# HPCForge/Bubbleformer

Hardware: AMD Instinct MI355X
Metric: train samples/sec, FiLMAViT 16x192x192x4ch, bs=8 per GPU (higher is better)
Workload: dtype bf16; 1 GPU; FiLMAViT-small (E=384, 6 heads, 12 blocks, P=16, 9 fluid params) fwd + relative-L2 loss + bwd + AdamW, 4-field 16x192x192 clips, batch 8 per GPU (BASELINE.json configs[1]); global_batch=8, parallelism=dp1

## Files before the change

### bubbleformer_amd/_lib.py

```python
import ctypes as C
import os
import subprocess

_HERE = os.path.dirname(os.path.abspath(__file__))
LIB_PATH = os.path.join(_HERE, "libbubbleformer_hip.so")
CSRC = os.path.join(_HERE, "csrc")

BF_DTYPE_F32, BF_DTYPE_BF16 = 0, 1
BF_LAY_KC, BF_LAY_XC = 0, 1
BF_PRO_NONE, BF_PRO_AFFINE, BF_PRO_AFFINE_GELU, BF_PRO_GELU = 0, 1, 2, 3
BF_AUX_NONE, BF_AUX_ADD, BF_AUX_DGELU = 0, 1, 2
BF_OUT_STORE, BF_OUT_STORE_F32, BF_OUT_ATOMIC_F32 = 0, 1, 2
BF_MAX_STAGES = 5
BF_LOSS_LIMBS = 5

vp, fp, i32, i64, f32 = C.c_void_p, C.c_void_p, C.c_int32, C.c_int64, C.c_float


class Operand(C.Structure):
    _fields_ = [("p", vp), ("ld", i64), ("layout", i32), ("seglen", i32), ("segstride", i64), ("gw", i32), ("gh", i32),
                ("gc", i32), ("pro", i32), ("sc", fp), ("sh", fp), ("rows_per_frame", i32), ("nch", i32)]


class Epilogue(C.Structure):
    _fields_ = [("bias", fp), ("colscale", fp), ("colshift", fp), ("aux_mode", i32), ("aux", vp), ("ld_aux", i64),
                ("out_mode", i32), ("c", vp), ("ldc", i64), ("seglen", i32), ("segstride", i64), ("gw", i32), ("gh", i32),
                ("gc", i32), ("gelu_out", vp), ("colsum", fp), ("rowscale", fp), ("rows_per_group", i32)]


class Dims(C.Structure):
    _fields_ = [(n, i32) for n in ("dtype", "B", "T", "h", "w", "E", "heads", "attn_scale", "feat_scale", "patch", "cin",
                                   "cout", "nfluid")]


TEMPORAL_FIELDS = ("gamma", "attn_scale_factor", "norm1_w", "norm1_b", "norm2_w", "norm2_b", "input_head_w", "input_head_b",
                   "output_head_w", "output_head_b", "qnorm_w", "qnorm_b", "knorm_w", "knorm_b", "rel_pos_emb")
SPATIAL_FIELDS = ("gamma_att", "gamma_mlp", "attn_scale_factor_x", "attn_scale_factor_y", "low_freq_scalar",
                  "high_freq_scalar", "norm1_w", "norm1_b", "norm2_w", "norm2_b", "input_head_w", "input_head_b",
                  "output_head_w", "output_head_b", "qnorm_w", "qnorm_b", "knorm_w", "knorm_b", "rel_pos_emb", "fc1_w", "fc1_b",
                  "fc2_w", "fc2_b", "mlp_norm_w", "mlp_norm_b")


class TemporalParams(C.Structure):
    _fields_ = [(n, fp) for n in TEMPORAL_FIELDS]


class SpatialParams(C.Structure):
    _fields_ = [(n, fp) for n in SPATIAL_FIELDS]


class FrameNorm(C.Structure):
    _fields_ = [("w", fp), ("b", fp), ("g", fp), ("gdiv", i32), ("mean", fp), ("rstd", fp), ("sc", fp), ("sh", fp), ("resid", vp), ("out", vp)]


class EmbedParams(C.Structure):
    _fields_ = [("conv_w", fp * BF_MAX_STAGES), ("in_w", fp * BF_MAX_STAGES), ("in_b", fp * BF_MAX_STAGES), ("film_ln_w", fp),
                ("film_ln_b", fp), ("film_w", fp), ("film_b", fp)]


class DebedParams(C.Structure):
    _fields_ = [("conv_w", fp * BF_MAX_STAGES), ("in_w", fp * BF_MAX_STAGES), ("in_b", fp * BF_MAX_STAGES)]


class ConvSrc(C.Structure):
    _fields_ = [("p", vp), ("C", i32), ("nchw", i32), ("f32", i32)]


class ConvGeo(C.Structure):
    _fields_ = [(n, i32) for n in ("F", "Hi", "Wi", "Ho", "Wo", "kh", "kw", "stride", "pad")]


BF_CONV_PRO_NONE, BF_CONV_PRO_AFFINE_GELU, BF_CONV_PRO_GELU = 0, 1, 2


class RenderTile(C.Structure):
    _fields_ = [("a", fp), ("b", fp), ("mask", fp), ("frame_stride", i64), ("slot_stride", i64), ("mask_frame_stride", i64), ("mask_slot_stride", i64),
                ("range", vp), ("kind", i32)]


class RenderGeom(C.Structure):
    _fields_ = [(n, i32) for n in ("H", "W", "scale", "rows", "cols", "ox", "oy", "pitch_x", "pitch_y", "bar_dx", "bar_w", "img_h", "img_w", "stride")] + [
        ("stroke", C.c_double)]


BF_RENDER_SDF, BF_RENDER_TEMP, BF_RENDER_SPEED = 0, 1, 2
BF_RENDER_MAX_TILES = 6

STAGE_DONE_FN = C.CFUNCTYPE(None, C.c_int, C.c_void_p)
P = C.POINTER
SIGNATURES = {
    "bf_last_error": (C.c_char_p, []),
    "bf_abi_version": (C.c_int, []),
    "bf_prof_enable": (None, [C.c_int]),
    "bf_debug_force_generic_attn": (None, [C.c_int]),
    "bf_debug_tokred_fold": (None, [C.c_int]),
    "bf_side_defer": (None, [C.c_int]),
    "bf_prep_stages": (C.c_int, [C.POINTER(Dims), C.c_int, C.POINTER(C.c_int32), C.POINTER(vp), C.POINTER(vp), C.POINTER(vp), vp]),
    "bf_stage_prepared": (None, [C.c_int]),
    "bf_trunk_train_fwd": (C.c_int, [C.POINTER(Dims), C.c_int, C.POINTER(C.c_int32), C.POINTER(vp), C.POINTER(vp), C.POINTER(vp), C.POINTER(vp), vp,
                                     C.POINTER(vp), vp, vp]),
    "bf_trunk_train_bwd": (C.c_int, [C.POINTER(Dims), C.c_int, C.POINTER(C.c_int32), C.POINTER(vp), C.POINTER(vp), C.POINTER(vp), C.POINTER(vp),
                                     C.POINTER(vp), vp, C.POINTER(vp), vp, C.POINTER(vp), vp, vp, vp, vp, vp]),
    "bf_field_stats_ws_doubles": (i64, [C.c_int]),
    "bf_field_stats": (C.c_int, [fp, vp, vp, C.c_int, vp, vp, vp]),
    "bf_stage_chain_next": (C.c_int, [C.POINTER(Dims), C.c_int, vp, vp]),
    "bf_stage_next_scale": (C.c_int, [fp, C.c_int]),
    "bf_gemm_fwd_frames": (C.c_int, [C.c_int, C.c_int, C.c_int, C.c_int, vp, i64, vp, i64, fp, fp, fp, fp, C.c_int, vp, vp, C.c_int,
                                     C.POINTER(FrameNorm), C.POINTER(FrameNorm), vp]),
    "bf_trunk_eval_weights_bytes": (i64, [C.POINTER(Dims), C.c_int, C.POINTER(C.c_int32)]),
    "bf_trunk_eval_prepare": (C.c_int, [C.POINTER(Dims), C.c_int, C.POINTER(C.c_int32), C.POINTER(vp), vp, vp]),
    "bf_trunk_eval_fwd": (C.c_int, [C.POINTER(Dims), C.c_int, C.POINTER(C.c_int32), C.POINTER(vp), vp, vp, vp, vp, vp]),
    "bf_frame_linear": (C.c_int, [C.c_int, C.c_int, C.c_int, C.c_int, C.c_int, vp, i64, vp, i64, fp, fp, fp, fp, fp, vp, i64, C.c_int, fp, fp, fp,
                                  vp, i64, fp, fp, vp, i64, vp]),
    "bf_side_join": (C.c_int, [vp]),
    "bf_prof_report": (C.c_int, [C.c_char_p, C.c_int]),
    "bf_gemm": (C.c_int, [C.c_int, C.c_int, C.c_int, C.c_int, P(Operand), P(Operand), P(Epilogue), C.c_int, vp]),
    "bf_gemm_tokred": (C.c_int, [C.c_int, C.c_int, C.c_int, i64, vp, i64, vp, i64, fp, C.c_int, fp, fp, i64, vp]),
    "bf_gemm_tokred_ws_floats": (i64, [C.c_int, C.c_int, i64]),
    "bf_gemm_inbwd_frames": (C.c_int, [C.c_int, C.c_int, C.c_int, C.c_int, vp, i64, vp, i64, vp, vp, vp, C.c_int, fp, fp, fp, fp, fp, C.c_int, vp]),
    "bf_gemm_inbwd_frames_chain": (C.c_int, [C.c_int, C.c_int, C.c_int, C.c_int, vp, i64, vp, i64, vp, vp, vp, C.c_int, fp, fp, fp, fp, fp, C.c_int,
                                             vp, vp, fp, fp, fp, fp, C.c_int, fp, vp]),
    "bf_in_stats": (C.c_int, [C.c_int, vp, C.c_int, C.c_int, C.c_int, fp, fp, fp, C.c_int, fp, fp, fp, fp, fp, fp, vp]),
    "bf_in_ws_floats": (i64, [C.c_int, C.c_int, C.c_int, C.c_int]),
    "bf_affine_apply": (C.c_int, [C.c_int, vp, vp, fp, fp, vp, i64, C.c_int, C.c_int, vp]),
    "bf_in_bwd": (C.c_int, [C.c_int, vp, vp, vp, vp, C.c_int, C.c_int, C.c_int, fp, fp, fp, fp, fp, C.c_int, C.c_int, fp, fp,
                            fp, fp, fp, vp]),
    "bf_colsum": (C.c_int, [C.c_int, vp, i64, C.c_int, fp, fp, vp]),
    "bf_attn_axial_fwd": (C.c_int, [C.c_int, vp, vp, i64, C.c_int, C.c_int, C.c_int, C.c_int, fp, fp, fp, fp, fp, fp, fp, vp]),
    "bf_attn_axial_norm_fwd": (C.c_int, [C.c_int, vp, vp, vp, i64, C.c_int, C.c_int, C.c_int, C.c_int, fp, fp, fp, fp, fp, fp, fp, fp, fp, fp, fp, fp,
                                         fp, vp]),
    "bf_attn_fwd": (C.c_int, [C.c_int, vp, vp, i64, C.c_int, i64, i64, i64, i64, C.c_int, C.c_int, fp, fp, fp, fp, fp, fp, f32,
                              C.c_int, vp]),
    "bf_attn_bwd": (C.c_int, [C.c_int, vp, vp, vp, i64, C.c_int, i64, i64, i64, i64, C.c_int, C.c_int, fp, fp, fp, fp, fp, fp,
                              fp, fp, fp, fp, fp, fp, f32, C.c_int, fp, i64, vp]),
    "bf_im2col_nchw": (C.c_int, [C.c_int, fp, vp, C.c_int, C.c_int, C.c_int, C.c_int, C.c_int, vp]),
    "bf_col2im_nchw": (C.c_int, [C.c_int, vp, fp, C.c_int, C.c_int, C.c_int, C.c_int, C.c_int, vp]),
    "bf_pm2nchw": (C.c_int, [fp, fp, fp, fp, C.c_int, C.c_int, C.c_int, C.c_int, C.c_int, vp]),
    "bf_debed_last_bwd": (C.c_int, [C.c_int, fp, fp, fp, fp, fp, vp, vp, vp, C.c_int, C.c_int, C.c_int, C.c_int, C.c_int, C.c_int, vp]),
    "bf_debed_last_bwd_norm": (C.c_int, [C.c_int, fp, fp, fp, fp, fp, vp, vp, vp, fp, fp, fp, fp, vp, fp, fp, C.c_int, C.c_int, C.c_int, C.c_int, C.c_int,
                                         C.c_int, fp, C.c_int64, vp]),
    "bf_gather_gemm": (C.c_int, [C.c_int, vp, vp, C.c_int, fp, fp, vp, C.c_int, C.c_int, C.c_int, C.c_int, C.c_int, vp]),
    "bf_scatter_gemm": (C.c_int, [C.c_int, vp, vp, C.c_int, fp, fp, vp, fp, C.c_int, C.c_int, C.c_int, C.c_int, C.c_int, vp]),
    "bf_gather_wgrad_ws_floats": (C.c_int64, [C.c_int, C.c_int, C.c_int]),
    "bf_gather_wgrad": (C.c_int, [C.c_int, vp, vp, fp, fp, fp, fp, fp, C.c_int, C.c_int, C.c_int, C.c_int, C.c_int, C.c_int, fp, C.c_int64, vp]),
    "bf_gather_gemm_rebuilt": (C.c_int, [C.c_int, vp, vp, vp, C.c_int, fp, fp, vp, C.c_int, C.c_int, C.c_int, C.c_int, C.c_int, vp]),
    "bf_gather_wgrad_rebuilt": (C.c_int, [C.c_int, vp, vp, vp, fp, fp, fp, C.c_int, C.c_int, C.c_int, C.c_int, C.c_int, C.c_int, fp, C.c_int64, vp]),
    "bf_stage_chain_head": (C.c_int, [vp, vp, vp]),
    "bf_stage_chain_tail": (C.c_int, [vp, vp, C.c_int]),
    "bf_embed_tail_ws_floats": (C.c_int64, [C.c_int, C.c_int, C.c_int, C.c_int, C.c_int]),
    "bf_embed_tail_bwd": (C.c_int, [C.c_int, vp, vp, vp, vp, vp, fp, fp, fp, fp, fp, fp, fp, fp, C.c_int, C.c_int, C.c_int, C.c_int, C.c_int, C.c_int,
                                    fp, C.c_int64, vp]),
    "bf_embed_first": (C.c_int, [C.c_int, fp, vp, vp, vp, C.c_int, C.c_int, C.c_int, C.c_int, C.c_int, C.c_int, fp, vp]),
    "bf_in_stats_merge_slices": (C.c_int, [C.c_int, C.c_int, C.c_int, C.c_int, C.c_int, fp, fp, fp, C.c_int, fp, fp, fp, fp, fp, fp, vp]),
    "bf_debed_last": (C.c_int, [C.c_int, vp, fp, fp, vp, fp, fp, fp, C.c_int, C.c_int, C.c_int, C.c_int, C.c_int, C.c_int, vp]),
    "bf_lploss_finalize": (C.c_int, [fp, C.c_int, C.c_int, fp, fp, vp]),
    "bf_nchw2pm": (C.c_int, [C.c_int, fp, fp, fp, fp, fp, vp, C.c_int, C.c_int, C.c_int, C.c_int, C.c_int, vp]),
    "bf_wprep": (C.c_int, [C.c_int, C.c_int, fp, vp, C.c_int, C.c_int, C.c_int, vp]),
    "bf_wgrad_unprep": (C.c_int, [C.c_int, fp, fp, C.c_int, C.c_int, C.c_int, C.c_int, vp]),
    "bf_film_net_fwd": (C.c_int, [fp, fp, fp, fp, fp, fp, fp, fp, C.c_int, C.c_int, C.c_int, vp]),
    "bf_film_net_bwd": (C.c_int, [fp, fp, fp, fp, fp, fp, fp, fp, fp, C.c_int, C.c_int, C.c_int, vp]),
    "bf_adamw": (C.c_int, [fp, fp, fp, fp, i64, C.c_int, f32, f32, f32, f32, f32, f32, vp]),
    "bf_adam": (C.c_int, [fp, fp, fp, fp, i64, C.c_int, f32, f32, f32, f32, f32, f32, vp]),
    "bf_lion": (C.c_int, [fp, fp, fp, i64, f32, f32, f32, f32, f32, vp]),
    "bf_grad_norm_ws_doubles": (i64, [i64]),
    "bf_grad_norm": (C.c_int, [fp, i64, f32, f32, fp, vp, i64, vp]),
    "bf_adamw_dev": (C.c_int, [fp, fp, fp, fp, i64, C.c_int, f32, f32, f32, f32, f32, f32, fp, f32, vp]),
    "bf_adam_dev": (C.c_int, [fp, fp, fp, fp, i64, C.c_int, f32, f32, f32, f32, f32, f32, fp, f32, vp]),
    "bf_lion_dev": (C.c_int, [fp, fp, fp, i64, f32, f32, f32, f32, f32, fp, f32, vp]),
    "bf_eikonal_sum": (C.c_int, [fp, i64, C.c_int, C.c_int, f32, vp, vp]),
    "bf_eikonal_l1_frames": (C.c_int, [fp, i64, C.c_int, C.c_int, f32, fp, vp]),
    "bf_heatflux_rows": (C.c_int, [fp, fp, i64, i64, C.c_int, f32, f32, f32, f32, fp, vp]),
    "bf_clip_gather": (C.c_int, [fp, i64, vp, vp, C.c_int, fp, fp, fp, C.c_int, C.c_int, C.c_int, C.c_int, C.c_int, C.c_int, C.c_int, vp]),
    "bf_clip_gather_batch": (C.c_int, [fp, i64, vp, i64, vp, vp, fp, fp, C.c_int, C.c_int, fp, vp, fp, fp, C.c_int, C.c_int, fp, fp, vp, C.c_int, fp,
                                       C.c_int, C.c_int, C.c_int, C.c_int, C.c_int, vp]),
    "bf_rollout_score_ws_doubles": (i64, [C.c_int, C.c_int, C.c_int, C.c_int, C.c_int]),
    "bf_rollout_score": (C.c_int, [fp, fp, i64, i64, C.c_int, vp, vp, vp, fp, fp, C.c_int, f32, fp, fp, fp, fp, fp, fp, vp, i64, C.c_int, C.c_int,
                                   C.c_int, C.c_int, C.c_int, C.c_int, C.c_int, C.c_int, vp]),
    "bf_rollout_heatflux": (C.c_int, [fp, fp, i64, i64, C.c_int, vp, vp, vp, fp, fp, C.c_int, C.c_int, fp, f32, f32, f32, f32, fp, fp, C.c_int, C.c_int,
                                      C.c_int, C.c_int, C.c_int, C.c_int, C.c_int, C.c_int, vp]),
    "bf_kde_kl_ws_doubles": (i64, [C.c_int, i64, i64, C.c_int]),
# ... 100 lines not shown
```

### bubbleformer_amd/csrc/bf_common.h

```cpp
#pragma once
#include <hip/hip_runtime.h>
#include <stdint.h>
#include <math.h>

#include "../../include/bubbleformer_hip.h"

typedef __bf16 bf16;
typedef __attribute__((ext_vector_type(8))) __bf16 bf16x8;
typedef __attribute__((ext_vector_type(4))) __bf16 bf16x4;
typedef __attribute__((ext_vector_type(4))) short s16x4;
typedef __attribute__((ext_vector_type(4))) float f32x4;

#define BF_WAVE 64
#define BF_IN_EPS 1e-5f

#define BF_CHECK_LAUNCH()                                   \
    do {                                                    \
        hipError_t e__ = hipGetLastError();                 \
        if (e__ != hipSuccess) return bf_fail(e__, __FILE__, __LINE__); \
    } while (0)
#define BF_REQUIRE(cond, msg)                                \
    do {                                                     \
        if (!(cond)) return bf_fail_msg(msg, __FILE__, __LINE__); \
    } while (0)

int bf_prof_begin(hipStream_t st);
bool bf_prof_is_on();
void bf_prof_end(int idx, hipStream_t st, const char* name, double flops, double bytes);
struct BfProfScope {
    int idx; hipStream_t st; const char* name; double flops, bytes;
    BfProfScope(hipStream_t s, const char* n, double f, double b) : idx(bf_prof_begin(s)), st(s), name(n), flops(f), bytes(b) {}
    ~BfProfScope() { if (idx >= 0) bf_prof_end(idx, st, name, flops, bytes); }
};

int bf_in_bwd_partials(int dtype, const void* dy, const void* x, const void* add, void* dx, int frames, int S, int C, const float* mean,
                       const float* rstd, const float* w, const float* b, const float* g, int gdiv, int gelu, float* ws, hipStream_t stream);
int bf_attn_bwd_partials(int dtype, const void* qkv, const void* dout, void* dqkv, int64_t nseq, int L, int64_t inner, int64_t outer_stride,
                         int64_t inner_stride, int64_t tok_stride, int heads, int d, const float* qw, const float* qb, const float* kw,
                         const float* kb, const float* emb, const float* hscale, float* dqw, float* dqb, float* dkw, float* dkb, float* demb,
                         float* dhscale, float out_scale, int accumulate, float* ws, int64_t ws_floats, int* rows, hipStream_t stream);
int bf_in_stats_apply(int dtype, const void* x, int frames, int S, int C, const float* w, const float* b, const float* g, int gdiv, const float* gb,
                      float* mean, float* rstd, float* sc, float* sh, float* ws, const void* resid, void* out, hipStream_t stream);
int bf_in_stats_apply_chain(int dtype, const void* x, int frames, int S, int C, const float* w, const float* b, const float* g, int gdiv, const float* gb,
                            float* mean, float* rstd, float* sc, float* sh, float* ws, const void* resid, void* out, const float* nw, const float* nb,
                            float* nmean, float* nrstd, float* nsc, float* nsh, void* nxn, bool* chained, hipStream_t stream);
int bf_wprep_multi(int dtype, int n, const int* mode, const float* const* src, void* const* dst, const int* R, const int* K, const int* Kp, hipStream_t st);
int bf_frame_scale(int dtype, const void* z, const float* m, int fdiv, void* out, long nrows, int S, int C, hipStream_t st);

int bf_gemm_slabs(int dtype, int M, int N, int K, const bf_operand* A, const bf_operand* B, float* out, long ldc, int accumulate, int splitk,
                  float* ws, long ws_floats, hipStream_t st);
int bf_tokred_narrow(int dtype, int C, int64_t P, const void* wide, const void* narrow, float* out, int ldo, int accumulate, int transposed,
                     const float* sc, const float* sh, int64_t rows_per_frame, float* ws, int64_t ws_floats, hipStream_t st);
int bf_gemm_pair_scaled(int M, int N, int K, const bf_operand* A, const bf_operand* B, const bf_epilogue* E, void* out2, const float* rowfac,
                        int rows_per_group, hipStream_t st);

#ifdef BF_EXPERIMENTS
#include <stdlib.h>
inline int bf_knob(const char* name, int dflt) { const char* v = getenv(name); return v ? atoi(v) : dflt; }
#else
constexpr int bf_knob(const char*, int dflt) { return dflt; }
#endif

struct BfPerDeviceOnce {
    bool done[64] = {};
    bool& flag() { int dev = 0; (void)hipGetDevice(&dev); return done[(dev >= 0 && dev < 64) ? dev : 0]; }
};
template <class T> struct BfPerDevice {
    T tab[64] = {};
    T& get() { int dev = 0; (void)hipGetDevice(&dev); return tab[(dev >= 0 && dev < 64) ? dev : 0]; }
};
int bf_fail(hipError_t e, const char* file, int line);
int bf_fail_msg(const char* msg, const char* file, int line);
int bf_decline(const char* msg);

__device__ __forceinline__ float to_f(float x) { return x; }
__device__ __forceinline__ float to_f(bf16 x) { return (float)x; }
template <typename T> __device__ __forceinline__ T from_f(float x);
template <> __device__ __forceinline__ float from_f<float>(float x) { return x; }
template <> __device__ __forceinline__ bf16 from_f<bf16>(float x) { return (bf16)x; }

template <typename T> struct Chunk;
template <> struct Chunk<float> {
    static constexpr int N = 4;
    float4 raw;
    __device__ __forceinline__ void load(const float* p) { raw = *reinterpret_cast<const float4*>(p); }
    __device__ __forceinline__ void store(float* p) const { *reinterpret_cast<float4*>(p) = raw; }
    __device__ __forceinline__ void zero() { raw = make_float4(0.f, 0.f, 0.f, 0.f); }
    __device__ __forceinline__ float get(int i) const { return i == 0 ? raw.x : i == 1 ? raw.y : i == 2 ? raw.z : raw.w; }
    __device__ __forceinline__ void set(int i, float v) { if (i == 0) raw.x = v; else if (i == 1) raw.y = v; else if (i == 2) raw.z = v; else raw.w = v; }
};
template <> struct Chunk<bf16> {
    static constexpr int N = 8;
    bf16x8 raw;
    __device__ __forceinline__ void load(const bf16* p) { raw = *reinterpret_cast<const bf16x8*>(p); }
    __device__ __forceinline__ void store(bf16* p) const { *reinterpret_cast<bf16x8*>(p) = raw; }
    __device__ __forceinline__ void zero() { for (int i = 0; i < 8; ++i) raw[i] = (bf16)0.f; }
    __device__ __forceinline__ float get(int i) const { return (float)raw[i]; }
    __device__ __forceinline__ void set(int i, float v) { raw[i] = (bf16)v; }
};

__device__ __forceinline__ float erf_fast(float x) {
    const float ax = fabsf(x);
    const float t = __builtin_amdgcn_rcpf(1.0f + 0.3275911f * ax);
    const float poly = t * (0.254829592f + t * (-0.284496736f + t * (1.421413741f + t * (-1.453152027f + t * 1.061405429f))));
    const float r = 1.0f - poly * __expf(-ax * ax);
    return copysignf(r, x);
}
__device__ __forceinline__ float gelu_f(float x) { return 0.5f * x * (1.0f + erf_fast(x * 0.70710678118654752440f)); }
__device__ __forceinline__ float dgelu_f(float x) {
    const float ax = fabsf(x) * 0.70710678118654752440f;
    const float t = __builtin_amdgcn_rcpf(1.0f + 0.3275911f * ax);
    const float poly = t * (0.254829592f + t * (-0.284496736f + t * (1.421413741f + t * (-1.453152027f + t * 1.061405429f))));
    const float e = __expf(-0.5f * x * x);
    const float cdf = 0.5f * (1.0f + copysignf(1.0f - poly * e, x));
    return cdf + x * (0.39894228040143267794f * e);
}

__device__ __forceinline__ float phi_fast(float x) {
    const float xc = fminf(fmaxf(x, -4.0f), 4.0f), u = xc * xc;
    float r = -1.520480094e-09f;
    r = r * u + 1.180964698e-07f; r = r * u - 4.014221545e-06f; r = r * u + 7.960997465e-05f; r = r * u - 1.041295800e-03f;
    r = r * u + 9.641715296e-03f; r = r * u - 6.614117438e-02f; r = r * u + 3.988329119e-01f;
    return 0.5f + xc * r;
}
__device__ __forceinline__ float gelu_fast(float x) { return x * phi_fast(x); }
__device__ __forceinline__ float dgelu_fast(float x) {
    const float xc = fminf(fmaxf(x, -4.0f), 4.0f), u = xc * xc;
    float r = 9.387459194e-10f;
    r = r * u - 7.941240515e-08f; r = r * u + 2.950722870e-06f; r = r * u - 6.380590451e-05f; r = r * u + 8.975979855e-04f;
// ... 21 lines not shown
```

### bubbleformer_amd/csrc/embed_debed.hip

```cpp
#include "model_common.h"

using namespace bfm;

namespace {
inline int roundup(int v, int m) { return (v + m - 1) / m * m; }

struct EmbedSaved {
    float *gb, *dgb, *chat, *crstd;
    void* patches; int Kp;
    void* y[BF_MAX_STAGES]; void* wc[BF_MAX_STAGES];
    float *mean[BF_MAX_STAGES], *rstd[BF_MAX_STAGES], *sc[BF_MAX_STAGES], *sh[BF_MAX_STAGES];
    int C[BF_MAX_STAGES], gh[BF_MAX_STAGES], gw[BF_MAX_STAGES]; long P[BF_MAX_STAGES];
    size_t bytes;
    EmbedSaved(const D& d, void* base) {
        Arena a(base);
        const int np = d.nfluid > 0 ? d.nfluid : 1;
        gb = a.f32((size_t)2 * d.B * d.E); dgb = a.f32((size_t)2 * d.B * d.E); chat = a.f32((size_t)d.B * np); crstd = a.f32(d.B);
        Kp = roundup(4 * d.cin, 8);
        const int H = d.h * d.patch, W = d.w * d.patch;
        for (int i = 0; i < d.nst; ++i) {
            C[i] = (i == d.nst - 1) ? d.E : d.E / 4;
            gh[i] = H >> (i + 1); gw[i] = W >> (i + 1);
            P[i] = d.F * gh[i] * gw[i];
        }
        patches = a.take((size_t)P[0] * Kp * d.es);
        for (int i = 0; i < d.nst; ++i) {
            const int kin = i == 0 ? Kp : 4 * C[i - 1];
            y[i] = a.take((size_t)P[i] * C[i] * d.es);
            wc[i] = a.take((size_t)C[i] * kin * d.es);
            const size_t fc = (size_t)d.F * C[i];
            mean[i] = a.f32(fc); rstd[i] = a.f32(fc); sc[i] = a.f32(fc); sh[i] = a.f32(fc);
        }
        bytes = a.off;
    }
};
struct DebedSaved {
    float *lossbuf, *coef;
    void* y[BF_MAX_STAGES]; void* wc[BF_MAX_STAGES];
    float *mean[BF_MAX_STAGES], *rstd[BF_MAX_STAGES], *sc[BF_MAX_STAGES], *sh[BF_MAX_STAGES];
    int Cin[BF_MAX_STAGES], Co[BF_MAX_STAGES], gh[BF_MAX_STAGES], gw[BF_MAX_STAGES]; long Pin[BF_MAX_STAGES];
    int Np;
    size_t bytes;
    DebedSaved(const D& d, void* base) {
        Arena a(base);
        lossbuf = a.f32((size_t)d.F * d.cout * 2 * 2 * BF_LOSS_LIMBS); coef = a.f32((size_t)d.F * d.cout);
        Np = roundup(4 * d.cout, 8);
        for (int i = 0; i < d.nst; ++i) {
            Cin[i] = i == 0 ? d.E : d.E / 4;
            Co[i] = (i == d.nst - 1) ? d.cout : d.E / 4;
            gh[i] = d.h << i; gw[i] = d.w << i;
            Pin[i] = d.F * gh[i] * gw[i];
            const bool last = i == d.nst - 1;
            wc[i] = a.take((size_t)Cin[i] * (last ? Np : 4 * Co[i]) * d.es);
            if (!last) {
                y[i] = a.take((size_t)Pin[i] * 4 * Co[i] * d.es);
                const size_t fc = (size_t)d.F * Co[i];
                mean[i] = a.f32(fc); rstd[i] = a.f32(fc); sc[i] = a.f32(fc); sh[i] = a.f32(fc);
            } else { y[i] = nullptr; mean[i] = rstd[i] = sc[i] = sh[i] = nullptr; }
        }
        bytes = a.off;
    }
};
int wgrad_slabs_else_atomics(const D& d, const Scratch& sc, int M, int N, long K, const bf_operand& A, const bf_operand& Bo, long ld, hipStream_t ss,
                             bool slabs = true) {
    const int splitk = splitk_for(M, N, K);
    const int src = slabs ? bf_gemm_slabs(d.dtype, M, N, (int)K, &A, &Bo, sc.wg, ld, 0, splitk, (float*)sc.t1b, sc.t1b_floats, ss) : 1;
    if (src <= 0) return src;
    ZERO_ON(ss, sc.wg, (size_t)M * N * 4);
    bf_epilogue e = epi_atomic(sc.wg, ld);
    return bf_gemm(d.dtype, M, N, (int)K, &A, &Bo, &e, splitk, ss);
}
}

extern "C" int64_t bf_embed_saved_bytes(const bf_dims* s) { D d; if (get_dims(s, &d) || d.nst < 1) return -1; return (int64_t)EmbedSaved(d, nullptr).bytes; }
extern "C" int64_t bf_debed_saved_bytes(const bf_dims* s) { D d; if (get_dims(s, &d) || d.nst < 1) return -1; return (int64_t)DebedSaved(d, nullptr).bytes; }

extern "C" int bf_embed_fwd(const bf_dims* dims, const bf_embed_params* p, const float* x, const float* fluid, void* out, void* saved,
                            void* scratch, bf_stream_t s) {
    D d; TRY(get_dims(dims, &d));
    BF_REQUIRE(p && x && out && saved && scratch && d.nst >= 1 && d.cin >= 1, "bf_embed_fwd: bad arguments");
    BF_REQUIRE((d.nfluid > 0) == (fluid != nullptr), "bf_embed_fwd: fluid parameters must be given exactly when nfluid > 0");
    hipStream_t st = (hipStream_t)s;
    TrunkLinks& L = links();
    L.clear(true);
    TRY(side_join_pending(L, st));
    EmbedSaved sv(d, saved);
    Scratch sc(d, scratch);
    const int n = d.nst, H = d.h * d.patch, W = d.w * d.patch;
    if (d.nfluid > 0)
        TRY(bf_film_net_fwd(fluid, p->film_ln_w, p->film_ln_b, p->film_w, p->film_b, sv.gb, sv.chat, sv.crstd, d.B, d.nfluid, 2 * d.E, st));
    bool stats_done = false;
    {
        int mode[BF_MAX_STAGES], R[BF_MAX_STAGES], K[BF_MAX_STAGES], Kp[BF_MAX_STAGES];
        const float* src[BF_MAX_STAGES]; void* dst[BF_MAX_STAGES];
        for (int i = 0; i < n; ++i) {
            src[i] = p->conv_w[i]; dst[i] = sv.wc[i]; mode[i] = i == 0 ? 0 : 1; R[i] = sv.C[i];
            K[i] = i == 0 ? 4 * d.cin : 4 * sv.C[i - 1]; Kp[i] = i == 0 ? sv.Kp : K[i];
        }
        TRY(bf_wprep_multi(d.dtype, n, mode, src, dst, R, K, Kp, st));
    }
    for (int i = 0; i < n; ++i) {
        const void* wc;
        if (i == 0) {
            wc = sv.wc[0];
            const int S0 = sv.gh[0] * sv.gw[0];
            static const bool part_on = bf_knob("BF_EMBED_STATS", 1) != 0;
            const bool part_ok = part_on && n > 1 && bf_in_ws_floats(d.dtype, (int)d.F, S0, sv.C[0]) >= (int64_t)2 * d.F * sv.C[0] * (1 + (S0 + 255) / 256);
            static const bool lean_on = bf_knob("BF_EMBED_LEAN", 1) != 0;
            const int64_t tail_need = n > 1 ? bf_embed_tail_ws_floats((int)d.F, sv.gh[1], sv.gw[1], sv.C[0], sv.Kp) : 0;
            const bool bwd_fits = tail_need > 0 && tail_need + (int64_t)sv.C[0] * sv.Kp <= sc.tokred_floats && d.F <= 512 &&
                                  (int64_t)d.F * (4 * 96 * 96) <= sc.t1b_floats;
            const bool lean = lean_on && part_ok && bwd_fits && d.dtype == BF_DTYPE_BF16 && sv.Kp == 16 && d.cin <= 4 && sv.C[0] == 96 && sv.C[1] == 96 && (W / 2) % 16 == 0 &&
                              sv.gw[1] % 16 == 0 && ((long)sv.gh[1] * sv.gw[1]) % 128 == 0 && S0 >= 1024;
            const int rc = bf_embed_first(d.dtype, x, wc, sv.patches, lean ? nullptr : sv.y[0], (int)d.F, sv.C[0], d.cin, H / 2, W / 2, sv.Kp,
                                          part_ok ? sc.in_ws + (size_t)2 * d.F * sv.C[0] : nullptr, st);
            if (rc < 0) return rc;
            if (rc == 1 && lean) return bf_fail_msg("bf_embed_fwd: the first-stage kernel declined a shape the lean path was chosen for", __FILE__, __LINE__);
            L.embed_lean_set(saved, lean);
            stats_done = rc == 0 && part_ok;
            if (rc == 1) {
                TRY(bf_im2col_nchw(d.dtype, x, sv.patches, (int)d.F, d.cin, H, W, sv.Kp, st));
                bf_operand A = op_plain(sv.patches, sv.Kp, BF_LAY_KC);
                bf_operand Bo = op_plain(wc, sv.Kp, BF_LAY_KC);
                bf_epilogue e = epi_store(sv.y[0], sv.C[0]);
                TRY(bf_gemm(d.dtype, (int)sv.P[0], sv.C[0], sv.Kp, &A, &Bo, &e, 1, st));
            }
        } else {
            const int cp = sv.C[i - 1];
            const bool reb = i == 1 && L.embed_lean_get(saved);
            const int grc = reb ? bf_gather_gemm_rebuilt(d.dtype, sv.patches, sv.wc[0], sv.wc[i], 0, sv.sc[0], sv.sh[0], sv.y[i], (int)d.F, sv.gh[i], sv.gw[i], cp, sv.C[i], st)
                                : bf_gather_gemm(d.dtype, sv.y[i - 1], sv.wc[i], 0, sv.sc[i - 1], sv.sh[i - 1], sv.y[i], (int)d.F, sv.gh[i], sv.gw[i], cp, sv.C[i], st);
            if (grc < 0) return grc;
            if (grc == 1 && reb) return bf_fail_msg("bf_embed_fwd: the rebuilt-rows stage kernel declined a shape the lean path was chosen for", __FILE__, __LINE__);
            if (grc == 1) {
                bf_operand A = op_plain(sv.y[i - 1], cp, BF_LAY_KC);
                op_gather(A, sv.gw[i], sv.gh[i], cp);
                op_affine(A, BF_PRO_AFFINE_GELU, sv.sc[i - 1], sv.sh[i - 1], (long)sv.gh[i] * sv.gw[i], cp);
                bf_operand Bo = op_plain(sv.wc[i], 4L * cp, BF_LAY_KC);
                bf_epilogue e = epi_store(sv.y[i], sv.C[i]);
                TRY(bf_gemm(d.dtype, (int)sv.P[i], sv.C[i], 4 * cp, &A, &Bo, &e, 1, st));
            }
        }
        const bool last = i == n - 1;
        const bool film = last && d.nfluid > 0;
        if (i == 0 && stats_done) {
            const int mrc = bf_in_stats_merge_slices(d.dtype, (int)d.F, sv.gh[0] * sv.gw[0], sv.C[0], 256, p->in_w[0], p->in_b[0], nullptr, 1, nullptr,
                                                     sv.mean[0], sv.rstd[0], sv.sc[0], sv.sh[0], sc.in_ws, st);
            if (mrc < 0) return mrc;
            if (mrc == 0) continue;
            if (L.embed_lean_get(saved)) return bf_fail_msg("bf_embed_fwd: slice statistics declined on the lean path", __FILE__, __LINE__);
        }
        if (last) {
            TRY(bf_in_stats_apply(d.dtype, sv.y[i], (int)d.F, sv.gh[i] * sv.gw[i], sv.C[i], p->in_w[i], p->in_b[i], film ? sv.gb : nullptr, d.T,
                                  film ? sv.gb + (size_t)d.B * d.E : nullptr, sv.mean[i], sv.rstd[i], sv.sc[i], sv.sh[i], sc.in_ws, nullptr, out, st));
            break;
        }
        TRY(bf_in_stats(d.dtype, sv.y[i], (int)d.F, sv.gh[i] * sv.gw[i], sv.C[i], p->in_w[i], p->in_b[i], film ? sv.gb : nullptr, d.T,
                        film ? sv.gb + (size_t)d.B * d.E : nullptr, sv.mean[i], sv.rstd[i], sv.sc[i], sv.sh[i], sc.in_ws, st));
    }
    return 0;
}

extern "C" int bf_embed_bwd(const bf_dims* dims, const bf_embed_params* p, const bf_embed_params* g, const void* dout, float* dx_in,
                            void* saved, void* scratch, bf_stream_t s) {
    D d; TRY(get_dims(dims, &d));
    BF_REQUIRE(p && g && dout && saved && scratch && d.nst >= 1, "bf_embed_bwd: bad arguments");
    hipStream_t st = (hipStream_t)s;
    TrunkLinks& L = links();
    TRY(side_join_pending(L, st));
    EmbedSaved sv(d, saved);
    Scratch sc(d, scratch);
    const int n = d.nst, H = d.h * d.patch, W = d.w * d.patch;
    auto buf = [&](int stage) { return (stage & 1) ? sc.t3 : sc.t4; };
    const bool film = d.nfluid > 0;
    if (film) ZERO(sv.dgb, (size_t)2 * d.B * d.E * 4);
    void* dy = buf(n - 1);
    TRY(bf_in_bwd(d.dtype, dout, sv.y[n - 1], nullptr, dy, (int)d.F, sv.gh[n - 1] * sv.gw[n - 1], sv.C[n - 1], sv.mean[n - 1], sv.rstd[n - 1],
                  p->in_w[n - 1], p->in_b[n - 1], film ? sv.gb : nullptr, d.T, 0, g->in_w[n - 1], g->in_b[n - 1], film ? sv.dgb : nullptr,
                  film ? sv.dgb + (size_t)d.B * d.E : nullptr, sc.in_ws, st));
    if (film)
        TRY(bf_film_net_bwd(sv.dgb, sv.chat, p->film_ln_w, p->film_ln_b, p->film_w, g->film_w, g->film_b, g->film_ln_w, g->film_ln_b, d.B,
                            d.nfluid, 2 * d.E, st));
    Fork fk(L, st);
    hipStream_t ss;
    for (int i = n - 1; i >= 1; --i) {
        const int cp = sv.C[i - 1], K4 = 4 * cp;
        const long rpf = (long)sv.gh[i] * sv.gw[i];
        TRY(fk.join());
        TRY(fk.begin(&ss));
        const bool lean = L.embed_lean_get(saved);
        if (i == 1 && lean && dx_in) {
            bf_operand A0 = op_plain(sv.patches, sv.Kp, BF_LAY_KC);
            bf_operand B0 = op_plain(sv.wc[0], sv.Kp, BF_LAY_KC);
            bf_epilogue e0 = epi_store(sv.y[0], sv.C[0]);
            TRY(bf_gemm(d.dtype, (int)sv.P[0], sv.C[0], sv.Kp, &A0, &B0, &e0, 1, st));
            L.embed_lean_set(saved, false);
            TRY(fk.join());
            TRY(fk.begin(&ss));
        }
        const bool reb = i == 1 && L.embed_lean_get(saved);
        const int wrc = reb ? bf_gather_wgrad_rebuilt(d.dtype, sv.patches, sv.wc[0], dy, sv.sc[0], sv.sh[0], sc.wg, 1, (int)d.F, sv.gh[i], sv.gw[i], cp, sv.C[i],
                                                      (float*)sc.t1b, sc.t1b_floats, ss)
                            : bf_gather_wgrad(d.dtype, sv.y[i - 1], dy, sv.sc[i - 1], sv.sh[i - 1], nullptr, nullptr, sc.wg, 1, (int)d.F, sv.gh[i], sv.gw[i], cp,
                                              sv.C[i], (float*)sc.t1b, sc.t1b_floats, ss);
        if (wrc < 0) return wrc;
        if (wrc == 1 && reb) return bf_fail_msg("bf_embed_bwd: the rebuilt-rows weight gradient declined a shape the lean path was chosen for", __FILE__, __LINE__);
        if (wrc == 1) {
            bf_operand A = op_plain(dy, sv.C[i], BF_LAY_XC);
            bf_operand Bo = op_plain(sv.y[i - 1], cp, BF_LAY_XC);
            op_gather(Bo, sv.gw[i], sv.gh[i], cp);
            op_affine(Bo, BF_PRO_AFFINE_GELU, sv.sc[i - 1], sv.sh[i - 1], rpf, cp);
            TRY(wgrad_slabs_else_atomics(d, sc, sv.C[i], K4, sv.P[i], A, Bo, K4, ss));
        }
        TRY(bf_wgrad_unprep(1, sc.wg, g->conv_w[i], sv.C[i], K4, K4, 0, ss));
        if (i == 1 && !dx_in) {
            static const bool tail_on = bf_knob("BF_EMBED_TAIL", 1) != 0;
            const int64_t need = bf_embed_tail_ws_floats((int)d.F, sv.gh[1], sv.gw[1], cp, sv.Kp);
            if (tail_on && need > 0 && need + (int64_t)cp * sv.Kp <= sc.tokred_floats) {
                float* dwprep = sc.tokred_ws + need;
                static const bool tail_map = bf_knob("BF_EMBED_TAIL_MAP", 0) != 0;
                const int trc = bf_embed_tail_bwd(d.dtype, dy, sv.wc[1], (tail_map && !L.embed_lean_get(saved)) ? sv.y[0] : nullptr, sv.patches, sv.wc[0], sv.sc[0], sv.sh[0], sv.mean[0], sv.rstd[0],
                                                  p->in_w[0], dwprep, g->in_w[0], g->in_b[0], (int)d.F, sv.gh[1], sv.gw[1], sv.C[1], cp, sv.Kp,
                                                  sc.tokred_ws, need, s);
                if (trc < 0) return trc;
                if (trc == 0) {
                    TRY(bf_wgrad_unprep(0, dwprep, g->conv_w[0], sv.C[0], 4 * d.cin, sv.Kp, 0, st));
                    return fk.join();
                }
            }
            if (L.embed_lean_get(saved)) return bf_fail_msg("bf_embed_bwd: the one-pass tail declined on the lean path (no stored stage-0 map)", __FILE__, __LINE__);
        }
        void* dact = buf(i - 1);
        {
            const int src = bf_scatter_gemm(d.dtype, dy, sv.wc[i], 1, nullptr, nullptr, dact, nullptr, (int)d.F, sv.gh[i], sv.gw[i], sv.C[i], cp, st);
            if (src < 0) return src;
            if (src == 1) {
                bf_operand A = op_plain(dy, sv.C[i], BF_LAY_KC);
                bf_operand Bo = op_plain(sv.wc[i], K4, BF_LAY_XC);
                bf_epilogue e = epi_store(dact, cp);
                epi_scatter(e, sv.gw[i], sv.gh[i], cp);
                TRY(bf_gemm(d.dtype, (int)sv.P[i], K4, sv.C[i], &A, &Bo, &e, 1, st));
            }
        }
        TRY(bf_in_bwd(d.dtype, dact, sv.y[i - 1], nullptr, dact, (int)d.F, sv.gh[i - 1] * sv.gw[i - 1], cp, sv.mean[i - 1], sv.rstd[i - 1],
                      p->in_w[i - 1], p->in_b[i - 1], nullptr, 1, 1, g->in_w[i - 1], g->in_b[i - 1], nullptr, nullptr, sc.in_ws, st));
        dy = dact;
    }
    {
        TRY(fk.join());
        if (dx_in) TRY(fk.begin(&ss)); else ss = st;
        const int nrc = sv.Kp == 16 ? bf_tokred_narrow(d.dtype, sv.C[0], sv.P[0], dy, sv.patches, sc.wg, sv.Kp, 0, 0, nullptr, nullptr, 0, sc.tokred_ws, sc.tokred_floats, ss) : 1;
        if (nrc < 0) return nrc;
        if (nrc == 1) {
            bf_operand A = op_plain(dy, sv.C[0], BF_LAY_XC);
            bf_operand Bo = op_plain(sv.patches, sv.Kp, BF_LAY_XC);
            TRY(wgrad_slabs_else_atomics(d, sc, sv.C[0], sv.Kp, sv.P[0], A, Bo, sv.Kp, ss));
        }
        TRY(bf_wgrad_unprep(0, sc.wg, g->conv_w[0], sv.C[0], 4 * d.cin, sv.Kp, 0, ss));
        if (dx_in) {
            void* dpatch = sc.t1;
            bf_operand A2 = op_plain(dy, sv.C[0], BF_LAY_KC);
            bf_operand B2 = op_plain(sv.wc[0], sv.Kp, BF_LAY_XC);
            bf_epilogue e2 = epi_store(dpatch, sv.Kp);
            TRY(bf_gemm(d.dtype, (int)sv.P[0], sv.Kp, sv.C[0], &A2, &B2, &e2, 1, st));
            TRY(bf_col2im_nchw(d.dtype, dpatch, dx_in, (int)d.F, d.cin, H, W, sv.Kp, st));
        }
    }
    return fk.join();
}

extern "C" int bf_debed_fwd(const bf_dims* dims, const bf_debed_params* p, const void* x, float* pred, const float* target, float* loss,
                            void* saved, void* scratch, bf_stream_t s) {
    D d; TRY(get_dims(dims, &d));
    BF_REQUIRE(p && x && pred && saved && scratch && d.nst >= 1 && d.cout >= 1, "bf_debed_fwd: bad arguments");
    BF_REQUIRE(!target || loss, "bf_debed_fwd: loss output missing");
    hipStream_t st = (hipStream_t)s;
    TrunkLinks& L = links();
    TRY(side_join_pending(L, st));
    DebedSaved sv(d, saved);
    Scratch sc(d, scratch);
    const int n = d.nst;
    {
        int mode[BF_MAX_STAGES], R[BF_MAX_STAGES], K[BF_MAX_STAGES], Kp[BF_MAX_STAGES];
        const float* src[BF_MAX_STAGES]; void* dst[BF_MAX_STAGES];
        for (int i = 0; i < n; ++i) {
            const bool last = i == n - 1;
            src[i] = p->conv_w[i]; dst[i] = sv.wc[i]; mode[i] = last ? 0 : 2;
            R[i] = last ? sv.Cin[i] : 4 * sv.Co[i]; K[i] = last ? 4 * sv.Co[i] : sv.Cin[i]; Kp[i] = last ? sv.Np : sv.Cin[i];
        }
        TRY(bf_wprep_multi(d.dtype, n, mode, src, dst, R, K, Kp, st));
    }
    for (int i = 0; i < n; ++i) {
        const bool last = i == n - 1;
        const int cin = sv.Cin[i], co = sv.Co[i];
        bf_operand A = op_plain(i == 0 ? x : sv.y[i - 1], cin, BF_LAY_KC);
        if (i > 0) op_affine(A, BF_PRO_AFFINE_GELU, sv.sc[i - 1], sv.sh[i - 1], (long)sv.gh[i] * sv.gw[i], cin);
        if (!last) {
            const int S4 = 4 * sv.gh[i] * sv.gw[i];
            const bool part_ok = i > 0 && S4 % 128 == 0 &&
                                 bf_in_ws_floats(d.dtype, (int)d.F, S4, co) >= (int64_t)2 * d.F * co * (1 + S4 / 128);
            const int src = i > 0 ? bf_scatter_gemm(d.dtype, sv.y[i - 1], sv.wc[i], 0, sv.sc[i - 1], sv.sh[i - 1], sv.y[i],
                                                    part_ok ? sc.in_ws + (size_t)2 * d.F * co : nullptr, (int)d.F, sv.gh[i], sv.gw[i], cin, co, st) : 1;
            if (src < 0) return src;
            if (src == 0 && part_ok) {
                const int mrc = bf_in_stats_merge_slices(d.dtype, (int)d.F, S4, co, 128, p->in_w[i], p->in_b[i], nullptr, 1, nullptr, sv.mean[i], sv.rstd[i],
                                                         sv.sc[i], sv.sh[i], sc.in_ws, st);
                if (mrc < 0) return mrc;
                if (mrc == 0) continue;
            }
            if (src == 1) {
                bf_operand Bo = op_plain(sv.wc[i], cin, BF_LAY_KC);
                bf_epilogue e = epi_store(sv.y[i], co);
                epi_scatter(e, sv.gw[i], sv.gh[i], co);
                TRY(bf_gemm(d.dtype, (int)sv.Pin[i], 4 * co, cin, &A, &Bo, &e, 1, st));
            }
            TRY(bf_in_stats(d.dtype, sv.y[i], (int)d.F, S4, co, p->in_w[i], p->in_b[i], nullptr, 1, nullptr, sv.mean[i],
                            sv.rstd[i], sv.sc[i], sv.sh[i], sc.in_ws, st));
        } else {
            if (target) ZERO(sv.lossbuf, (size_t)d.F * d.cout * 2 * BF_LOSS_LIMBS * 8);
            const int rc = i > 0 ? bf_debed_last(d.dtype, sv.y[i - 1], sv.sc[i - 1], sv.sh[i - 1], sv.wc[i], pred, target, sv.lossbuf, (int)d.F, cin, co,
                                                 sv.gh[i], sv.gw[i], sv.Np, st) : 1;
            if (rc < 0) return rc;
            if (rc == 1) {
                bf_operand Bo = op_plain(sv.wc[i], sv.Np, BF_LAY_XC);
                float* pm = (float*)sc.t4;
                bf_epilogue e = epi_store(pm, sv.Np);
                e.out_mode = BF_OUT_STORE_F32;
                TRY(bf_gemm(d.dtype, (int)sv.Pin[i], sv.Np, cin, &A, &Bo, &e, 1, st));
                TRY(bf_pm2nchw(pm, pred, target, sv.lossbuf, (int)d.F, co, sv.gh[i], sv.gw[i], sv.Np, st));
            }
            if (target) TRY(bf_lploss_finalize(sv.lossbuf, (int)d.F, co, loss, sv.coef, st));
        }
    }
    return 0;
}

extern "C" int bf_debed_bwd(const bf_dims* dims, const bf_debed_params* p, const bf_debed_params* g, const void* x, const float* dpred,
                            const float* pred, const float* target, const float* loss_scale, void* dx, void* saved, void* scratch,
                            bf_stream_t s) {
    D d; TRY(get_dims(dims, &d));
    BF_REQUIRE(p && g && x && dx && saved && scratch && d.nst >= 1, "bf_debed_bwd: bad arguments");
    BF_REQUIRE(dpred || (pred && target), "bf_debed_bwd: need dpred or (pred, target) of the fused loss");
    hipStream_t st = (hipStream_t)s;
    TrunkLinks& L = links();
    L.clear(false);
    TRY(side_join_pending(L, st));
    DebedSaved sv(d, saved);
    Scratch sc(d, scratch);
    const int n = d.nst;
    auto buf = [&](int stage) { return (stage & 1) ? sc.t3 : sc.t4; };
    void* dy = nullptr;
    Fork fk(L, st);
    hipStream_t ss;
    for (int i = n - 1; i >= 0; --i) {
        const bool last = i == n - 1;
        const int cin = sv.Cin[i], co = sv.Co[i];
        const long rpf = (long)sv.gh[i] * sv.gw[i];
        const void* ain = i == 0 ? x : sv.y[i - 1];
        void* dact = i == 0 ? dx : buf(i);
        bool normed = false;
        if (last) {
            void* dpm = sc.t1;
            if (i > 0) {
                const int nrc = bf_debed_last_bwd_norm(d.dtype, dpred, pred, target, sv.coef, loss_scale, sv.wc[i], dpm, ain, sv.mean[i - 1], sv.rstd[i - 1],
                                                       p->in_w[i - 1], p->in_b[i - 1], dact, g->in_w[i - 1], g->in_b[i - 1], (int)d.F, cin, co, sv.gh[i],
                                                       sv.gw[i], sv.Np, sc.in_ws, bf_in_ws_floats(d.dtype, (int)d.F, (int)rpf, cin), st);
                if (nrc < 0) return nrc;
                normed = nrc == 0;
            }
            const int rc = normed ? 0 : bf_debed_last_bwd(d.dtype, dpred, pred, target, sv.coef, loss_scale, sv.wc[i], dpm, dact, (int)d.F, cin, co, sv.gh[i], sv.gw[i], sv.Np, st);
            if (rc < 0) return rc;
            if (rc == 1) TRY(bf_nchw2pm(d.dtype, dpred, pred, target, sv.coef, loss_scale, dpm, (int)d.F, co, sv.gh[i], sv.gw[i], sv.Np, st));
            TRY(fk.begin(&ss));
            const int nrc = (sv.Np == 16 && i > 0) ? bf_tokred_narrow(d.dtype, cin, sv.Pin[i], ain, dpm, sc.wg, cin, 0, 1, sv.sc[i - 1], sv.sh[i - 1], rpf,
                                                                      sc.tokred_ws, sc.tokred_floats, ss) : 1;
            if (nrc < 0) return nrc;
            if (nrc == 1) {
                bf_operand A = op_plain(dpm, sv.Np, BF_LAY_XC);
                bf_operand Bo = op_plain(ain, cin, BF_LAY_XC);
                if (i > 0) op_affine(Bo, BF_PRO_AFFINE_GELU, sv.sc[i - 1], sv.sh[i - 1], rpf, cin);
                TRY(wgrad_slabs_else_atomics(d, sc, sv.Np, cin, sv.Pin[i], A, Bo, cin, ss, cin % 4 == 0));
            }
            TRY(bf_wgrad_unprep(0, sc.wg, g->conv_w[i], cin, 4 * co, sv.Np, 1, ss));
            if (rc == 1) {
                bf_operand A = op_plain(dpm, sv.Np, BF_LAY_KC);
                bf_operand Bo = op_plain(sv.wc[i], sv.Np, BF_LAY_KC);
                bf_epilogue e = epi_store(dact, cin);
                TRY(bf_gemm(d.dtype, (int)sv.Pin[i], cin, sv.Np, &A, &Bo, &e, 1, st));
            }
        } else {
            const int N4 = 4 * co;
            TRY(fk.join());
            TRY(fk.begin(&ss));
            const int wrc = i > 0 ? bf_gather_wgrad(d.dtype, dy, ain, nullptr, nullptr, sv.sc[i - 1], sv.sh[i - 1], sc.wg, 0, (int)d.F, sv.gh[i], sv.gw[i], co,
                                                    cin, (float*)sc.t1b, sc.t1b_floats, ss) : 1;
            if (wrc < 0) return wrc;
            if (wrc == 1) {
                bf_operand A = op_plain(dy, co, BF_LAY_XC);
                op_gather(A, sv.gw[i], sv.gh[i], co);
                bf_operand Bo = op_plain(ain, cin, BF_LAY_XC);
                if (i > 0) op_affine(Bo, BF_PRO_AFFINE_GELU, sv.sc[i - 1], sv.sh[i - 1], rpf, cin);
                TRY(wgrad_slabs_else_atomics(d, sc, N4, cin, sv.Pin[i], A, Bo, cin, ss));
            }
            TRY(bf_wgrad_unprep(2, sc.wg, g->conv_w[i], N4, cin, cin, 0, ss));
            {
                const int grc = bf_gather_gemm(d.dtype, dy, sv.wc[i], 1, nullptr, nullptr, dact, (int)d.F, sv.gh[i], sv.gw[i], co, cin, st);
                if (grc < 0) return grc;
                if (grc == 1) {
                    bf_operand A = op_plain(dy, co, BF_LAY_KC);
                    op_gather(A, sv.gw[i], sv.gh[i], co);
                    bf_operand Bo = op_plain(sv.wc[i], cin, BF_LAY_XC);
                    bf_epilogue e = epi_store(dact, cin);
                    TRY(bf_gemm(d.dtype, (int)sv.Pin[i], cin, N4, &A, &Bo, &e, 1, st));
                }
            }
        }
        if (i > 0) {
            if (!normed)
                TRY(bf_in_bwd(d.dtype, dact, sv.y[i - 1], nullptr, dact, (int)d.F, (int)rpf, cin, sv.mean[i - 1], sv.rstd[i - 1], p->in_w[i - 1],
                              p->in_b[i - 1], nullptr, 1, 1, g->in_w[i - 1], g->in_b[i - 1], nullptr, nullptr, sc.in_ws, st));
            dy = dact;
        }
    }
    return fk.join();
}
```

### bubbleformer_amd/csrc/model.hip

```cpp
#include "model_common.h"

bool bf_attn_raw_modes(int dtype, int d);
int bf_gemm_tokred_deferred(int dtype, int Nout, int Kin, int64_t M, const void* dy, int64_t ldy, const void* x, int64_t ldx, float* out,
                            int accumulate, float* colsum, float* ws, int64_t ws_floats, hipStream_t stream);
const float* bf_gemm_tokred_pending_out();
int bf_gemm_inbwd_frames_scaled(int dtype, int M, int N, int K, const void* A, int64_t lda, const void* B, int64_t ldb, const void* x,
                                const void* add, void* out, int S, const float* mean, const float* rstd, const float* w, float* ws,
                                const float* fscale, int fdiv, void* out_s, const float* f_s, int fdiv_s, hipStream_t stream);

using namespace bfm;

namespace {

bool g_side_defer = false;

BfPerDevice<TrunkLinks> g_links;

int launch_reduce_jobs(ReduceJobs& J, hipStream_t st);
__global__ void __launch_bounds__(256) stage_prep_multi_kernel(PrepBatch b);

}

bool bfm::side_defer() { return g_side_defer; }
TrunkLinks& bfm::links() { return g_links.get(); }
int bfm::flush_pending_reduce(TrunkLinks& L, hipStream_t st) {
    if (!L.reduce.on) return 0;
    L.reduce.on = false;
    TRY(launch_reduce_jobs(L.reduce.jobs, L.reduce.st));
    return L.hand_over(L.reduce.st, st);
}
int bfm::side_join_pending(TrunkLinks& L, hipStream_t main, int set) {
    if (set < 0) TRY(flush_pending_reduce(L, main));
    SideStream* s = L.side_stream();
    if (set < 0 && bf_gemm_tokred_pending()) {
        hipStream_t ws_st = s ? s->st : main;
        TRY(bf_gemm_tokred_flush(ws_st));
        if (s) { HIP_TRY(hipEventRecord(s->join, s->st)); HIP_TRY(hipStreamWaitEvent(main, s->join, 0)); }
    }
    if (!s) return 0;
    for (int i = 0; i < 2; ++i)
        if ((set < 0 || set == i) && s->pending[i]) {
            HIP_TRY(hipStreamWaitEvent(main, s->tail[i], 0));
            s->pending[i] = false;
        }
    return 0;
}
int bfm::launch_stage_prep(const D& d, const PrepBatch& b, int m, int planes, hipStream_t st) {
    hipLaunchKernelGGL(stage_prep_multi_kernel, dim3(std::max(64, d.E), planes, m), dim3(256), 0, st, b);
    BF_CHECK_LAUNCH();
    return 0;
}

namespace {

int launch_with_pending(TrunkLinks& L, ReduceJobs& J, hipStream_t st) {
    if (L.reduce.on && L.reduce.st == st && J.fits(L.reduce.jobs)) {
        L.reduce.on = false;
        const ReduceJobs& P = L.reduce.jobs;
        for (int i = 0; i < P.n_in; ++i) TRY(J.push(P.in[i]));
        for (int i = 0; i < P.n_attn; ++i) TRY(J.push(P.at[i]));
    }
    TRY(flush_pending_reduce(L, st));
    return launch_reduce_jobs(J, st);
}

__device__ __forceinline__ void outproj_prep_row(const float* __restrict__ W, const float* __restrict__ bias, const float* __restrict__ nb,
                                                 const float* __restrict__ gamma, const float* __restrict__ lo, const float* __restrict__ hi,
                                                 float* __restrict__ alpha, float* __restrict__ beta, float* __restrict__ mc, int E, int n,
                                                 void* __restrict__ wscaled, int dtype) {
    __shared__ float red[4];
    __shared__ float s_alpha;
    float acc = 0.f;
    if (lo) for (int k = threadIdx.x; k < E; k += blockDim.x) acc += W[(long)n * E + k] * nb[k];
    acc = wave_sum(acc);
    if ((threadIdx.x & 63) == 0) red[threadIdx.x >> 6] = acc;
    __syncthreads();
    if (threadIdx.x == 0) {
        float m = bias[n];
        for (int i = 0; i < (int)(blockDim.x >> 6); ++i) m += red[i];
        const float l = lo ? lo[n] : 0.f, h = hi ? hi[n] : 0.f, g = gamma[n];
        alpha[n] = g * (1.f + h);
        beta[n] = g * (bias[n] * (1.f + h) + (lo ? m * (l - h) : 0.f));
        mc[n] = m;
        s_alpha = g * (1.f + h);
    }
    if (wscaled) {
        __syncthreads();
        const float al = s_alpha;
        for (int k = threadIdx.x; k < E; k += blockDim.x) {
            const float v = al * W[(long)n * E + k];
            if (dtype == BF_DTYPE_BF16) reinterpret_cast<bf16*>(wscaled)[(long)n * E + k] = (bf16)v;
            else reinterpret_cast<float*>(wscaled)[(long)n * E + k] = v;
        }
    }
}
__global__ void __launch_bounds__(256) outproj_prep_kernel(PrepArgs a) {
    outproj_prep_row(a.W, a.bias, a.nb, a.gamma, a.lo, a.hi, a.alpha, a.beta, a.mc, a.E, blockIdx.x, a.wscaled, a.dtype);
}
__global__ void outproj_finalize_kernel(const float* __restrict__ G, const float* __restrict__ csum, const float* __restrict__ W,
                                        const float* __restrict__ bias, const float* __restrict__ nb, const float* __restrict__ gamma,
                                        const float* __restrict__ lo, const float* __restrict__ hi, const float* __restrict__ mc,
                                        float* __restrict__ dW, float* __restrict__ dbias, float* __restrict__ dnb, float* __restrict__ dgamma,
                                        float* __restrict__ dlo, float* __restrict__ dhi, int E) {
    __shared__ float red[4];
    __shared__ float s_dmc, s_alpha;
    if ((int)blockIdx.x >= E) {
        __shared__ float part[16][16];
        __shared__ float coef[1024];
        for (int n = threadIdx.x; n < E; n += blockDim.x) coef[n] = csum[n] * gamma[n] * (lo[n] - hi[n]);
        __syncthreads();
        const int c = threadIdx.x & 15, k = ((int)blockIdx.x - E) * 16 + c, q = threadIdx.x >> 4;
        float a = 0.f;
        if (k < E) {
            int n = q;
            for (; n + 112 < E; n += 128) {
                float wv[8];
// ... 261 lines not shown
    bf_operand A = op_plain(dy, Kdim, BF_LAY_KC);
    bf_operand Bo = op_plain(w_xc, Nout, BF_LAY_XC);
    bf_epilogue e = epi_store(tmp, Nout);
    if (f.fscale) { e.rowscale = f.fscale; e.rows_per_group = (int)(d.S * f.fdiv); }
    TRY(bf_gemm(d.dtype, (int)d.N, Nout, Kdim, &A, &Bo, &e, 1, st));
    return bf_in_bwd_partials(d.dtype, tmp, f.x, f.add, f.dx, (int)d.F, (int)d.S, Nout, f.mean, f.rstd, f.w, f.b, nullptr, 1, 0, f.ws, st);
}
int outproj_bwd(const D& d, const Scratch& sc, const void* dout, const void* on, const void* w_s,
                const float* W, const float* bias, const float* nb, const float* gamma, const float* lo, const float* hi,
                const float* alpha, const float* mc, float* dW, float* dbias, float* dnb, float* dgamma, float* dlo, float* dhi,
                void* don, hipStream_t st, Fork& fk, const InFuse* fu = nullptr) {
    TRY(fk.run([=](hipStream_t ss) -> int {
        const void* dsrc = dout;
        const int trc = bf_gemm_tokred_deferred(d.dtype, d.E, d.E, d.N, dsrc, d.E, on, d.E, sc.G, 0, sc.csum, sc.tokred_ws, sc.tokred_floats, ss);
        if (trc < 0) return trc;
        if (trc == 1) {
            ZERO_ON(ss, sc.G, (size_t)((char*)sc.csum - (char*)sc.G) + (size_t)d.E * 4);
            bf_operand A = op_plain(dsrc, d.E, BF_LAY_XC);
            bf_operand Bo = op_plain(on, d.E, BF_LAY_XC);
            bf_epilogue e = epi_atomic(sc.G, d.E);
            e.colsum = sc.csum;
            TRY(bf_gemm(d.dtype, d.E, d.E, (int)d.N, &A, &Bo, &e, splitk_for(d.E, d.E, d.N), ss));
        }
        return 0;
    }));
    fk.run_late([=](hipStream_t ss) -> int {
        if (bf_gemm_tokred_pending_out() == sc.G) TRY(bf_gemm_tokred_flush(ss));
        hipLaunchKernelGGL(outproj_finalize_kernel, dim3(d.E + (lo ? bf_cdiv(d.E, 16) : 0)), dim3(256), 0, ss, sc.G, sc.csum, W, bias, nb, gamma, lo, hi, mc,
                           dW, dbias, dnb, dgamma, dlo, dhi, d.E);
        BF_CHECK_LAUNCH();
        return 0;
    });
    if (fu) return dgrad_inbwd(d, dout, d.E, w_s, d.E, don, *fu, st);
    {
        bf_operand A = op_plain(dout, d.E, BF_LAY_KC);
        bf_operand Bo = op_plain(w_s, d.E, BF_LAY_XC);
        bf_epilogue e = epi_store(don, d.E);
        TRY(bf_gemm(d.dtype, (int)d.N, d.E, d.E, &A, &Bo, &e, 1, st));
    }
    return 0;
}
int linear_bwd(const D& d, const Scratch& sc, const void* dy, int Nout, const void* x, int Kin, int xpro, const float* xsc, const float* xsh,
               const void* w_c, float* dW, float* db, void* dxn, const bf_epilogue* dx_epi, hipStream_t st, Fork& fk, const InFuse* fu = nullptr,
               bool last = false, const void* w_t = nullptr, void* scaled_out = nullptr, const float* rowfac = nullptr, int rpg = 1,
               bool* scaled_done = nullptr) {
    TRY(fk.run([=](hipStream_t ss) -> int {
        const void* xo = x;
        int pro = xpro;
        bf_operand A = op_plain(dy, Nout, BF_LAY_XC);
        if (pro == BF_PRO_AFFINE) {
            TRY(bf_affine_apply(d.dtype, x, nullptr, xsc, xsh, sc.s1, d.N, (int)d.S, Kin, ss));
            xo = sc.s1;
            pro = BF_PRO_NONE;
        }
        bf_operand Bo = op_plain(xo, Kin, BF_LAY_XC);
        if (pro == BF_PRO_NONE) {
            const int trc = bf_gemm_tokred_deferred(d.dtype, Nout, Kin, d.N, dy, Nout, xo, Kin, dW, 1, db, sc.tokred_ws, sc.tokred_floats, ss);
            if (trc <= 0) return trc;
        }
        if (pro != BF_PRO_NONE) op_affine(Bo, pro, xsc, xsh, d.S, Kin);
        bf_epilogue e = epi_atomic(dW, Kin);
        e.colsum = db;
        return bf_gemm(d.dtype, Nout, Kin, (int)d.N, &A, &Bo, &e, splitk_for(Nout, Kin, d.N), ss);
    }));
    if (last) TRY(fk.flush());
    if (fu) return dgrad_inbwd(d, dy, Nout, w_c, Kin, dxn, *fu, st);
    {
        bf_operand A = op_plain(dy, Nout, BF_LAY_KC);
        bf_operand Bo = w_t ? op_plain(w_t, Nout, BF_LAY_KC) : op_plain(w_c, Kin, BF_LAY_XC);
        bf_epilogue e = dx_epi ? *dx_epi : epi_store(dxn, Kin);
        e.c = dxn; e.ldc = Kin;
        if (scaled_out && rowfac && d.dtype == BF_DTYPE_BF16) {
            const int rc = bf_gemm_pair_scaled((int)d.N, Kin, Nout, &A, &Bo, &e, scaled_out, rowfac, rpg, st);
            if (rc < 0) return rc;
            if (rc == 0) { if (scaled_done) *scaled_done = true; return 0; }
        }
        TRY(bf_gemm(d.dtype, (int)d.N, Kin, Nout, &A, &Bo, &e, 1, st));
    }
    return 0;
}

}

extern "C" int64_t bf_temporal_saved_bytes(const bf_dims* s) { D d; if (get_dims(s, &d)) return -1; return (int64_t)TemporalSaved(d, nullptr).bytes; }
extern "C" int64_t bf_spatial_saved_bytes(const bf_dims* s) { D d; if (get_dims(s, &d)) return -1; return (int64_t)SpatialSaved(d, nullptr).bytes; }
static size_t dbr_bytes(const D& d) { return (((size_t)d.N * d.E * d.es) + 255) & ~(size_t)255; }
extern "C" int64_t bf_scratch_bytes(const bf_dims* s) { D d; if (get_dims(s, &d)) return -1; return 2 * (int64_t)Scratch(d, nullptr).bytes + 2 * (int64_t)dbr_bytes(d); }

extern "C" void bf_side_defer(int on) { g_side_defer = on != 0; }
extern "C" int bf_side_join(bf_stream_t s) { return side_join_pending(g_links.get(), (hipStream_t)s); }

extern "C" void bf_stage_prepared(int on) { g_links.get().hints.prepared = on != 0; }
extern "C" int bf_stage_chain_tail(const bf_spatial_params* prev_p, const void* prev_saved, int has_drop_mlp) {
    g_links.get().hints.tail = NextTail{prev_p && prev_saved, prev_p, prev_saved, has_drop_mlp != 0};
    return 0;
}
extern "C" int bf_stage_next_scale(const float* factors, int fdiv) { g_links.get().hints.scale = NextScale{factors, fdiv > 0 ? fdiv : 1}; return 0; }
static NextHead next_head(const D& d, int kind, const void* params, void* saved) {
    auto of = [&](auto* np, const auto& sv) { return NextHead{true, np->norm1_w, np->norm1_b, sv.mean1, sv.rstd1, sv.sc1, sv.sh1, sv.xn, saved}; };
    return kind == 0 ? of((const bf_temporal_params*)params, TemporalSaved(d, saved)) : of((const bf_spatial_params*)params, SpatialSaved(d, saved));
}
extern "C" int bf_stage_chain_next(const bf_dims* dims, int next_kind, const void* next_params, void* next_saved) {
    NextHead& h = g_links.get().hints.head;
    h = NextHead{};
    if (!dims || !next_params || !next_saved) return 0;
    BF_REQUIRE(next_kind == 0 || next_kind == 1, "bf_stage_chain_next: kind must be 0 (temporal) or 1 (spatial)");
    D d; TRY(get_dims(dims, &d));
    h = next_head(d, next_kind, next_params, next_saved);
    return 0;
}
extern "C" int bf_stage_chain_head(const bf_dims* dims, const bf_temporal_params* next_p, void* next_saved) {
    return bf_stage_chain_next(dims, 0, next_p, next_saved);
}

static int temporal_fwd(TrunkLinks& L, const StageHints& H, const bf_dims* dims, const bf_temporal_params* p, const void* x, void* out, void* saved,
                        void* scratch, const float* drop, bf_stream_t s) {
    D d; TRY(get_dims(dims, &d));
    BF_REQUIRE(p && x && out && saved && scratch, "bf_temporal_fwd: null pointer");
    hipStream_t st = (hipStream_t)s;
    const bool head_done = L.take_head_done(saved, st);
    TRY(side_join_pending(L, st));
    TemporalSaved sv(d, saved);
    Scratch sc(d, scratch);
    const void* wv[4];
    TRY(wviews(d, stage_prep(d, 0, p, sv.prep_dst(), nullptr), H.prepared, wv, st));
    const void *win_c = wv[0], *wout_c = wv[1];
    if (!head_done)
        TRY(bf_in_stats_apply(d.dtype, x, (int)d.F, (int)d.S, d.E, p->norm1_w, p->norm1_b, nullptr, 1, nullptr, sv.mean1, sv.rstd1, sv.sc1, sv.sh1, sc.in_ws,
                              nullptr, sv.xn, st));
    TRY(qkv_gemm(d, sv.xn, win_c, p->input_head_b, sv.qkv, st));
    TRY(bf_attn_fwd(d.dtype, sv.qkv, sv.o, (long)d.B * d.S, d.T, d.S, (long)d.T * d.S, 1, d.S, d.heads, d.d, p->qnorm_w, p->qnorm_b,
                    p->knorm_w, p->knorm_b, p->rel_pos_emb, d.attn_scale ? p->attn_scale_factor : nullptr, 1.f, 0, st));
    TRY(bf_in_stats_apply(d.dtype, sv.o, (int)d.F, (int)d.S, d.E, p->norm2_w, p->norm2_b, nullptr, 1, nullptr, sv.mean2, sv.rstd2, sv.sc2, sv.sh2, sc.in_ws,
                          nullptr, sv.on, st));
    if (H.head.armed) {
        const NextHead& h = H.head;
        const bf_frame_norm n2{h.w, h.b, nullptr, 1, h.mean, h.rstd, h.sc, h.sh, nullptr, h.xn};
        const int rc = bf_gemm_fwd_frames(d.dtype, (int)d.N, d.E, d.E, sv.on, d.E, sv.wout_t, d.E, nullptr, sv.alpha, sv.beta, drop, d.T, x, out, (int)d.S,
                                          nullptr, &n2, s);
        if (rc < 0) return rc;
        if (rc == 0) { L.head_done = {h.saved, st}; return 0; }
    }
    TRY(outproj_gemm(d, sv.on, wout_c, sv.alpha, sv.beta, x, out, drop, (long)d.T * d.S, st));
    return 0;
}

static int temporal_bwd(TrunkLinks& L, const StageHints& H, const bf_dims* dims, const bf_temporal_params* p, const bf_temporal_params* g, const void* x,
                        const void* dout, void* dx, void* saved, void* scratch, const float* drop, bf_stream_t s) {
    D d; TRY(get_dims(dims, &d));
    BF_REQUIRE(p && g && x && dout && dx && saved && scratch, "bf_temporal_bwd: null pointer");
    hipStream_t st = (hipStream_t)s;
    TemporalSaved sv(d, saved);
    Scratch sc(d, bwd_scratch(L, d, scratch));
    const void* win_c = d.dtype == BF_DTYPE_F32 ? (const void*)p->input_head_w : sv.win_c;
    Fork fk(L, st, true, L.scratch_parity);
    if (fk.deferred) TRY(side_join_pending(L, st, fk.set));
    void* don = sc.t1;
    void* dO = sc.t1b;
    void* dqkv = sc.t3;
    const void* dbr = dout;
    if (drop) {
        const TrunkLinks::DbrReady& r = L.dbr_ready;
        if (r.dx == dout && r.f == drop && r.buf && r.st == st) dbr = r.buf;
        else {
            TRY(bf_frame_scale(d.dtype, dout, drop, d.T, sc.t4, d.N, (int)d.S, d.E, st));
            dbr = sc.t4;
        }
    }
    L.dbr_ready = TrunkLinks::DbrReady{};
    const InFuse fu2{sv.o, nullptr, dO, sv.mean2, sv.rstd2, p->norm2_w, p->norm2_b, sc.in_ws2};
    TRY(outproj_bwd(d, sc, dbr, sv.on, sv.wout_s, p->output_head_w, p->output_head_b, p->norm2_b, p->gamma, nullptr, nullptr,
                    sv.alpha, sv.mc, g->output_head_w, g->output_head_b, nullptr, g->gamma, nullptr, nullptr, don, st, fk, &fu2));
    ReduceJobs jobs;
    TRY(jobs.push(InReduceJob{sc.in_ws2, (int)d.F, d.E, p->norm2_w, p->norm2_b, nullptr, 1, g->norm2_w, g->norm2_b, nullptr, nullptr, nullptr, nullptr}));
    {
        int rows = 0;
        TRY(bf_attn_bwd_partials(d.dtype, sv.qkv, dO, dqkv, (long)d.B * d.S, d.T, d.S, (long)d.T * d.S, 1, d.S, d.heads, d.d, p->qnorm_w, p->qnorm_b,
                                 p->knorm_w, p->knorm_b, p->rel_pos_emb, d.attn_scale ? p->attn_scale_factor : nullptr, g->qnorm_w, g->qnorm_b,
                                 g->knorm_w, g->knorm_b, g->rel_pos_emb, d.attn_scale ? g->attn_scale_factor : nullptr, 1.f, 0, sc.attn_ws,
                                 Scratch::ATTN_WS_FLOATS, &rows, st));
        TRY(jobs.push(AttnReduceJob{sc.attn_ws, rows, d.d, d.heads, g->qnorm_w, g->qnorm_b, g->knorm_w, g->knorm_b, g->rel_pos_emb,
                                    d.attn_scale ? g->attn_scale_factor : nullptr}));
    }
    void* dxn = sc.t1;
    InFuse fu1{x, dout, dx, sv.mean1, sv.rstd1, p->norm1_w, p->norm1_b, sc.in_ws};
    TailNorm tn;
    bool tail_done = false;
    static const bool chain_on = bf_knob("BF_BWD_CHAIN", 1) != 0;
    if (H.tail.armed && chain_on && fk.deferred && d.dtype == BF_DTYPE_BF16 && d.S == 144 && d.F % 2 == 0) {
        const NextTail& h = H.tail;
        const int oset = L.scratch_parity ^ 1;
        TRY(side_join_pending(L, st, oset));
        Scratch so(d, (char*)scratch + (size_t)oset * Scratch(d, nullptr).bytes);
        SpatialSaved ps(d, const_cast<void*>(h.saved));
        tn = TailNorm{ps.z, so.t1, ps.mean3, ps.rstd3, h.p->mlp_norm_w, h.drop ? ps.gtab : h.p->gamma_mlp, h.drop ? 1 : (int)d.F, L.tail_ws_flip ? so.in_ws5 : so.in_ws4, &tail_done};
        L.tail_ws_flip = !L.tail_ws_flip;
        fu1.tail = &tn;
    }
    if (H.tail.armed) L.tail_done = TrunkLinks::TailDone{};
    TRY(linear_bwd(d, sc, dqkv, 3 * d.E, sv.xn, d.E, BF_PRO_NONE, nullptr, nullptr, win_c, g->input_head_w, g->input_head_b, dxn, nullptr, st, fk, &fu1, true));
    if (tail_done) L.tail_done = {H.tail.saved, dx, tn.ws, st};
    TRY(jobs.push(InReduceJob{sc.in_ws, (int)d.F, d.E, p->norm1_w, p->norm1_b, nullptr, 1, g->norm1_w, g->norm1_b, nullptr, nullptr, nullptr, nullptr}));
    TRY(launch_with_pending(L, jobs, st));
    return fk.join();
}
extern "C" int bf_temporal_fwd(const bf_dims* dims, const bf_temporal_params* p, const void* x, void* out, void* saved, void* scratch,
                               const float* drop, bf_stream_t s) {
    TrunkLinks& L = g_links.get();
    return temporal_fwd(L, L.take_hints(), dims, p, x, out, saved, scratch, drop, s);
}
extern "C" int bf_temporal_bwd(const bf_dims* dims, const bf_temporal_params* p, const bf_temporal_params* g, const void* x, const void* dout,
                               void* dx, void* saved, void* scratch, const float* drop, bf_stream_t s) {
    TrunkLinks& L = g_links.get();
    return temporal_bwd(L, L.take_hints(), dims, p, g, x, dout, dx, saved, scratch, drop, s);
}

static int prep_stages(TrunkLinks& L, const bf_dims* dims, int n, const int32_t* kinds, const void* const* params, void* const* saved,
                       const float* const* drop_mlp, bf_stream_t s) {
    D d; TRY(get_dims(dims, &d));
    BF_REQUIRE(n >= 1 && kinds && params && saved, "bf_prep_stages: bad arguments");
    if (d.dtype != BF_DTYPE_BF16) return 1;
    hipStream_t st = (hipStream_t)s;
    TRY(side_join_pending(L, st));
    for (int i0 = 0; i0 < n; i0 += PREP_BATCH) {
        PrepBatch b;
        memset(&b, 0, sizeof(b));
        const int m = std::min(PREP_BATCH, n - i0);
        for (int i = 0; i < m; ++i) {
            const int k = i0 + i;
            BF_REQUIRE(params[k] && saved[k] && (kinds[k] == 0 || kinds[k] == 1), "bf_prep_stages: bad stage entry");
            b.s[i] = kinds[k] == 0 ? stage_prep(d, 0, params[k], TemporalSaved(d, saved[k]).prep_dst(), nullptr)
                                   : stage_prep(d, 1, params[k], SpatialSaved(d, saved[k]).prep_dst(), drop_mlp ? drop_mlp[k] : nullptr);
        }
        TRY(launch_stage_prep(d, b, m, 7, st));
    }
    return 0;
}
extern "C" int bf_prep_stages(const bf_dims* dims, int n, const int32_t* kinds, const void* const* params, void* const* saved,
                              const float* const* drop_mlp, bf_stream_t s) {
    return prep_stages(g_links.get(), dims, n, kinds, params, saved, drop_mlp, s);
}

static int spatial_fwd(TrunkLinks& L, const StageHints& H, const bf_dims* dims, const bf_spatial_params* p, const void* x, void* out, void* saved,
                       void* scratch, const float* drop_att, const float* drop_mlp, bf_stream_t s) {
    D d; TRY(get_dims(dims, &d));
    BF_REQUIRE(p && x && out && saved && scratch, "bf_spatial_fwd: null pointer");
    hipStream_t st = (hipStream_t)s;
    const bool head_done = L.take_head_done(saved, st);
    TRY(side_join_pending(L, st));
    SpatialSaved sv(d, saved);
    Scratch sc(d, scratch);
    const void* wv[4];
    TRY(wviews(d, stage_prep(d, 1, p, sv.prep_dst(), drop_mlp), H.prepared, wv, st));
    const void *win_c = wv[0], *wout_c = wv[1], *w1_c = wv[2], *w2_c = wv[3];
    if (!head_done)
        TRY(bf_in_stats_apply(d.dtype, x, (int)d.F, (int)d.S, d.E, p->norm1_w, p->norm1_b, nullptr, 1, nullptr, sv.mean1, sv.rstd1, sv.sc1, sv.sh1, sc.in_ws,
                              nullptr, sv.xn, st));
    TRY(qkv_gemm(d, sv.xn, win_c, p->input_head_b, sv.qkv, st));
    {
        const int rc = bf_attn_axial_norm_fwd(d.dtype, sv.qkv, sv.o, sv.on, d.F, (int)d.h, (int)d.w, d.heads, d.d, p->qnorm_w, p->qnorm_b, p->knorm_w,
                                              p->knorm_b, p->rel_pos_emb, d.attn_scale ? p->attn_scale_factor_x : nullptr,
                                              d.attn_scale ? p->attn_scale_factor_y : nullptr, p->norm2_w, p->norm2_b, sv.mean2, sv.rstd2, sv.sc2,
                                              sv.sh2, st);
        if (rc < 0) return rc;
        if (rc == 1) {
            TRY(bf_attn_axial_fwd(d.dtype, sv.qkv, sv.o, d.F, (int)d.h, (int)d.w, d.heads, d.d, p->qnorm_w, p->qnorm_b, p->knorm_w, p->knorm_b,
                                  p->rel_pos_emb, d.attn_scale ? p->attn_scale_factor_x : nullptr, d.attn_scale ? p->attn_scale_factor_y : nullptr, st));
            TRY(bf_in_stats_apply(d.dtype, sv.o, (int)d.F, (int)d.S, d.E, p->norm2_w, p->norm2_b, nullptr, 1, nullptr, sv.mean2, sv.rstd2, sv.sc2, sv.sh2,
                                  sc.in_ws, nullptr, sv.on, st));
        }
    }
    TRY(outproj_gemm(d, sv.on, wout_c, sv.alpha, sv.beta, x, sv.x1, drop_att, d.S, st));
    {
        bf_operand A = op_plain(sv.x1, d.E, BF_LAY_KC);
        bf_operand Bo = op_plain(w1_c, d.E, BF_LAY_KC);
        bf_epilogue e = epi_store(sv.pre, 4L * d.E);
        e.bias = p->fc1_b;
        e.gelu_out = sv.hid;
        TRY(bf_gemm(d.dtype, (int)d.N, 4 * d.E, d.E, &A, &Bo, &e, 1, st));
    }
    const float* g3 = p->gamma_mlp;
    int g3div = (int)d.F;
    if (drop_mlp) {
        if (d.dtype == BF_DTYPE_F32) {
            hipLaunchKernelGGL(frame_table_kernel, dim3(bf_cdiv(d.F * d.E, 256)), dim3(256), 0, st, drop_mlp, 1, (const float*)p->gamma_mlp, sv.gtab, (int)d.F, d.E);
            BF_CHECK_LAUNCH();
        }
        g3 = sv.gtab; g3div = 1;
    }
    if (d.dtype == BF_DTYPE_BF16) {
        const bf_frame_norm n1{p->mlp_norm_w, p->mlp_norm_b, g3, g3div, sv.mean3, sv.rstd3, sv.sc3, sv.sh3, sv.x1, out};
        const NextHead& h = H.head;
        const bf_frame_norm n2{h.w, h.b, nullptr, 1, h.mean, h.rstd, h.sc, h.sh, nullptr, h.xn};
        const int rc = bf_gemm_fwd_frames(d.dtype, (int)d.N, d.E, 4 * d.E, sv.hid, 4L * d.E, sv.w2t_c, d.E, p->fc2_b, nullptr, nullptr, nullptr, 1, nullptr, sv.z,
                                          (int)d.S, &n1, h.armed ? &n2 : nullptr, s);
        if (rc < 0) return rc;
        if (rc == 0) {
            if (h.armed) L.head_done = {h.saved, st};
            return 0;
        }
    }
    {
        bf_operand A = op_plain(sv.hid, 4L * d.E, BF_LAY_KC);
        bf_operand Bo = op_plain(w2_c, 4L * d.E, BF_LAY_KC);
        bf_epilogue e = epi_store(sv.z, d.E);
        e.bias = p->fc2_b;
        TRY(bf_gemm(d.dtype, (int)d.N, d.E, 4 * d.E, &A, &Bo, &e, 1, st));
    }
    if (H.head.armed) {
        const NextHead& h = H.head;
        bool chained = false;
        TRY(bf_in_stats_apply_chain(d.dtype, sv.z, (int)d.F, (int)d.S, d.E, p->mlp_norm_w, p->mlp_norm_b, g3, g3div, nullptr, sv.mean3, sv.rstd3, sv.sc3, sv.sh3,
                                    sc.in_ws, sv.x1, out, h.w, h.b, h.mean, h.rstd, h.sc, h.sh, h.xn, &chained, st));
        if (chained) L.head_done = {h.saved, st};
        return 0;
    }
    TRY(bf_in_stats_apply(d.dtype, sv.z, (int)d.F, (int)d.S, d.E, p->mlp_norm_w, p->mlp_norm_b, g3, g3div, nullptr, sv.mean3, sv.rstd3,
                          sv.sc3, sv.sh3, sc.in_ws, sv.x1, out, st));
    return 0;
}

static int spatial_bwd(TrunkLinks& L, const StageHints& H, const bf_dims* dims, const bf_spatial_params* p, const bf_spatial_params* g, const void* x,
                       const void* dout, void* dx, void* saved, void* scratch, const float* drop_att, const float* drop_mlp, bf_stream_t s) {
// ... 27 lines not shown
        bf_epilogue e; memset(&e, 0, sizeof(e));
        e.aux_mode = BF_AUX_DGELU; e.aux = sv.pre; e.ld_aux = 4L * d.E; e.out_mode = BF_OUT_STORE;
        static const bool use_t = bf_knob("BF_FC2_DGRAD_T", 1) != 0;
        TRY(linear_bwd(d, sc, dz, d.E, sv.hid, 4 * d.E, BF_PRO_NONE, nullptr, nullptr, w2_c, g->fc2_w, g->fc2_b, dpre, &e, st, fk, nullptr, false,
                       (!f32 && use_t) ? sv.w2t_c : nullptr));
    }
    void* dx1 = sc.t1b;
    bool dbr_done = false;
    {
        bf_epilogue e; memset(&e, 0, sizeof(e));
        e.aux_mode = BF_AUX_ADD; e.aux = dout; e.ld_aux = d.E; e.out_mode = BF_OUT_STORE;
        TRY(linear_bwd(d, sc, dpre, 4 * d.E, sv.x1, d.E, BF_PRO_NONE, nullptr, nullptr, w1_c, g->fc1_w, g->fc1_b, dx1, &e, st, fk, nullptr, false, nullptr,
                       drop_att ? sc.e5 : nullptr, drop_att, (int)d.S, &dbr_done));
    }
    void* don = sc.e6;
    const void* dbr = dx1;
    if (dbr_done) dbr = sc.e5;
    else if (drop_att) {
        TRY(bf_frame_scale(d.dtype, dx1, drop_att, 1, sc.e5, d.N, (int)d.S, d.E, st));
        dbr = sc.e5;
    }
    void* dO = sc.e7;
    const InFuse fu2{sv.o, nullptr, dO, sv.mean2, sv.rstd2, p->norm2_w, p->norm2_b, sc.in_ws2};
    TRY(outproj_bwd(d, sc, dbr, sv.on, sv.wout_s, p->output_head_w, p->output_head_b, p->norm2_b, p->gamma_att,
                    d.feat_scale ? p->low_freq_scalar : nullptr, d.feat_scale ? p->high_freq_scalar : nullptr, sv.alpha, sv.mc,
                    g->output_head_w, g->output_head_b, g->norm2_b, g->gamma_att, d.feat_scale ? g->low_freq_scalar : nullptr,
                    d.feat_scale ? g->high_freq_scalar : nullptr, don, st, fk, &fu2));
    TRY(jobs.push(InReduceJob{sc.in_ws2, (int)d.F, d.E, p->norm2_w, p->norm2_b, nullptr, 1, g->norm2_w, g->norm2_b, nullptr, nullptr, nullptr, nullptr}));
    void* dqkv = sc.t3;
    {
        int rows = 0;
        static const bool raw_on = bf_knob("BF_ATTN_RAW", 1) != 0;
        const bool rawm = raw_on && bf_attn_raw_modes(d.dtype, d.d);
        TRY(bf_attn_bwd_partials(d.dtype, sv.qkv, dO, dqkv, d.F * d.h, d.w, 1, d.w, 0, 1, d.heads, d.d, p->qnorm_w, p->qnorm_b, p->knorm_w, p->knorm_b,
                                 p->rel_pos_emb, d.attn_scale ? p->attn_scale_factor_x : nullptr, g->qnorm_w, g->qnorm_b, g->knorm_w, g->knorm_b,
                                 g->rel_pos_emb, d.attn_scale ? g->attn_scale_factor_x : nullptr, 0.5f, rawm ? 2 : 0, sc.attn_ws, Scratch::ATTN_WS_FLOATS, &rows, st));
        TRY(jobs.push(AttnReduceJob{sc.attn_ws, rows, d.d, d.heads, g->qnorm_w, g->qnorm_b, g->knorm_w, g->knorm_b, g->rel_pos_emb,
                                    d.attn_scale ? g->attn_scale_factor_x : nullptr}));
        TRY(bf_attn_bwd_partials(d.dtype, sv.qkv, dO, dqkv, d.F * d.w, d.h, d.w, d.S, 1, d.w, d.heads, d.d, p->qnorm_w, p->qnorm_b, p->knorm_w, p->knorm_b,
                                 p->rel_pos_emb, d.attn_scale ? p->attn_scale_factor_y : nullptr, g->qnorm_w, g->qnorm_b, g->knorm_w, g->knorm_b,
                                 g->rel_pos_emb, d.attn_scale ? g->attn_scale_factor_y : nullptr, 0.5f, rawm ? 5 : 1, sc.attn_ws2, Scratch::ATTN_WS_FLOATS, &rows, st));
        TRY(jobs.push(AttnReduceJob{sc.attn_ws2, rows, d.d, d.heads, g->qnorm_w, g->qnorm_b, g->knorm_w, g->knorm_b, g->rel_pos_emb,
                                    d.attn_scale ? g->attn_scale_factor_y : nullptr}));
    }
    void* dxn = sc.e6;
    InFuse fu1{x, dx1, dx, sv.mean1, sv.rstd1, p->norm1_w, p->norm1_b, sc.in_ws};
    bool scaled_done = false;
    const NextScale& ns = H.scale;
    L.dbr_ready = TrunkLinks::DbrReady{};
    static const bool scaled_on = bf_knob("BF_BWD_SCALED_COPY", 1) != 0;
    if (ns.f && scaled_on && fk.deferred && d.dtype == BF_DTYPE_BF16) {
        fu1.scaled_out = (char*)scratch + 2 * Scratch(d, nullptr).bytes + (L.dbr_flip ? dbr_bytes(d) : 0);
        fu1.scaled_f = ns.f; fu1.scaled_fdiv = ns.fdiv; fu1.scaled_done = &scaled_done;
    }
    TRY(linear_bwd(d, sc, dqkv, 3 * d.E, sv.xn, d.E, BF_PRO_NONE, nullptr, nullptr, win_c, g->input_head_w, g->input_head_b, dxn, nullptr, st, fk, &fu1, true));
    if (scaled_done) { L.dbr_ready = {dx, ns.f, fu1.scaled_out, st}; L.dbr_flip = !L.dbr_flip; }
    TRY(jobs.push(InReduceJob{sc.in_ws, (int)d.F, d.E, p->norm1_w, p->norm1_b, nullptr, 1, g->norm1_w, g->norm1_b, nullptr, nullptr, nullptr, nullptr}));
    static const bool merge_on = bf_knob("BF_REDUCE_MERGE", 1) != 0;
    if (fk.deferred && merge_on) { L.reduce.jobs = jobs; L.reduce.on = true; L.reduce.st = st; }
    else TRY(launch_reduce_jobs(jobs, st));
    return fk.join();
}
extern "C" int bf_spatial_fwd(const bf_dims* dims, const bf_spatial_params* p, const void* x, void* out, void* saved, void* scratch,
                              const float* drop_att, const float* drop_mlp, bf_stream_t s) {
    TrunkLinks& L = g_links.get();
    return spatial_fwd(L, L.take_hints(), dims, p, x, out, saved, scratch, drop_att, drop_mlp, s);
}
extern "C" int bf_spatial_bwd(const bf_dims* dims, const bf_spatial_params* p, const bf_spatial_params* g, const void* x, const void* dout,
                              void* dx, void* saved, void* scratch, const float* drop_att, const float* drop_mlp, bf_stream_t s) {
    TrunkLinks& L = g_links.get();
    return spatial_bwd(L, L.take_hints(), dims, p, g, x, dout, dx, saved, scratch, drop_att, drop_mlp, s);
}

extern "C" int bf_trunk_train_fwd(const bf_dims* dims, int n, const int32_t* kinds, const void* const* params, void* const* saved,
                                  const float* const* drop_a, const float* const* drop_b, const void* x, void* const* acts, void* scratch,
                                  bf_stream_t s) {
    D d; TRY(get_dims(dims, &d));
    BF_REQUIRE(n >= 1 && kinds && params && saved && x && acts && scratch, "bf_trunk_train_fwd: bad arguments");
    for (int i = 0; i < n; ++i)
        BF_REQUIRE(params[i] && saved[i] && acts[i] && (kinds[i] == 0 || kinds[i] == 1), "bf_trunk_train_fwd: bad stage entry");
    TrunkLinks& L = g_links.get();
    (void)L.take_hints();
    const bool b16 = d.dtype == BF_DTYPE_BF16;
    if (b16) {
        const int rc = prep_stages(L, dims, n, kinds, params, saved, drop_b, s);
        if (rc < 0) return rc;
    }
    for (int i = 0; i < n; ++i) {
        const void* in = i ? acts[i - 1] : x;
        StageHints H;
        H.prepared = b16;
        if (b16 && i + 1 < n && kinds[i + 1] != kinds[i]) H.head = next_head(d, kinds[i + 1], params[i + 1], saved[i + 1]);
        TRY(kinds[i] == 0
            ? temporal_fwd(L, H, dims, (const bf_temporal_params*)params[i], in, acts[i], saved[i], scratch, drop_a ? drop_a[i] : nullptr, s)
            : spatial_fwd(L, H, dims, (const bf_spatial_params*)params[i], in, acts[i], saved[i], scratch, drop_a ? drop_a[i] : nullptr,
                          drop_b ? drop_b[i] : nullptr, s));
    }
    return 0;
}

extern "C" int bf_trunk_train_bwd(const bf_dims* dims, int n, const int32_t* kinds, const void* const* params, const void* const* grads,
                                  void* const* saved, const float* const* drop_a, const float* const* drop_b, const void* x, void* const* acts,
                                  const void* dout, void* const* gbuf3, void* dx, void* scratch, bf_stage_done_fn stage_done, void* user,
                                  bf_stream_t s) {
    D d; TRY(get_dims(dims, &d));
    BF_REQUIRE(n >= 1 && kinds && params && grads && saved && x && acts && dout && gbuf3 && dx && scratch, "bf_trunk_train_bwd: bad arguments");
    BF_REQUIRE(gbuf3[0] && gbuf3[1] && gbuf3[2], "bf_trunk_train_bwd: three gradient buffers are needed");
    TrunkLinks& L = g_links.get();
    (void)L.take_hints();
    const void* cur = dout;
    int rot = 0;
    for (int i = n - 1; i >= 0; --i) {
        BF_REQUIRE(params[i] && grads[i] && saved[i] && (kinds[i] == 0 || kinds[i] == 1), "bf_trunk_train_bwd: bad stage entry");
        const void* in = i ? acts[i - 1] : x;
        void* gout = i ? gbuf3[rot] : dx;
        rot = (rot + 1) % 3;
        StageHints H;
        if (kinds[i] == 0) {
            if (i > 0 && kinds[i - 1] == 1) H.tail = NextTail{true, (const bf_spatial_params*)params[i - 1], saved[i - 1], drop_b && drop_b[i - 1]};
            TRY(temporal_bwd(L, H, dims, (const bf_temporal_params*)params[i], (const bf_temporal_params*)grads[i], in, cur, gout, saved[i], scratch,
                             drop_a ? drop_a[i] : nullptr, s));
        } else {
            if (i > 0 && kinds[i - 1] == 0 && drop_a && drop_a[i - 1]) H.scale = NextScale{drop_a[i - 1], d.T};
            TRY(spatial_bwd(L, H, dims, (const bf_spatial_params*)params[i], (const bf_spatial_params*)grads[i], in, cur, gout, saved[i], scratch,
                            drop_a ? drop_a[i] : nullptr, drop_b ? drop_b[i] : nullptr, s));
        }
        if (stage_done) stage_done(i, user);
        cur = gout;
    }
    return 0;
}
```

### bubbleformer_amd/csrc/model_common.h

```cpp
#pragma once
#include <algorithm>
#include <functional>
#include <vector>
#include "bf_common.h"
#include "param_reduce.h"
#include <stdlib.h>
#include <string.h>

int bf_gemm_tokred_flush(hipStream_t st);
bool bf_gemm_tokred_pending();

namespace bfm __attribute__((visibility("hidden"))) {

struct D {
    int dtype, B, T, h, w, E, heads, attn_scale, feat_scale, patch, cin, cout, nfluid;
    long N, F, S;
    int d, nst;
    size_t es;
};
inline int get_dims(const bf_dims* s, D* o) {
    if (!s) return bf_fail_msg("dims: null", __FILE__, __LINE__);
    o->dtype = s->dtype; o->B = s->B; o->T = s->T; o->h = s->h; o->w = s->w; o->E = s->E; o->heads = s->heads;
    o->attn_scale = s->attn_scale; o->feat_scale = s->feat_scale; o->patch = s->patch; o->cin = s->cin; o->cout = s->cout;
    o->nfluid = s->nfluid;
    if (o->B < 1 || o->T < 1 || o->h < 1 || o->w < 1 || o->E < 8 || o->E > 1024 || o->heads < 1 || o->E % o->heads)
        return bf_fail_msg("dims: bad sizes", __FILE__, __LINE__);
    if (o->dtype != BF_DTYPE_F32 && o->dtype != BF_DTYPE_BF16) return bf_fail_msg("dims: bad dtype", __FILE__, __LINE__);
    o->F = (long)o->B * o->T; o->S = (long)o->h * o->w; o->N = o->F * o->S; o->d = o->E / o->heads;
    o->es = bf_esize(o->dtype);
    const int ch = o->dtype == BF_DTYPE_BF16 ? 8 : 4;
    if (o->E % ch || o->d % ch) return bf_fail_msg("dims: E and head dim must be multiples of the 16-byte chunk", __FILE__, __LINE__);
    if (o->T > 128 || o->h > 128 || o->w > 128) return bf_fail_msg("dims: attention axes are limited to 128 tokens", __FILE__, __LINE__);
    o->nst = 0;
    if (o->patch > 0) {
        int p = o->patch;
        while (p > 1) { if (p & 1) return bf_fail_msg("dims: patch must be a power of two", __FILE__, __LINE__); p >>= 1; o->nst++; }
        if (o->nst < 1 || o->nst > BF_MAX_STAGES) return bf_fail_msg("dims: patch size out of range", __FILE__, __LINE__);
        if (o->nst > 1 && (o->E / 4) % ch) return bf_fail_msg("dims: E/4 must be a multiple of the 16-byte chunk", __FILE__, __LINE__);
    }
    return 0;
}

struct Arena {
    char* base; size_t off;
    explicit Arena(void* p) : base((char*)p), off(0) {}
    void* take(size_t bytes) { void* r = base ? base + off : nullptr; off += (bytes + 255) & ~(size_t)255; return r; }
    float* f32(size_t n) { return (float*)take(n * 4); }
};

inline bf_operand op_plain(const void* p, long ld, int layout) {
    bf_operand o; memset(&o, 0, sizeof(o)); o.p = p; o.ld = ld; o.layout = layout; return o;
}
inline void op_affine(bf_operand& o, int pro, const float* sc, const float* sh, long rpf, int nch) {
    o.pro = pro; o.sc = sc; o.sh = sh; o.rows_per_frame = (int)rpf; o.nch = nch;
}
inline void op_gather(bf_operand& o, int gw, int gh, int C) { o.gw = gw; o.gh = gh; o.gc = C; o.seglen = 2 * C; o.segstride = 2L * gw * C; }
inline bf_epilogue epi_store(void* c, long ldc) { bf_epilogue e; memset(&e, 0, sizeof(e)); e.c = c; e.ldc = ldc; e.out_mode = BF_OUT_STORE; return e; }
inline bf_epilogue epi_atomic(float* c, long ldc) { bf_epilogue e = epi_store(c, ldc); e.out_mode = BF_OUT_ATOMIC_F32; return e; }
inline void epi_scatter(bf_epilogue& e, int gw, int gh, int C) { e.gw = gw; e.gh = gh; e.gc = C; e.seglen = 2 * C; e.segstride = 2L * gw * C; }

inline int splitk_for(int M, int N, long K) {
    const long tiles = (long)bf_cdiv(M, 128) * bf_cdiv(N, 128);
    static const long target = bf_knob("BF_SPLITK_TARGET", 256);
    long s = (target + tiles / 2) / tiles;
    const long kt = (K + 63) / 64;
    if (s > kt / 4) s = kt / 4;
    if (s < 1) s = 1;
    return (int)s;
}

#define TRY(x) do { int rc__ = (x); if (rc__) return rc__; } while (0)
#define ZERO(ptr, bytes) do { hipError_t e__ = hipMemsetAsync((ptr), 0, (bytes), st); if (e__ != hipSuccess) return bf_fail(e__, __FILE__, __LINE__); } while (0)
#define ZERO_ON(stream, ptr, bytes) do { hipError_t e__ = hipMemsetAsync((ptr), 0, (bytes), (stream)); if (e__ != hipSuccess) return bf_fail(e__, __FILE__, __LINE__); } while (0)
#define HIP_TRY(x) do { hipError_t e__ = (x); if (e__ != hipSuccess) return bf_fail(e__, __FILE__, __LINE__); } while (0)

struct SideStream { hipStream_t st = nullptr; hipEvent_t fork = nullptr, join = nullptr, tail[2] = {nullptr, nullptr}; bool failed = false; bool pending[2] = {false, false}; };
bool side_defer();

struct NextHead { bool armed = false; const float *w = nullptr, *b = nullptr; float *mean = nullptr, *rstd = nullptr, *sc = nullptr, *sh = nullptr; void* xn = nullptr; const void* saved = nullptr; };
struct NextTail { bool armed = false; const bf_spatial_params* p = nullptr; const void* saved = nullptr; bool drop = false; };
struct NextScale { const float* f = nullptr; int fdiv = 1; };
struct StageHints { bool prepared = false; NextHead head; NextTail tail; NextScale scale; };

struct ReduceJobs {
    static constexpr int IN_CAP = 6, ATTN_CAP = 4;
    int n_in = 0, n_attn = 0; InReduceJob in[IN_CAP]; AttnReduceJob at[ATTN_CAP];
    bool at_follows[ATTN_CAP] = {};
    bool fits(const ReduceJobs& o) const { return n_in + o.n_in <= IN_CAP && n_attn + o.n_attn <= ATTN_CAP; }
    int push(const InReduceJob& j) { BF_REQUIRE(n_in < IN_CAP, "ReduceJobs: more InstanceNorm reductions than one launch holds"); in[n_in++] = j; return 0; }
    int push(const AttnReduceJob& j) { BF_REQUIRE(n_attn < ATTN_CAP, "ReduceJobs: more attention reductions than one launch holds"); at[n_attn++] = j; return 0; }
};

struct TrunkLinks {
    StageHints hints;
    StageHints take_hints() { const StageHints h = hints; hints = StageHints{}; return h; }
    struct HeadDone { const void* saved = nullptr; hipStream_t st = nullptr; } head_done;
    struct TailDone { const void* saved = nullptr; const void* dx = nullptr; float* ws = nullptr; hipStream_t st = nullptr; } tail_done;
    struct DbrReady { const void* dx = nullptr; const float* f = nullptr; void* buf = nullptr; hipStream_t st = nullptr; } dbr_ready;
    int scratch_parity = 0; bool tail_ws_flip = false, dbr_flip = false;
    bool take_head_done(const void* saved, hipStream_t st) { const bool hit = head_done.saved == saved && head_done.st == st; head_done = HeadDone{}; return hit; }
    struct { ReduceJobs jobs; bool on = false; hipStream_t st = nullptr; } reduce;
    hipEvent_t handoff = nullptr;
    SideStream side;
    std::vector<const void*> embed_lean;

    SideStream* side_stream() {
        static const bool enabled = bf_knob("BF_SIDE_STREAM", 1) != 0;
        if (!enabled) return nullptr;
        SideStream& s = side;
        if (!s.st && !s.failed) {
            int lo = 0, hi = 0;
            (void)hipDeviceGetStreamPriorityRange(&lo, &hi);
            const unsigned ef = hipEventDisableTiming | hipEventDisableSystemFence;
            if (hipStreamCreateWithPriority(&s.st, hipStreamNonBlocking, lo) != hipSuccess || hipEventCreateWithFlags(&s.fork, ef) != hipSuccess ||
                hipEventCreateWithFlags(&s.join, ef) != hipSuccess || hipEventCreateWithFlags(&s.tail[0], ef) != hipSuccess ||
                hipEventCreateWithFlags(&s.tail[1], ef) != hipSuccess) { s.failed = true; s.st = nullptr; }
        }
        return s.st ? &s : nullptr;
    }
    int hand_over(hipStream_t from, hipStream_t to) {
        if (from == to) return 0;
        if (!handoff) HIP_TRY(hipEventCreateWithFlags(&handoff, hipEventDisableTiming));
        HIP_TRY(hipEventRecord(handoff, from));
        HIP_TRY(hipStreamWaitEvent(to, handoff, 0));
        return 0;
    }
    void clear(bool forward_side) {
        if (forward_side) { hints.prepared = false; hints.head = NextHead{}; head_done = HeadDone{}; }
        hints.tail = NextTail{}; hints.scale = NextScale{}; tail_done = TailDone{}; dbr_ready = DbrReady{};
    }
    bool embed_lean_get(const void* saved) const { return std::find(embed_lean.begin(), embed_lean.end(), saved) != embed_lean.end(); }
    void embed_lean_set(const void* saved, bool lean) {
        const auto it = std::find(embed_lean.begin(), embed_lean.end(), saved);
        if (it == embed_lean.end()) { if (lean) embed_lean.push_back(saved); }
        else if (!lean) { *it = embed_lean.back(); embed_lean.pop_back(); }
    }
};
TrunkLinks& links();
int flush_pending_reduce(TrunkLinks& L, hipStream_t st);
int side_join_pending(TrunkLinks& L, hipStream_t main, int set = -1);

struct Fork {
    hipStream_t main; SideStream* s; bool used = false; bool deferred; int set;
    std::vector<std::function<int(hipStream_t)>> jobs;
    std::vector<std::function<int(hipStream_t)>> late;
    hipStream_t last_side = nullptr;
    explicit Fork(TrunkLinks& L, hipStream_t m, bool may_defer = false, int scratch_set = 0) : main(m), s(L.side_stream()), set(scratch_set) {
        deferred = may_defer && side_defer() && s != nullptr;
    }
    int begin(hipStream_t* out) {
        *out = main;
        if (!s) return 0;
        HIP_TRY(hipEventRecord(s->fork, main));
        HIP_TRY(hipStreamWaitEvent(s->st, s->fork, 0));
        used = true;
        *out = s->st;
        return 0;
    }
    template <class F> int run(F&& job) {
        hipStream_t ss;
        const int rc = begin(&ss);
        last_side = ss;
        return rc ? rc : job(ss);
    }
    template <class F> void run_late(F&& job) { late.push_back(job); }
    int drain_late() {
        if (late.empty()) return 0;
        hipStream_t ss = last_side ? last_side : main;
        for (auto& j : late) TRY(j(ss));
        late.clear();
        return 0;
    }
    int flush() {
        if (!deferred || jobs.empty()) return 0;
        hipStream_t ss;
        TRY(begin(&ss));
        for (auto& j : jobs) TRY(j(ss));
        jobs.clear();
        return 0;
    }
    int join() {
        if (deferred) {
            TRY(flush());
            TRY(drain_late());
            if (used) { HIP_TRY(hipEventRecord(s->tail[set], s->st)); s->pending[set] = true; used = false; }
            return 0;
        }
        TRY(drain_late());
        if (bf_gemm_tokred_pending()) TRY(bf_gemm_tokred_flush(last_side ? last_side : main));
        if (!s || !used) return 0;
        HIP_TRY(hipEventRecord(s->join, s->st));
        HIP_TRY(hipStreamWaitEvent(main, s->join, 0));
        used = false;
        return 0;
    }
};

struct Scratch {
    float *G, *csum, *zeros, *ones, *wg, *attn_ws, *attn_ws2, *in_ws, *in_ws2, *in_ws3, *in_ws4, *in_ws5;
    float* tokred_ws; int64_t tokred_floats;
    static constexpr long ATTN_WS_FLOATS = 1024L * (4 * 128 + 32 * 16 + 16);
    void *t1, *t3, *t4, *t1b; int64_t t1b_floats;
    void *s1, *e5, *e6, *e7;
    size_t bytes;
    Scratch(const D& d, void* base) {
        Arena a(base);
        const int cm = d.nst > 1 ? d.E / 4 : d.E;
        size_t wgn = (size_t)d.E * d.E;
        wgn = std::max(wgn, (size_t)4 * cm * d.E);
        wgn = std::max(wgn, (size_t)d.E * 64);
        G = a.f32((size_t)d.E * d.E);
        csum = a.f32((size_t)4 * d.E);
        zeros = a.f32((size_t)4 * d.E);
        ones = a.f32((size_t)4 * d.E);
        wg = a.f32(wgn);
        tokred_floats = bf_gemm_tokred_ws_floats(4 * d.E, d.E, d.N);
        tokred_ws = a.f32((size_t)tokred_floats);
        attn_ws = a.f32(ATTN_WS_FLOATS);
        attn_ws2 = a.f32(ATTN_WS_FLOATS);
        {
            int64_t n = bf_in_ws_floats(d.dtype, (int)d.F, (int)d.S, d.E);
            long Si = d.S;
            for (int i = 1; i < d.nst; ++i) { Si *= 4; n = std::max(n, bf_in_ws_floats(d.dtype, (int)d.F, (int)Si, cm)); }
// ... 63 lines not shown
```

### bubbleformer_amd/csrc/patch.hip

```cpp
#include "bf_common.h"
#include "param_reduce.h"
#include <algorithm>

namespace {
constexpr int NT = 256;

template <typename T>
__global__ void __launch_bounds__(NT) im2col_kernel(const float* __restrict__ x, T* __restrict__ out, int C, int H, int W,
                                                   int Kp, long P) {
    const int W2 = W / 2, H2 = H / 2;
    const long total = P * C;
    for (long i = (long)blockIdx.x * NT + threadIdx.x; i < total; i += (long)gridDim.x * NT) {
        const int xo = (int)(i % W2);
        long t = i / W2;
        const int c = (int)(t % C);
        t /= C;
        const int yo = (int)(t % H2);
        const long f = t / H2;
        const float* src = x + ((f * C + c) * H + 2 * yo) * (long)W + 2 * xo;
        const float2 r0 = *reinterpret_cast<const float2*>(src);
        const float2 r1 = *reinterpret_cast<const float2*>(src + W);
        const long p = (f * H2 + yo) * W2 + xo;
        T* dst = out + p * Kp + c * 4;
        dst[0] = from_f<T>(r0.x); dst[1] = from_f<T>(r0.y); dst[2] = from_f<T>(r1.x); dst[3] = from_f<T>(r1.y);
// ... 523 lines not shown

extern "C" int bf_im2col_nchw(int dtype, const float* x, void* out, int frames, int C, int H, int W, int Kp, bf_stream_t stream) {
    BF_REQUIRE(x && out && frames > 0 && C > 0 && H > 0 && W > 0 && H % 2 == 0 && W % 2 == 0 && Kp >= 4 * C, "bf_im2col_nchw: bad arguments");
    const long P = (long)frames * (H / 2) * (W / 2);
    hipStream_t st = (hipStream_t)stream;
    if (dtype == BF_DTYPE_BF16) {
        hipLaunchKernelGGL(im2col_kernel<bf16>, dim3(grid_for(P * C)), dim3(NT), 0, st, x, (bf16*)out, C, H, W, Kp, P);
        if (Kp > 4 * C) hipLaunchKernelGGL(zero_pad_cols_kernel<bf16>, dim3(grid_for(P * (Kp - 4 * C))), dim3(NT), 0, st, (bf16*)out, 4 * C, Kp, P);
    } else {
        hipLaunchKernelGGL(im2col_kernel<float>, dim3(grid_for(P * C)), dim3(NT), 0, st, x, (float*)out, C, H, W, Kp, P);
        if (Kp > 4 * C) hipLaunchKernelGGL(zero_pad_cols_kernel<float>, dim3(grid_for(P * (Kp - 4 * C))), dim3(NT), 0, st, (float*)out, 4 * C, Kp, P);
    }
    BF_CHECK_LAUNCH();
    return 0;
}

extern "C" int bf_col2im_nchw(int dtype, const void* g, float* dx, int frames, int C, int H, int W, int Kp, bf_stream_t stream) {
    BF_REQUIRE(g && dx && frames > 0 && C > 0 && H % 2 == 0 && W % 2 == 0 && Kp >= 4 * C, "bf_col2im_nchw: bad arguments");
    const long P = (long)frames * (H / 2) * (W / 2);
    if (dtype == BF_DTYPE_BF16) hipLaunchKernelGGL(col2im_kernel<bf16>, dim3(grid_for(P * C)), dim3(NT), 0, (hipStream_t)stream, (const bf16*)g, dx, C, H, W, Kp, P);
    else hipLaunchKernelGGL(col2im_kernel<float>, dim3(grid_for(P * C)), dim3(NT), 0, (hipStream_t)stream, (const float*)g, dx, C, H, W, Kp, P);
    BF_CHECK_LAUNCH();
    return 0;
}

extern "C" int bf_pm2nchw(const float* pm, float* pred, const float* y, float* lossbuf, int frames, int Co, int h, int w, int Np,
                          bf_stream_t stream) {
    BF_REQUIRE(pm && pred && frames > 0 && Co > 0 && h > 0 && w > 0 && Np >= 4 * Co && Np % 4 == 0, "bf_pm2nchw: bad arguments");
    BF_REQUIRE(!y || lossbuf, "bf_pm2nchw: loss buffer missing");
    dim3 grid(std::max(1, std::min(bf_cdiv((long)h * w, NT), 64)), frames);
    hipLaunchKernelGGL(pm2nchw_kernel, grid, dim3(NT), 0, (hipStream_t)stream, pm, pred, y, lossbuf, Co, h, w, Np);
    BF_CHECK_LAUNCH();
    return 0;
}

extern "C" int bf_debed_last(int dtype, const void* act, const float* sc, const float* sh, const void* wc, float* pred, const float* y,
                             float* lossbuf, int frames, int Ci, int Co, int h, int w, int Np, bf_stream_t stream) {
    BF_REQUIRE(act && sc && sh && wc && pred && frames > 0 && Ci > 0 && Co > 0 && h > 0 && w > 0, "bf_debed_last: bad arguments");
    BF_REQUIRE(!y || lossbuf, "bf_debed_last: loss buffer missing");
    if (dtype != BF_DTYPE_BF16 || Np != 16 || Co > 4 || Ci % 32 != 0 || Ci > 128 || w % 16 != 0) return 1;
    static const bool off = bf_knob("BF_DEBED_LAST", 1) == 0;
    if (off) return 1;
    const int GF = h * w / 16;
    dim3 grid(bf_cdiv(GF, (NT / 64) * DL_GPW), frames);
    hipStream_t st = (hipStream_t)stream;
    const double P = (double)frames * h * w;
    BfProfScope prof(st, "debed_last", 2.0 * P * Ci * 16, P * (2.0 * Ci + 16.0 * Co * (y ? 2 : 1)));
#define DL(KS) hipLaunchKernelGGL(debed_last_kernel<KS>, grid, dim3(NT), 0, st, (const bf16*)act, sc, sh, (const bf16*)wc, pred, y, lossbuf, Co, h, w)
    switch (Ci / 32) { case 1: DL(1); break; case 2: DL(2); break; case 3: DL(3); break; default: DL(4); break; }
#undef DL
    BF_CHECK_LAUNCH();
    return 0;
}

static int debed_last_bwd_launch(int dtype, const float* dpred, const float* pred, const float* y, const float* coef, const float* gscale,
                                 const void* wc, void* dpm, void* dact, int frames, int Ci, int Co, int h, int w, int Np, float* part,
                                 bf_stream_t stream) {
    BF_REQUIRE(wc && dpm && (dact || part) && (dpred || (pred && y && coef)) && frames > 0 && Ci > 0 && Co > 0 && h > 0 && w > 0, "bf_debed_last_bwd: bad arguments");
    if (dtype != BF_DTYPE_BF16 || Np != 16 || Co > 4 || Ci % 32 != 0 || Ci > 128 || w % 16 != 0) return 1;
    static const bool off = bf_knob("BF_DEBED_LAST_BWD", 1) == 0;
    if (off) return 1;
    const int GF = h * w / 16;
    dim3 grid(bf_cdiv(GF, (NT / 64) * DL_GPW), frames);
    hipStream_t st = (hipStream_t)stream;
    static const int perm = bf_knob("BF_DL_PERM", 1);
    const double P = (double)frames * h * w;
    BfProfScope prof(st, "patch16", 2.0 * P * Ci * 16, P * (2.0 * Ci + 32.0 + 16.0 * Co * (dpred ? 1 : 2)));
#define DLB(T) hipLaunchKernelGGL(debed_last_bwd_kernel<T>, grid, dim3(NT), 0, st, dpred, pred, y, coef, gscale, (const bf16*)wc, (bf16*)dpm, (bf16*)dact, Co, h, w, part, perm)
    switch (Ci / 32) { case 1: DLB(2); break; case 2: DLB(4); break; case 3: DLB(6); break; default: DLB(8); break; }
#undef DLB
    BF_CHECK_LAUNCH();
    return 0;
}

extern "C" int bf_debed_last_bwd(int dtype, const float* dpred, const float* pred, const float* y, const float* coef, const float* gscale,
                                 const void* wc, void* dpm, void* dact, int frames, int Ci, int Co, int h, int w, int Np, bf_stream_t stream) {
    return debed_last_bwd_launch(dtype, dpred, pred, y, coef, gscale, wc, dpm, dact, frames, Ci, Co, h, w, Np, nullptr, stream);
}

extern "C" int bf_debed_last_bwd_norm(int dtype, const float* dpred, const float* pred, const float* y, const float* coef, const float* gscale,
                                      const void* wc, void* dpm, const void* ymap, const float* mean, const float* rstd, const float* in_w,
                                      const float* in_b, void* dx, float* d_in_w, float* d_in_b, int frames, int Ci, int Co, int h, int w, int Np,
                                      float* ws, int64_t ws_floats, bf_stream_t stream) {
    if (dtype != BF_DTYPE_BF16 || Np != 16 || Co > 4 || Ci % 32 != 0 || Ci > 128 || w % 16 != 0)
        return bf_decline("bf_debed_last_bwd_norm covers bf16, Np = 16, Co <= 4, Ci a multiple of 32 up to 128, w a multiple of 16");
    static const bool off = bf_knob("BF_DEBED_LAST_NORM", 1) == 0;
    if (off) return bf_decline("bf_debed_last_bwd_norm: switched off (BF_DEBED_LAST_NORM=0)");
    BF_REQUIRE(wc && dpm && ymap && mean && rstd && in_w && in_b && dx && ws && (dpred || (pred && y && coef)) && frames > 0 && Co > 0 && h > 0 && w > 0,
               "bf_debed_last_bwd_norm: bad arguments");
    const int GF = h * w / 16, nsl = bf_cdiv(GF, DL_GPW);
    if (ws_floats < (int64_t)2 * frames * Ci * (1 + nsl))
        return bf_decline("bf_debed_last_bwd_norm: workspace smaller than 2 * frames * Ci * (1 + slices) floats (bf_in_ws_floats)");
    float* tot = ws;
    float* part = ws + (size_t)2 * frames * Ci;
    dim3 grid(bf_cdiv(GF, (NT / 64) * DL_GPW), frames);
    hipStream_t st = (hipStream_t)stream;
    const double P = (double)frames * h * w;
    const DlInb nb1{(const bf16*)ymap, mean, rstd, in_w, in_b, nullptr, 0.f};
    const DlInb nb2{(const bf16*)ymap, mean, rstd, in_w, in_b, tot, 1.0f / (float)(h * w)};
    {
        BfProfScope prof(st, "debed_last_bwd<stats>", 2.0 * P * Ci * 16, P * (2.0 * Ci + 32.0 + 16.0 * Co * (dpred ? 1 : 2)));
#define DLN(T) hipLaunchKernelGGL((debed_last_inbwd_kernel<T, 1>), grid, dim3(NT), 0, st, dpred, pred, y, coef, gscale, (const bf16*)wc, (bf16*)dpm, (bf16*)dx, Co, h, w, part, nb1)
        switch (Ci / 32) { case 1: DLN(2); break; case 2: DLN(4); break; case 3: DLN(6); break; default: DLN(8); break; }
#undef DLN
        BF_CHECK_LAUNCH();
    }
    hipLaunchKernelGGL(dl_slice_sum_kernel, dim3(bf_cdiv(Ci, 64), frames), dim3(NT), 0, st, (const float*)part, Ci, nsl, tot);
    BF_CHECK_LAUNCH();
    {
        BfProfScope prof(st, "debed_last_bwd<apply>", 2.0 * P * Ci * 16, P * (4.0 * Ci + 32.0));
#define DLN(T) hipLaunchKernelGGL((debed_last_inbwd_kernel<T, 2>), grid, dim3(NT), 0, st, nullptr, nullptr, nullptr, nullptr, nullptr, (const bf16*)wc, (bf16*)dpm, (bf16*)dx, Co, h, w, nullptr, nb2)
        switch (Ci / 32) { case 1: DLN(2); break; case 2: DLN(4); break; case 3: DLN(6); break; default: DLN(8); break; }
#undef DLN
        BF_CHECK_LAUNCH();
    }
    if (d_in_w || d_in_b) {
        const InReduceJob j{tot, frames, Ci, in_w, in_b, nullptr, 1, d_in_w, d_in_b, nullptr, nullptr, nullptr, nullptr};
        hipLaunchKernelGGL(dl_param_reduce_kernel, dim3(bf_cdiv(Ci, 64), bf_cdiv(frames, j.rdiv())), dim3(64 * BF_RED_FL), 0, st, j);
        BF_CHECK_LAUNCH();
    }
    return 0;
}

extern "C" int bf_embed_first(int dtype, const float* x, const void* wc, void* patches, void* y0, int frames, int C0, int cin, int h2, int w2,
                              int Kp, float* stat_part, bf_stream_t stream) {
    BF_REQUIRE(x && wc && patches && (y0 || stat_part), "bf_embed_first: null pointer");
    static const bool off = bf_knob("BF_EMBED_FIRST", 1) == 0;
    if (off) return 1;
    return debed_last_bwd_launch(dtype, x, nullptr, nullptr, nullptr, nullptr, wc, patches, y0, frames, C0, cin, h2, w2, Kp, stat_part, stream);
}

extern "C" int bf_lploss_finalize(const float* lossbuf, int frames, int Co, float* loss, float* coef, bf_stream_t stream) {
    BF_REQUIRE(lossbuf && loss && frames > 0 && Co > 0, "bf_lploss_finalize: bad arguments");
    hipLaunchKernelGGL(lploss_finalize_kernel, dim3(1), dim3(NT), 0, (hipStream_t)stream, lossbuf, frames, Co, loss, coef);
    BF_CHECK_LAUNCH();
    return 0;
}

extern "C" int bf_nchw2pm(int dtype, const float* dpred, const float* pred, const float* y, const float* coef, const float* gscale,
                          void* dpm, int frames, int Co, int h, int w, int Np, bf_stream_t stream) {
    BF_REQUIRE(dpm && (dpred || (pred && y && coef)) && Np >= 4 * Co && Np % 4 == 0, "bf_nchw2pm: bad arguments");
    const long P = (long)frames * h * w;
    if (dtype == BF_DTYPE_BF16) hipLaunchKernelGGL(nchw2pm_kernel<bf16>, dim3(grid_for(P * (Np / 4))), dim3(NT), 0, (hipStream_t)stream, dpred, pred, y, coef, gscale, (bf16*)dpm, Co, h, w, Np, P);
    else hipLaunchKernelGGL(nchw2pm_kernel<float>, dim3(grid_for(P * (Np / 4))), dim3(NT), 0, (hipStream_t)stream, dpred, pred, y, coef, gscale, (float*)dpm, Co, h, w, Np, P);
    BF_CHECK_LAUNCH();
    return 0;
}

extern "C" int bf_wprep(int dtype, int mode, const float* src, void* dst, int R, int K, int Kp, bf_stream_t stream) {
    BF_REQUIRE(src && dst && R > 0 && K > 0 && Kp >= K && mode >= 0 && mode <= 2, "bf_wprep: bad arguments");
    BF_REQUIRE(mode == 0 || Kp == K, "bf_wprep: padding only with mode 0");
    if (dtype == BF_DTYPE_BF16) hipLaunchKernelGGL(wprep_kernel<bf16>, dim3(grid_for((long)R * Kp)), dim3(NT), 0, (hipStream_t)stream, src, (bf16*)dst, mode, R, K, Kp);
    else hipLaunchKernelGGL(wprep_kernel<float>, dim3(grid_for((long)R * Kp)), dim3(NT), 0, (hipStream_t)stream, src, (float*)dst, mode, R, K, Kp);
    BF_CHECK_LAUNCH();
    return 0;
}

int bf_wprep_multi(int dtype, int n, const int* mode, const float* const* src, void* const* dst, const int* R, const int* K, const int* Kp, hipStream_t st) {
    BF_REQUIRE(n >= 1 && n <= BF_MAX_STAGES && mode && src && dst && R && K && Kp, "bf_wprep_multi: bad arguments");
    WprepJobs j;
    long most = 0;
    for (int i = 0; i < n; ++i) {
        BF_REQUIRE(src[i] && dst[i] && R[i] > 0 && K[i] > 0 && Kp[i] >= K[i] && mode[i] >= 0 && mode[i] <= 2 && (mode[i] == 0 || Kp[i] == K[i]), "bf_wprep_multi: bad entry");
        j.src[i] = src[i]; j.dst[i] = dst[i]; j.mode[i] = mode[i]; j.R[i] = R[i]; j.K[i] = K[i]; j.Kp[i] = Kp[i];
        most = std::max(most, (long)R[i] * Kp[i]);
    }
    const dim3 grid(std::min<long>(bf_cdiv(most, NT), 256), n);
    if (dtype == BF_DTYPE_BF16) hipLaunchKernelGGL(wprep_multi_kernel<bf16>, grid, dim3(NT), 0, st, j);
    else hipLaunchKernelGGL(wprep_multi_kernel<float>, grid, dim3(NT), 0, st, j);
    BF_CHECK_LAUNCH();
    return 0;
}

extern "C" int bf_wgrad_unprep(int mode, const float* gsrc, float* gdst, int R, int K, int Kp, int transposed, bf_stream_t stream) {
    BF_REQUIRE(gsrc && gdst && R > 0 && K > 0 && Kp >= K && mode >= 0 && mode <= 2, "bf_wgrad_unprep: bad arguments");
    hipLaunchKernelGGL(wgrad_unprep_kernel, dim3(grid_for((long)R * K)), dim3(NT), 0, (hipStream_t)stream, gsrc, gdst, mode, R, K, Kp, transposed);
    BF_CHECK_LAUNCH();
    return 0;
}

extern "C" int bf_film_net_fwd(const float* cond, const float* lnw, const float* lnb, const float* W, const float* bias, float* gb,
                               float* chat, float* crstd, int B, int P, int E2, bf_stream_t stream) {
    BF_REQUIRE(cond && lnw && lnb && W && bias && gb && chat && crstd && B > 0 && P > 0 && E2 > 0, "bf_film_net_fwd: bad arguments");
    hipLaunchKernelGGL(film_net_fwd_kernel, dim3(B), dim3(NT), 0, (hipStream_t)stream, cond, lnw, lnb, W, bias, gb, chat, crstd, B, P, E2);
    BF_CHECK_LAUNCH();
    return 0;
}

extern "C" int bf_film_net_bwd(const float* dgb, const float* chat, const float* lnw, const float* lnb, const float* W, float* dW,
// ... 7 lines not shown
```

### bubbleformer_amd/models/axial_vit.py

```python
import numpy as np
import torch
import torch.nn as nn

from .. import ops
from ..layers import AttentionBlock, AxialAttentionBlock, FiLMMLP, HMLPDebed, HMLPEmbed
from ._api import register_model

__all__ = ["AViT", "FiLMConditionedAViT", "SpaceTimeBlock"]


class SpaceTimeBlock(nn.Module):

    def __init__(self, embed_dim: int = 768, num_heads: int = 12, drop_path: float = 0.0, attn_scale: bool = True,
                 feat_scale: bool = True):
        super().__init__()
        self.temporal = AttentionBlock(embed_dim=embed_dim, num_heads=num_heads, drop_path=drop_path, attn_scale=attn_scale)
        self.spatial = AxialAttentionBlock(embed_dim=embed_dim, num_heads=num_heads, drop_path=drop_path, attn_scale=attn_scale,
                                           feat_scale=feat_scale)

    def forward_tokens(self, tok: torch.Tensor, drops=None, chain_to=None) -> torch.Tensor:
        if tok.is_cuda:
            ops.chain_next(self.spatial.stage_params(), "spatial")
        tok = self.temporal.forward_tokens(tok) if drops is None else self.temporal.forward_tokens(tok, drops[0])
        if chain_to is not None and tok.is_cuda:
            ops.chain_next(chain_to.stage_params())
        if drops is None:
            return self.spatial.forward_tokens(tok)
        return self.spatial.forward_tokens(tok, drops[1], drops[2])

    def forward(self, x: torch.Tensor) -> torch.Tensor:
        return ops.as_reference_layout(self.forward_tokens(ops.as_tokens(x)))


class _AxialBase(nn.Module):
    def _build(self, input_fields, output_fields, patch_size, embed_dim, num_heads, processor_blocks, drop_path, attn_scale,
               feat_scale, compute_dtype):
        self.compute_dtype = compute_dtype if compute_dtype is not None else torch.float32
        self.patch_size = patch_size
        self.embed = HMLPEmbed(patch_size=patch_size, in_channels=input_fields, embed_dim=embed_dim)
        self.dp = np.linspace(0, drop_path, processor_blocks)

    def _finish(self, output_fields, patch_size, embed_dim, num_heads, processor_blocks, attn_scale, feat_scale):
        self.blocks = nn.ModuleList([
            SpaceTimeBlock(embed_dim=embed_dim, num_heads=num_heads, drop_path=self.dp[i], attn_scale=attn_scale, feat_scale=feat_scale)
            for i in range(processor_blocks)
        ])
        self.debed = HMLPDebed(patch_size=patch_size, embed_dim=embed_dim, out_channels=output_fields)

    def _process(self, tok):
        if not self.training and not torch.is_grad_enabled() and len(self.blocks) > 0 and ops.trunk_eval_applies(tok):
            from .. import torch_ops
            b0 = self.blocks[0]
            kinds, params = [], []
            for blk in self.blocks:
                kinds += [0, 1]
                params += list(blk.temporal.stage_params()) + list(blk.spatial.stage_params())
            owner = self.__dict__.get("_bf_eval_owner")
            if owner is None:
                owner = self.__dict__["_bf_eval_owner"] = ops.new_eval_token()
            return torch.ops.bubbleformer_amd.trunk_eval(tok.contiguous(), b0.temporal.num_heads, bool(b0.temporal.attn_scale),
                                                        bool(b0.spatial.feat_scale), kinds, params, owner)
        rates = [float(getattr(blk.temporal.drop_path, "drop_prob", 0.0)) for blk in self.blocks]
        table = None
        if self.training and any(r > 0.0 for r in rates):
            B, F = tok.shape[0], tok.shape[0] * tok.shape[1]
            cache = self.__dict__.setdefault("_keep_cache", {})
            key = (str(tok.device), tuple(rates))
            if key not in cache:
                cache.clear()
                cache[key] = torch.tensor([1.0 - r for r in rates], dtype=torch.float32, device=tok.device)[:, None]
            keep = cache[key]
            table = torch.bernoulli(keep.expand(len(rates), B + 2 * F)).div_(keep)
        drops = [None] * len(self.blocks)
        if table is not None:
            for i in range(len(self.blocks)):
                if rates[i] > 0.0:
                    drops[i] = (table[i, :B], table[i, B:B + F], table[i, B + F:])
        if tok.is_cuda and self.blocks:
            b0 = self.blocks[0]
            seq = []
            for i, blk in enumerate(self.blocks):
                dr = drops[i]
                seq.append(("temporal", blk.temporal.stage_params(), None if dr is None else (dr[0],)))
                seq.append(("spatial", blk.spatial.stage_params(), None if dr is None else (dr[1], dr[2])))
            out = ops.trunk_train(tok, b0.temporal.num_heads, b0.temporal.attn_scale, b0.spatial.feat_scale, seq)
            if out is not None:
                return out
        if tok.is_cuda and self.blocks:
            b0 = self.blocks[0]
            stages = []
            for i, blk in enumerate(self.blocks):
                stages.append(("temporal", blk.temporal.stage_params(), None))
                stages.append(("spatial", blk.spatial.stage_params(), drops[i][2] if drops[i] is not None else None))
            ops.prepare_stages(tok, b0.temporal.num_heads, b0.temporal.attn_scale, b0.spatial.feat_scale, stages)
        try:
            for i, blk in enumerate(self.blocks):
                tok = blk.forward_tokens(tok, drops[i], self.blocks[i + 1].temporal if i + 1 < len(self.blocks) else None)
        finally:
            ops.discard_prepared()
        return tok


@register_model("avit")
class AViT(_AxialBase):
    def __init__(self, input_fields: int = 3, output_fields: int = 3, time_window: int = 12, patch_size: int = 16,
                 embed_dim: int = 768, num_heads: int = 12, processor_blocks: int = 12, drop_path: int = 0.2,
                 attn_scale: bool = True, feat_scale: bool = True, compute_dtype=None):
        super().__init__()
        self.drop_path = drop_path
        self._build(input_fields, output_fields, patch_size, embed_dim, num_heads, processor_blocks, drop_path, attn_scale,
                    feat_scale, compute_dtype)
        self._finish(output_fields, patch_size, embed_dim, num_heads, processor_blocks, attn_scale, feat_scale)

    def tokens(self, x):
        return self._process(self.embed.tokens(x, compute_dtype=self.compute_dtype))

    def forward(self, x: torch.Tensor) -> torch.Tensor:
        return self.debed.from_tokens(self.tokens(x))

    def forward_loss(self, x, target):
        return self.debed.loss_from_tokens(self.tokens(x), target)


@register_model("filmavit")
class FiLMConditionedAViT(_AxialBase):
    def __init__(self, input_fields: int = 3, output_fields: int = 3, time_window: int = 12, patch_size: int = 16,
                 embed_dim: int = 768, num_heads: int = 12, processor_blocks: int = 12, drop_path: int = 0.2,
                 attn_scale: bool = True, feat_scale: bool = True, num_fluid_params: int = 8, compute_dtype=None):
        super().__init__()
        self._build(input_fields, output_fields, patch_size, embed_dim, num_heads, processor_blocks, drop_path, attn_scale,
                    feat_scale, compute_dtype)
        self.film_embed = FiLMMLP(num_fluid_params, embed_dim)
        self._finish(output_fields, patch_size, embed_dim, num_heads, processor_blocks, attn_scale, feat_scale)

    def tokens(self, x, fluid_params):
        tok = self.embed.tokens(x, fluid_params, self.film_embed.film_params(), compute_dtype=self.compute_dtype)
        return self._process(tok)

    def forward(self, x: torch.Tensor, fluid_params: torch.Tensor) -> torch.Tensor:
        return self.debed.from_tokens(self.tokens(x, fluid_params))

    def forward_loss(self, x, fluid_params, target):
        return self.debed.loss_from_tokens(self.tokens(x, fluid_params), target)
```

### bubbleformer_amd/ops.py

```python
import collections
import ctypes as C
import os
from typing import List, Optional, Sequence

import torch

from . import _lib as L

_SCRATCH = {}


def _require_gpu(t: torch.Tensor) -> None:
    if not t.is_cuda:
        raise L.BubbleformerHipError(
            "bubbleformer_amd runs only on a ROCm GPU (gfx950): got a tensor on %s; there is no CPU fallback" % t.device)


def _dt(t: torch.dtype) -> int:
    if t == torch.float32:
        return L.BF_DTYPE_F32
    if t == torch.bfloat16:
        return L.BF_DTYPE_BF16
    raise L.BubbleformerHipError(f"unsupported compute dtype {t}")

# ... 324 lines not shown
        d = make_dims(x.dtype, B, T, h, w, E, heads, attn_scale, feat_scale)
        lib = L.lib()
        params = [_f32c(p) for p in params]
        drop_a = None if drop_a is None else drop_a.contiguous().float()
        drop_b = None if drop_b is None else drop_b.contiguous().float()
        pre = _LINKS.prepared.pop(_stage_key(kind, params), None) if _LINKS.prepared else None
        if pre is not None and (pre[0] != _dims_key(d) or (pre[2] is None) != (drop_b is None) or
                                (drop_b is not None and pre[2].data_ptr() != drop_b.data_ptr())):
            pre = None
        nxt, _LINKS.next = _LINKS.next, None
        if nxt is not None and nxt[0] != kind:
            pn = _LINKS.prepared.get(nxt)
            if pn is not None and pn[0][:7] == _dims_key(d)[:7]:
                dn = L.Dims(*pn[0])
                L.check(lib.bf_stage_chain_next(C.byref(dn), 0 if nxt[0] == "temporal" else 1, C.addressof(pn[3]), _p(pn[1])), "bf_stage_chain_next")
        if kind == "temporal":
            st = pre[3] if pre else L.TemporalParams(*[_p(p) for p in params])
            saved = pre[1] if pre else _saved(lib.bf_temporal_saved_bytes(C.byref(d)), x.device, "bf_temporal_saved_bytes")
            fwd = lib.bf_temporal_fwd
        else:
            st = pre[3] if pre else L.SpatialParams(*[_p(p) for p in params])
            saved = pre[1] if pre else _saved(lib.bf_spatial_saved_bytes(C.byref(d)), x.device, "bf_spatial_saved_bytes")
            fwd = lib.bf_spatial_fwd
        out = torch.empty_like(x)
        lib.bf_stage_prepared(1 if pre else 0)
        if kind == "temporal":
            rc = fwd(C.byref(d), C.byref(st), _p(x), _p(out), _p(saved), _p(scratch_for(d, x.device)), _p(drop_a), _stream())
        else:
            rc = fwd(C.byref(d), C.byref(st), _p(x), _p(out), _p(saved), _p(scratch_for(d, x.device)), _p(drop_a), _p(drop_b), _stream())
        L.check(rc, f"bf_{kind}_fwd")
        last, _LINKS.last_spatial = _LINKS.last_spatial, None
        lastt, _LINKS.last_temporal = _LINKS.last_temporal, None
        ctx.prev_spatial = ctx.next_scale = None
        if kind == "temporal" and drop_a is not None and x.dtype == torch.bfloat16:
            _LINKS.last_temporal = (out.data_ptr(), drop_a, T)
        if kind == "spatial" and lastt is not None and lastt[0] == x.data_ptr():
            ctx.next_scale = (lastt[1], lastt[2])
        if kind == "spatial":
            if x.dtype == torch.bfloat16 and os.environ.get("BF_STAGE_CHAIN", "1") != "0":
                _LINKS.last_spatial = (out.data_ptr(), (tuple(x.shape), x.dtype), st, saved, drop_b is not None, params)
        elif last is not None and last[0] == x.data_ptr() and last[1] == (tuple(x.shape), x.dtype):
            ctx.prev_spatial = last[2:]
        ctx.drops = (drop_a, drop_b)
        ctx.kind, ctx.cfg = kind, (heads, attn_scale, feat_scale)
        ctx.save_for_backward(x, saved, *[p for p in params if p is not None])
        ctx.mask = [p is not None for p in params]
        return out

    @staticmethod
    def backward(ctx, dout):
        x, saved, *ps = ctx.saved_tensors
        it = iter(ps)
        params = [next(it) if m else None for m in ctx.mask]
        heads, attn_scale, feat_scale = ctx.cfg
        B, T, h, w, E = x.shape
        d = make_dims(x.dtype, B, T, h, w, E, heads, attn_scale, feat_scale)
        lib = L.lib()
        dout = dout.contiguous()
        gviews, ret, direct = _stage_grads(params)
        if ctx.kind == "temporal":
            st, gs, bwd = L.TemporalParams(*[_p(p) for p in params]), L.TemporalParams(*[_p(g) for g in gviews]), lib.bf_temporal_bwd
        else:
            st, gs, bwd = L.SpatialParams(*[_p(p) for p in params]), L.SpatialParams(*[_p(g) for g in gviews]), lib.bf_spatial_bwd
        dx = torch.empty_like(x)
        drop_a, drop_b = ctx.drops
        if ctx.kind == "temporal":
            ps = getattr(ctx, "prev_spatial", None)
            if ps is not None and direct:
                L.check(lib.bf_stage_chain_tail(C.byref(ps[0]), _p(ps[1]), 1 if ps[2] else 0), "bf_stage_chain_tail")
            rc = bwd(C.byref(d), C.byref(st), C.byref(gs), _p(x), _p(dout), _p(dx), _p(saved), _p(scratch_for(d, x.device)), _p(drop_a), _stream())
        else:
            ns = getattr(ctx, "next_scale", None)
            if ns is not None and direct:
                lib.bf_stage_next_scale(_p(ns[0]), ns[1])
            rc = bwd(C.byref(d), C.byref(st), C.byref(gs), _p(x), _p(dout), _p(dx), _p(saved), _p(scratch_for(d, x.device)), _p(drop_a),
                     _p(drop_b), _stream())
        L.check(rc, f"bf_{ctx.kind}_bwd")
        if _DEFER["on"]:
            _DEFER["keep"].append((saved, dout, x))
        _stage_done(params, direct)
        return (dx, None, None, None, None, None, None, *ret)


class _TrunkFn(torch.autograd.Function):

    @staticmethod
    def forward(ctx, x, cfg, kinds, masks, drops, *flat):
        _require_gpu(x)
        heads, attn_scale, feat_scale = cfg
        x = x.contiguous()
        B, T, h, w, E = x.shape
        d = make_dims(x.dtype, B, T, h, w, E, heads, attn_scale, feat_scale)
        lib = L.lib()
        n = len(kinds)
        it = iter(flat)
        plist = [[_f32c(next(it)) if m else None for m in mask] for mask in masks]
        for kind, ps in zip(kinds, plist):
            _check_stage_params(kind, ps, E, heads, x.device)
        structs = [(L.TemporalParams if kind == "temporal" else L.SpatialParams)(*[_p(p) for p in ps]) for kind, ps in zip(kinds, plist)]
        kinds_c = (C.c_int32 * n)(*[0 if k == "temporal" else 1 for k in kinds])
        pp = (C.c_void_p * n)(*[C.addressof(s) for s in structs])
        nb = {"temporal": lib.bf_temporal_saved_bytes(C.byref(d)), "spatial": lib.bf_spatial_saved_bytes(C.byref(d))}
        if min(nb.values()) < 0:
            L.check(-1, "bf_*_saved_bytes")
        offs, total = [], 0
        for k in kinds:
            offs.append(total)
            total += (nb[k] + 255) // 256 * 256
        arena = torch.empty(total, dtype=torch.uint8, device=x.device)
        sp = (C.c_void_p * n)(*[arena.data_ptr() + o for o in offs])
        acts = torch.empty((max(n - 1, 1),) + tuple(x.shape), dtype=x.dtype, device=x.device)
        out = torch.empty_like(x)
        ap = (C.c_void_p * n)(*([acts[i].data_ptr() for i in range(n - 1)] + [out.data_ptr()]))
        da = [None if dr is None or dr[0] is None else dr[0].contiguous().float() for dr in drops]
        db = [None if dr is None or len(dr) < 2 or dr[1] is None else dr[1].contiguous().float() for dr in drops]
        dap = (C.c_void_p * n)(*[_p(t) for t in da])
        dbp = (C.c_void_p * n)(*[_p(t) for t in db])
        L.check(lib.bf_trunk_train_fwd(C.byref(d), n, kinds_c, pp, sp, dap, dbp, _p(x), ap, _p(scratch_for(d, x.device)), _stream()), "bf_trunk_train_fwd")
        ctx.cfg, ctx.kinds, ctx.masks, ctx.offs = cfg, kinds, masks, offs
        ctx.drops = (da, db)
        ctx.save_for_backward(x, arena, acts, *[p for ps in plist for p in ps if p is not None])
        return out

    @staticmethod
    def backward(ctx, dout):
        x, arena, acts, *flat = ctx.saved_tensors
        heads, attn_scale, feat_scale = ctx.cfg
        kinds, masks = ctx.kinds, ctx.masks
        B, T, h, w, E = x.shape
        d = make_dims(x.dtype, B, T, h, w, E, heads, attn_scale, feat_scale)
        lib = L.lib()
        n = len(kinds)
        it = iter(flat)
        plist = [[next(it) if m else None for m in mask] for mask in masks]
        pstructs, gstructs, rets, directs = [], [], [], []
        for kind, ps in zip(kinds, plist):
            gviews, ret, direct = _stage_grads(ps)
            cls = L.TemporalParams if kind == "temporal" else L.SpatialParams
            pstructs.append(cls(*[_p(p) for p in ps]))
            gstructs.append(cls(*[_p(g) for g in gviews]))
            rets.append(ret)
            directs.append(direct)
        kinds_c = (C.c_int32 * n)(*[0 if k == "temporal" else 1 for k in kinds])
        pp = (C.c_void_p * n)(*[C.addressof(s) for s in pstructs])
        gp = (C.c_void_p * n)(*[C.addressof(s) for s in gstructs])
        sp = (C.c_void_p * n)(*[arena.data_ptr() + o for o in ctx.offs])
        ap = (C.c_void_p * n)(*([acts[i].data_ptr() for i in range(n - 1)] + [None]))
        da, db = ctx.drops
        dap = (C.c_void_p * n)(*[_p(t) for t in da])
        dbp = (C.c_void_p * n)(*[_p(t) for t in db])
        dout = dout.contiguous()
        gbuf = torch.empty((3,) + tuple(x.shape), dtype=x.dtype, device=x.device)
        g3 = (C.c_void_p * 3)(*[gbuf[i].data_ptr() for i in range(3)])
        dx = torch.empty_like(x)
        on_ready = _DIRECT["on_ready"]
        errs = []

        def done(i, _user):
            try:
                if directs[i] and on_ready is not None:
                    on_ready([p.data_ptr() for p in plist[i] if p is not None])
            except BaseException as e:
                errs.append(e)

        cb = L.STAGE_DONE_FN(done)
        rc = lib.bf_trunk_train_bwd(C.byref(d), n, kinds_c, pp, gp, sp, dap, dbp, _p(x), ap, _p(dout), g3, _p(dx), _p(scratch_for(d, x.device)),
                                    C.cast(cb, C.c_void_p), None, _stream())
        L.check(rc, "bf_trunk_train_bwd")
        if errs:
            raise errs[0]
        if not all(directs):
            L.check(lib.bf_side_join(_stream()), "bf_side_join")
        if _DEFER["on"]:
            _DEFER["keep"].append((arena, acts, dout, x, gbuf))
        flat_ret = [g for ret, mask in zip(rets, masks) for g, m in zip(ret, mask) if m]
        return (dx, None, None, None, None, *flat_ret)


def trunk_train(tok: torch.Tensor, heads: int, attn_scale: bool, feat_scale: bool, stages) -> Optional[torch.Tensor]:
    if not tok.is_cuda or not stages or os.environ.get("BF_TRUNK_NATIVE", "1") == "0" or os.environ.get("BF_STAGE_CHAIN", "1") == "0":
        return None
    if tok.dim() != 5:
        raise L.BubbleformerHipError("trunk_train: tokens must be (B, T, h, w, E)")
    kinds = tuple(k for k, _, _ in stages)
    masks = tuple(tuple(p is not None for p in ps) for _, ps, _ in stages)
    flat = [p for _, ps, _ in stages for p in ps if p is not None]
    drops = [dr for _, _, dr in stages]
    return _TrunkFn.apply(tok, (heads, bool(attn_scale), bool(feat_scale)), kinds, masks, drops, *flat)


def temporal_block(x: torch.Tensor, heads: int, attn_scale: bool, params: List[Optional[torch.Tensor]], drop=None) -> torch.Tensor:
    return _BlockFn.apply(x, "temporal", heads, attn_scale, True, drop, None, *params)


def spatial_block(x: torch.Tensor, heads: int, attn_scale: bool, feat_scale: bool, params: List[Optional[torch.Tensor]], drop_att=None,
                  drop_mlp=None) -> torch.Tensor:
    return _BlockFn.apply(x, "spatial", heads, attn_scale, feat_scale, drop_att, drop_mlp, *params)

# ... 1313 lines not shown
```

### include/bubbleformer_hip.h

```cpp
#ifndef BUBBLEFORMER_HIP_H
#define BUBBLEFORMER_HIP_H

#include <stdint.h>

#ifdef __cplusplus
extern "C" {
#endif

typedef void* bf_stream_t;

enum { BF_DTYPE_F32 = 0, BF_DTYPE_BF16 = 1 };

enum { BF_LAY_KC = 0,
       BF_LAY_XC = 1   };
enum { BF_PRO_NONE = 0, BF_PRO_AFFINE = 1, BF_PRO_AFFINE_GELU = 2, BF_PRO_GELU = 3 };
enum { BF_AUX_NONE = 0, BF_AUX_ADD = 1 , BF_AUX_DGELU = 2  };
enum { BF_OUT_STORE = 0 , BF_OUT_ATOMIC_F32 = 2 ,
       BF_OUT_STORE_F32 = 1  };

typedef struct bf_operand {
    const void* p;
    int64_t ld;
    int32_t layout;
    int32_t seglen;
// ... 183 lines not shown
int64_t bf_bubble_links_ws_bytes(int64_t pairs, int max_bubbles);
int bf_bubble_links(const int32_t* labels, const int32_t* count, const int32_t* attached, const int32_t* area, int64_t sequences, int T, int H, int W,
                    int max_bubbles, int32_t* successor, int32_t* n_successors, int32_t* predecessor, int32_t* n_predecessors, int32_t* departure_area,
                    int32_t* events, void* ws, int64_t ws_bytes, bf_stream_t stream);
int bf_bubble_track_ids(const int32_t* count, const int32_t* successor, const int32_t* predecessor, int64_t sequences, int T, int max_bubbles,
                        int32_t* track_id, int32_t* n_tracks, bf_stream_t stream);
int bf_rollout_bubble_links(const float* pred, const float* frames, int64_t field_stride, int64_t total_frames, int nfields, const int64_t* first,
                            const int32_t* step, const int32_t* field, const float* diff, const float* div, int max_bubbles, const int32_t* labels,
                            const int32_t* count_pred, const int32_t* count_tgt, const int32_t* attached_pred, const int32_t* attached_tgt,
                            const int32_t* area_pred, const int32_t* area_tgt, int32_t* successor_pred, int32_t* successor_tgt, int32_t* n_successors_pred,
                            int32_t* n_successors_tgt, int32_t* predecessor_pred, int32_t* predecessor_tgt, int32_t* n_predecessors_pred,
                            int32_t* n_predecessors_tgt, int32_t* departure_area_pred, int32_t* departure_area_tgt, int32_t* events_pred,
                            int32_t* events_tgt, void* ws, int64_t ws_bytes, int B, int T, int C, int H, int W, int Ho, int Wo, int steps,
                            bf_stream_t stream);
int64_t bf_field_errors_ws_bytes(int64_t frames, int H, int W);
int bf_field_errors(const float* pred, const float* target, const float* sdf, int64_t frames, int H, int W, int interface_radius, int lo, int hi,
                    int want_spectra, float* rmse, float* max_error, float* boundary_rmse, float* interface_rmse, int32_t* interface_cells,
                    float* spectral_error, float* spectrum_error, float* spectrum_pred, float* spectrum_target, void* ws, int64_t ws_bytes,
                    bf_stream_t stream);
int bf_rollout_errors(const float* pred, const float* frames, int64_t field_stride, int64_t total_frames, int nfields, const int64_t* first,
                      const int32_t* step, const int32_t* field, const float* diff, const float* div, int sdf_channel, int interface_radius, int lo,
                      int hi, int want_spectra, float* rmse, float* max_error, float* boundary_rmse, float* interface_rmse, int32_t* interface_cells,
                      float* spectral_error, float* spectrum_error, float* spectrum_pred, float* spectrum_target, void* ws, int64_t ws_bytes, int B, int T,
                      int C, int H, int W, int Ho, int Wo, int steps, bf_stream_t stream);
int64_t bf_lp_rows_ws_doubles(int64_t rows, int64_t n);
int bf_lp_rows_fwd(const float* pred, const float* y, int64_t rows, int64_t n, double p, float* ratio, double* sums, double* ws, int64_t ws_doubles,
                   bf_stream_t stream);
int bf_lp_rows_bwd(const float* pred, const float* y, const float* g, const double* sums, int64_t rows, int64_t n, double p, float* dpred,
                   bf_stream_t stream);
int bf_eikonal_bwd(const float* phi, int64_t frames, int H, int W, float dx, const float* g, float* dphi, bf_stream_t stream);
int bf_lion(float* p, const float* g, float* m, int64_t n, float lr, float beta1, float beta2, float wd, float gscale,
            bf_stream_t stream);
int64_t bf_grad_norm_ws_doubles(int64_t n);
int bf_grad_norm(const float* g, int64_t n, float gscale, float max_norm, float* out, double* ws, int64_t ws_doubles, bf_stream_t stream);
int bf_adamw_dev(float* p, const float* g, float* m, float* v, int64_t n, int step, float lr, float beta1, float beta2, float eps,
                 float wd, float gscale, const float* coef_dev, float clip_value, bf_stream_t stream);
int bf_adam_dev(float* p, const float* g, float* m, float* v, int64_t n, int step, float lr, float beta1, float beta2, float eps,
                float wd, float gscale, const float* coef_dev, float clip_value, bf_stream_t stream);
int bf_lion_dev(float* p, const float* g, float* m, int64_t n, float lr, float beta1, float beta2, float wd, float gscale,
                const float* coef_dev, float clip_value, bf_stream_t stream);


typedef struct bf_dims {
    int32_t dtype;
    int32_t B, T, h, w;
    int32_t E, heads;
    int32_t attn_scale, feat_scale;
    int32_t patch;
    int32_t cin, cout;
    int32_t nfluid;
} bf_dims;

typedef struct bf_temporal_params {
    float *gamma, *attn_scale_factor, *norm1_w, *norm1_b, *norm2_w, *norm2_b, *input_head_w, *input_head_b,
          *output_head_w, *output_head_b, *qnorm_w, *qnorm_b, *knorm_w, *knorm_b, *rel_pos_emb;
} bf_temporal_params;
typedef struct bf_spatial_params {
    float *gamma_att, *gamma_mlp, *attn_scale_factor_x, *attn_scale_factor_y, *low_freq_scalar, *high_freq_scalar,
          *norm1_w, *norm1_b, *norm2_w, *norm2_b, *input_head_w, *input_head_b, *output_head_w, *output_head_b,
          *qnorm_w, *qnorm_b, *knorm_w, *knorm_b, *rel_pos_emb, *fc1_w, *fc1_b, *fc2_w, *fc2_b, *mlp_norm_w, *mlp_norm_b;
} bf_spatial_params;
#define BF_MAX_STAGES 5
typedef struct bf_embed_params {
    float* conv_w[BF_MAX_STAGES];
    float* in_w[BF_MAX_STAGES];
    float* in_b[BF_MAX_STAGES];
    float *film_ln_w, *film_ln_b, *film_w, *film_b;
} bf_embed_params;
typedef struct bf_debed_params {
    float* conv_w[BF_MAX_STAGES];
    float* in_w[BF_MAX_STAGES];
    float* in_b[BF_MAX_STAGES];
} bf_debed_params;

int64_t bf_temporal_saved_bytes(const bf_dims* d);
int64_t bf_spatial_saved_bytes(const bf_dims* d);
int64_t bf_embed_saved_bytes(const bf_dims* d);
int64_t bf_debed_saved_bytes(const bf_dims* d);
int64_t bf_scratch_bytes(const bf_dims* d);

int bf_prep_stages(const bf_dims* dims, int n, const int32_t* kinds, const void* const* params, void* const* saved,
                   const float* const* drop_mlp, bf_stream_t stream);
void bf_stage_prepared(int on);
int64_t bf_trunk_eval_weights_bytes(const bf_dims* dims, int n, const int32_t* kinds);
int bf_trunk_eval_prepare(const bf_dims* dims, int n, const int32_t* kinds, const void* const* params, void* weights, bf_stream_t stream);
int bf_trunk_eval_fwd(const bf_dims* dims, int n, const int32_t* kinds, const void* const* params, const void* weights, const void* x,
                      void* out, void* scratch, bf_stream_t stream);
typedef void (*bf_stage_done_fn)(int stage, void* user);
int bf_trunk_train_fwd(const bf_dims* dims, int n, const int32_t* kinds, const void* const* params, void* const* saved,
                       const float* const* drop_a, const float* const* drop_b, const void* x, void* const* acts, void* scratch, bf_stream_t stream);
int bf_trunk_train_bwd(const bf_dims* dims, int n, const int32_t* kinds, const void* const* params, const void* const* grads, void* const* saved,
                       const float* const* drop_a, const float* const* drop_b, const void* x, void* const* acts, const void* dout,
                       void* const* gbuf3, void* dx, void* scratch, bf_stage_done_fn stage_done, void* user, bf_stream_t stream);
int bf_stage_chain_head(const bf_dims* dims, const bf_temporal_params* next_p, void* next_saved);
int bf_stage_chain_next(const bf_dims* dims, int next_kind, const void* next_params, void* next_saved);
int bf_stage_chain_tail(const bf_spatial_params* prev_p, const void* prev_saved, int has_drop_mlp);
int bf_stage_next_scale(const float* factors, int fdiv);
int bf_temporal_fwd(const bf_dims* d, const bf_temporal_params* p, const void* x, void* out, void* saved, void* scratch,
                    const float* drop, bf_stream_t s);
int bf_temporal_bwd(const bf_dims* d, const bf_temporal_params* p, const bf_temporal_params* g, const void* x, const void* dout,
                    void* dx, void* saved, void* scratch, const float* drop, bf_stream_t s);
int bf_spatial_fwd(const bf_dims* d, const bf_spatial_params* p, const void* x, void* out, void* saved, void* scratch,
                   const float* drop_att, const float* drop_mlp, bf_stream_t s);
int bf_spatial_bwd(const bf_dims* d, const bf_spatial_params* p, const bf_spatial_params* g, const void* x, const void* dout,
                   void* dx, void* saved, void* scratch, const float* drop_att, const float* drop_mlp, bf_stream_t s);
int bf_embed_fwd(const bf_dims* d, const bf_embed_params* p, const float* x, const float* fluid, void* out, void* saved, void* scratch, bf_stream_t s);
int bf_embed_bwd(const bf_dims* d, const bf_embed_params* p, const bf_embed_params* g, const void* dout, float* dx_in, void* saved,
                 void* scratch, bf_stream_t s);
int bf_debed_fwd(const bf_dims* d, const bf_debed_params* p, const void* x, float* pred, const float* target, float* loss,
                 void* saved, void* scratch, bf_stream_t s);
int bf_debed_bwd(const bf_dims* d, const bf_debed_params* p, const bf_debed_params* g, const void* x, const float* dpred,
                 const float* pred, const float* target, const float* loss_scale, void* dx, void* saved, void* scratch,
                 bf_stream_t s);

enum { BF_CONV_PRO_NONE = 0, BF_CONV_PRO_AFFINE_GELU = 1 , BF_CONV_PRO_GELU = 2  };
typedef struct bf_conv_src {
    const void* p;
    int32_t C, nchw, f32;
} bf_conv_src;
typedef struct bf_conv_geo {
    int32_t F, Hi, Wi, Ho, Wo, kh, kw, stride, pad;
} bf_conv_geo;
int bf_conv_fwd(int dtype, const bf_conv_geo* geo, const bf_conv_src* s0, const bf_conv_src* s1, int pro, const float* sc, const float* sh,
                const void* w, int N, const float* bias, const bf_conv_src* resid, const bf_conv_src* out, int transposed, bf_stream_t stream);
int64_t bf_conv_wgrad_ws_floats(int R, int K, int64_t M);
int bf_conv_wgrad(int dtype, const bf_conv_geo* geo, const bf_conv_src* rows, const bf_conv_src* s0, const bf_conv_src* s1, int pro,
                  const float* sc, const float* sh, float* dw, int accumulate, float* ws, int64_t ws_floats, bf_stream_t stream);
int bf_conv_colsum(int dtype, const bf_conv_src* src, int F, int H, int W, float* out, int accumulate, float* ws, int64_t ws_floats,
                   bf_stream_t stream);
int64_t bf_gn_ws_floats(int F, int C, int G);
int bf_gn_fwd(int dtype, const bf_conv_src* s0, const bf_conv_src* s1, int F, int H, int W, int G, const float* gamma, const float* beta,
              float eps, float* mean, float* rstd, float* sc, float* sh, float* ws, bf_stream_t stream);
int bf_gn_bwd(int dtype, const float* dA, const bf_conv_src* s0, const bf_conv_src* s1, int F, int H, int W, int G, const float* gamma,
              const float* mean, const float* rstd, const float* sc, const float* sh, const bf_conv_src* add, const bf_conv_src* dx0,
              const bf_conv_src* dx1, float* dgamma, float* dbeta, int accumulate, float* ws, bf_stream_t stream);
int bf_unet_lploss_fwd(const float* pred, const float* target, int B, int T, int C, int64_t HW, float* loss, float* coef, float* ws,
                       bf_stream_t stream);
int bf_unet_lploss_bwd(const float* pred, const float* target, const float* coef, const float* dloss, int planes, int64_t HW, float* dpred,
                       bf_stream_t stream);

int64_t bf_bn_ws_floats(int64_t M, int C);
int bf_bn_fwd(int dtype, const void* x, int B, int64_t HW, int C, const float* gamma, const float* beta, float eps, float momentum,
              float* running_mean, float* running_var, int64_t* num_batches_tracked, float* mean, float* rstd, float* sc, float* sh, float* ws,
              bf_stream_t stream);
int bf_bn_eval(int B, int C, const float* gamma, const float* beta, float eps, const float* running_mean, const float* running_var, float* sc,
               float* sh, bf_stream_t stream);
int bf_bn_act(int dtype, const void* x, int B, int H, int W, int C, const float* sc, const float* sh, void* a, void* p, uint8_t* idx,
              bf_stream_t stream);
int bf_bn_bwd(int dtype, const float* dA, int64_t ldA, int offA, const void* dP, const uint8_t* idx, const void* x, int B, int H, int W, int C,
              const float* gamma, const float* mean, const float* rstd, const float* sc, const float* sh, void* dx, float* dgamma, float* dbeta,
              int accumulate, float* ws, bf_stream_t stream);

enum { BF_RENDER_SDF = 0 , BF_RENDER_TEMP = 1 , BF_RENDER_SPEED = 2  };
#define BF_RENDER_MAX_TILES 6
typedef struct bf_render_tile {
    const float* a;
    const float* b;
    const float* mask;
    int64_t frame_stride;
    int64_t slot_stride;
    int64_t mask_frame_stride, mask_slot_stride;
    const double* range;
    int32_t kind;
} bf_render_tile;
typedef struct bf_render_geom {
    int32_t H, W, scale, rows, cols, ox, oy, pitch_x, pitch_y, bar_dx, bar_w, img_h, img_w, stride;
// ... 19 lines not shown
```

Baseline: 824.4 samples/s.

## Overlap trunk weight prep, FiLM backward and debed wgrad on side stream

Forks the per-step trunk weight preparation onto the side stream before the embed forward, so it runs alongside the embedding, with the arena allocated early and reused by the trunk forward. It also moves the FiLM-net backward reduction onto the side stream during the embed backward, and launches the last debed weight-gradient GEMM as soon as the norm statistics are ready instead of after the full norm backward. Each piece sits behind its own knob. The cost is extra events and cross-stream dependencies, plus the risk of contention for compute units.

```diff
diff --git a/bubbleformer_amd/_lib.py b/bubbleformer_amd/_lib.py
--- a/bubbleformer_amd/_lib.py
+++ b/bubbleformer_amd/_lib.py
@@ -96,6 +96,8 @@
     "bf_debug_tokred_fold": (None, [C.c_int]),
     "bf_side_defer": (None, [C.c_int]),
     "bf_prep_stages": (C.c_int, [C.POINTER(Dims), C.c_int, C.POINTER(C.c_int32), C.POINTER(vp), C.POINTER(vp), C.POINTER(vp), vp]),
+    "bf_trunk_prep_fork": (C.c_int, [C.POINTER(Dims), C.c_int, C.POINTER(C.c_int32), C.POINTER(vp), C.POINTER(vp), C.POINTER(vp), vp]),
+    "bf_debug_end_folds": (None, [C.c_int]),
     "bf_stage_prepared": (None, [C.c_int]),
     "bf_trunk_train_fwd": (C.c_int, [C.POINTER(Dims), C.c_int, C.POINTER(C.c_int32), C.POINTER(vp), C.POINTER(vp), C.POINTER(vp), C.POINTER(vp), vp,
                                      C.POINTER(vp), vp, vp]),
diff --git a/bubbleformer_amd/csrc/bf_common.h b/bubbleformer_amd/csrc/bf_common.h
--- a/bubbleformer_amd/csrc/bf_common.h
+++ b/bubbleformer_amd/csrc/bf_common.h
@@ -2,6 +2,7 @@
 #include <hip/hip_runtime.h>
 #include <stdint.h>
 #include <math.h>
+#include <functional>
 
 #include "../../include/bubbleformer_hip.h"
 
@@ -45,6 +46,10 @@
                             float* mean, float* rstd, float* sc, float* sh, float* ws, const void* resid, void* out, const float* nw, const float* nb,
                             float* nmean, float* nrstd, float* nsc, float* nsh, void* nxn, bool* chained, hipStream_t stream);
 int bf_wprep_multi(int dtype, int n, const int* mode, const float* const* src, void* const* dst, const int* R, const int* K, const int* Kp, hipStream_t st);
+int bf_debed_last_bwd_norm_mid(int dtype, const float* dpred, const float* pred, const float* y, const float* coef, const float* gscale,
+                               const void* wc, void* dpm, const void* ymap, const float* mean, const float* rstd, const float* in_w,
+                               const float* in_b, void* dx, float* d_in_w, float* d_in_b, int frames, int Ci, int Co, int h, int w, int Np,
+                               float* ws, int64_t ws_floats, const std::function<int()>* after_stats, hipStream_t stream);
 int bf_frame_scale(int dtype, const void* z, const float* m, int fdiv, void* out, long nrows, int S, int C, hipStream_t st);
 
 int bf_gemm_slabs(int dtype, int M, int N, int K, const bf_operand* A, const bf_operand* B, float* out, long ldc, int accumulate, int splitk,
diff --git a/bubbleformer_amd/csrc/embed_debed.hip b/bubbleformer_amd/csrc/embed_debed.hip
--- a/bubbleformer_amd/csrc/embed_debed.hip
+++ b/bubbleformer_amd/csrc/embed_debed.hip
@@ -83,7 +83,12 @@
     hipStream_t st = (hipStream_t)s;
     TrunkLinks& L = links();
     L.clear(true);
-    TRY(side_join_pending(L, st));
+    {
+        TrunkLinks::PrepFork& pf = L.prep_fork;
+        const bool keep = pf.armed && !pf.seen_embed && pf.st == st;
+        if (keep) pf.seen_embed = true;
+        TRY(side_join_pending(L, st, -1, keep));
+    }
     EmbedSaved sv(d, saved);
     Scratch sc(d, scratch);
     const int n = d.nst, H = d.h * d.patch, W = d.w * d.patch;
@@ -173,14 +178,33 @@
     const int n = d.nst, H = d.h * d.patch, W = d.w * d.patch;
     auto buf = [&](int stage) { return (stage & 1) ? sc.t3 : sc.t4; };
     const bool film = d.nfluid > 0;
-    if (film) ZERO(sv.dgb, (size_t)2 * d.B * d.E * 4);
+    const int Sl = sv.gh[n - 1] * sv.gw[n - 1], Cl = sv.C[n - 1];
+    const bool film_side = film && n >= 2 && end_fold(FOLD_FILM_SIDE) && L.side_stream() != nullptr &&
+                           bf_in_ws_floats(d.dtype, (int)d.F, Sl, Cl) <= bf_in_ws_floats(d.dtype, (int)d.F, (int)d.S, d.E);
+    const size_t dgb_bytes = (size_t)2 * d.B * d.E * 4;
+    if (film && !film_side) ZERO(sv.dgb, dgb_bytes);
     void* dy = buf(n - 1);
-    TRY(bf_in_bwd(d.dtype, dout, sv.y[n - 1], nullptr, dy, (int)d.F, sv.gh[n - 1] * sv.gw[n - 1], sv.C[n - 1], sv.mean[n - 1], sv.rstd[n - 1],
-                  p->in_w[n - 1], p->in_b[n - 1], film ? sv.gb : nullptr, d.T, 0, g->in_w[n - 1], g->in_b[n - 1], film ? sv.dgb : nullptr,
-                  film ? sv.dgb + (size_t)d.B * d.E : nullptr, sc.in_ws, st));
-    if (film)
-        TRY(bf_film_net_bwd(sv.dgb, sv.chat, p->film_ln_w, p->film_ln_b, p->film_w, g->film_w, g->film_b, g->film_ln_w, g->film_ln_b, d.B,
-                            d.nfluid, 2 * d.E, st));
+    if (film_side) {
+        TRY(bf_in_bwd_partials(d.dtype, dout, sv.y[n - 1], nullptr, dy, (int)d.F, Sl, Cl, sv.mean[n - 1], sv.rstd[n - 1], p->in_w[n - 1], p->in_b[n - 1],
+                               sv.gb, d.T, 0, sc.in_ws2, st));
+    } else {
+        TRY(bf_in_bwd(d.dtype, dout, sv.y[n - 1], nullptr, dy, (int)d.F, Sl, Cl, sv.mean[n - 1], sv.rstd[n - 1],
+                      p->in_w[n - 1], p->in_b[n - 1], film ? sv.gb : nullptr, d.T, 0, g->in_w[n - 1], g->in_b[n - 1], film ? sv.dgb : nullptr,
+                      film ? sv.dgb + (size_t)d.B * d.E : nullptr, sc.in_ws, st));
+        if (film)
+            TRY(bf_film_net_bwd(sv.dgb, sv.chat, p->film_ln_w, p->film_ln_b, p->film_w, g->film_w, g->film_b, g->film_ln_w, g->film_ln_b, d.B,
+                                d.nfluid, 2 * d.E, st));
+    }
+    bool film_pending = film_side;
+    auto film_tail = [&](hipStream_t q) -> int {
+        ZERO_ON(q, sv.dgb, dgb_bytes);
+        ReduceJobs J;
+        TRY(J.push(InReduceJob{sc.in_ws2, (int)d.F, Cl, p->in_w[n - 1], p->in_b[n - 1], sv.gb, d.T, g->in_w[n - 1], g->in_b[n - 1], sv.dgb,
+                               sv.dgb + (size_t)d.B * d.E, nullptr, nullptr}));
+        TRY(run_reduce_jobs(J, q));
+        return bf_film_net_bwd(sv.dgb, sv.chat, p->film_ln_w, p->film_ln_b, p->film_w, g->film_w, g->film_b, g->film_ln_w, g->film_ln_b, d.B,
+                               d.nfluid, 2 * d.E, q);
+    };
     Fork fk(L, st);
     hipStream_t ss;
     for (int i = n - 1; i >= 1; --i) {
@@ -213,6 +237,7 @@
             TRY(wgrad_slabs_else_atomics(d, sc, sv.C[i], K4, sv.P[i], A, Bo, K4, ss));
         }
         TRY(bf_wgrad_unprep(1, sc.wg, g->conv_w[i], sv.C[i], K4, K4, 0, ss));
+        if (film_pending && (i <= n - 2 || i == 1)) { film_pending = false; TRY(film_tail(ss)); }
         if (i == 1 && !dx_in) {
             static const bool tail_on = bf_knob("BF_EMBED_TAIL", 1) != 0;
             const int64_t need = bf_embed_tail_ws_floats((int)d.F, sv.gh[1], sv.gw[1], cp, sv.Kp);
@@ -361,27 +386,33 @@
         bool normed = false;
         if (last) {
             void* dpm = sc.t1;
+            auto wgrad_last = [&]() -> int {
+                TRY(fk.begin(&ss));
+                const int nrc = (sv.Np == 16 && i > 0) ? bf_tokred_narrow(d.dtype, cin, sv.Pin[i], ain, dpm, sc.wg, cin, 0, 1, sv.sc[i - 1], sv.sh[i - 1], rpf,
+                                                                          sc.tokred_ws, sc.tokred_floats, ss) : 1;
+                if (nrc < 0) return nrc;
+                if (nrc == 1) {
+                    bf_operand A = op_plain(dpm, sv.Np, BF_LAY_XC);
+                    bf_operand Bo = op_plain(ain, cin, BF_LAY_XC);
+                    if (i > 0) op_affine(Bo, BF_PRO_AFFINE_GELU, sv.sc[i - 1], sv.sh[i - 1], rpf, cin);
+                    TRY(wgrad_slabs_else_atomics(d, sc, sv.Np, cin, sv.Pin[i], A, Bo, cin, ss, cin % 4 == 0));
+                }
+                return bf_wgrad_unprep(0, sc.wg, g->conv_w[i], cin, 4 * co, sv.Np, 1, ss);
+            };
+            bool wgrad_forked = false;
             if (i > 0) {
-                const int nrc = bf_debed_last_bwd_norm(d.dtype, dpred, pred, target, sv.coef, loss_scale, sv.wc[i], dpm, ain, sv.mean[i - 1], sv.rstd[i - 1],
-                                                       p->in_w[i - 1], p->in_b[i - 1], dact, g->in_w[i - 1], g->in_b[i - 1], (int)d.F, cin, co, sv.gh[i],
-                                                       sv.gw[i], sv.Np, sc.in_ws, bf_in_ws_floats(d.dtype, (int)d.F, (int)rpf, cin), st);
+                const std::function<int()> mid = [&]() -> int { wgrad_forked = true; return wgrad_last(); };
+                const int nrc = bf_debed_last_bwd_norm_mid(d.dtype, dpred, pred, target, sv.coef, loss_scale, sv.wc[i], dpm, ain, sv.mean[i - 1], sv.rstd[i - 1],
+                                                           p->in_w[i - 1], p->in_b[i - 1], dact, g->in_w[i - 1], g->in_b[i - 1], (int)d.F, cin, co, sv.gh[i],
+                                                           sv.gw[i], sv.Np, sc.in_ws, bf_in_ws_floats(d.dtype, (int)d.F, (int)rpf, cin),
+                                                           end_fold(FOLD_DEBED_EARLY) ? &mid : nullptr, st);
                 if (nrc < 0) return nrc;
                 normed = nrc == 0;
             }
             const int rc = normed ? 0 : bf_debed_last_bwd(d.dtype, dpred, pred, target, sv.coef, loss_scale, sv.wc[i], dpm, dact, (int)d.F, cin, co, sv.gh[i], sv.gw[i], sv.Np, st);
             if (rc < 0) return rc;
             if (rc == 1) TRY(bf_nchw2pm(d.dtype, dpred, pred, target, sv.coef, loss_scale, dpm, (int)d.F, co, sv.gh[i], sv.gw[i], sv.Np, st));
-            TRY(fk.begin(&ss));
-            const int nrc = (sv.Np == 16 && i > 0) ? bf_tokred_narrow(d.dtype, cin, sv.Pin[i], ain, dpm, sc.wg, cin, 0, 1, sv.sc[i - 1], sv.sh[i - 1], rpf,
-                                                                      sc.tokred_ws, sc.tokred_floats, ss) : 1;
-            if (nrc < 0) return nrc;
-            if (nrc == 1) {
-                bf_operand A = op_plain(dpm, sv.Np, BF_LAY_XC);
-                bf_operand Bo = op_plain(ain, cin, BF_LAY_XC);
-                if (i > 0) op_affine(Bo, BF_PRO_AFFINE_GELU, sv.sc[i - 1], sv.sh[i - 1], rpf, cin);
-                TRY(wgrad_slabs_else_atomics(d, sc, sv.Np, cin, sv.Pin[i], A, Bo, cin, ss, cin % 4 == 0));
-            }
-            TRY(bf_wgrad_unprep(0, sc.wg, g->conv_w[i], cin, 4 * co, sv.Np, 1, ss));
+            if (!wgrad_forked) TRY(wgrad_last());
             if (rc == 1) {
                 bf_operand A = op_plain(dpm, sv.Np, BF_LAY_KC);
                 bf_operand Bo = op_plain(sv.wc[i], sv.Np, BF_LAY_KC);
diff --git a/bubbleformer_amd/csrc/model.hip b/bubbleformer_amd/csrc/model.hip
--- a/bubbleformer_amd/csrc/model.hip
+++ b/bubbleformer_amd/csrc/model.hip
@@ -13,6 +13,7 @@
 namespace {
 
 bool g_side_defer = false;
+int g_end_folds = ~0;
 
 BfPerDevice<TrunkLinks> g_links;
 
@@ -22,6 +23,11 @@
 }
 
 bool bfm::side_defer() { return g_side_defer; }
+bool bfm::end_fold(EndFold which) {
+    static const int knobs = (bf_knob("BF_FOLD_PREP", 1) ? 1 << FOLD_PREP_FORK : 0) | (bf_knob("BF_FOLD_FILM", 1) ? 1 << FOLD_FILM_SIDE : 0) |
+                             (bf_knob("BF_FOLD_DEBED_EARLY", 1) ? 1 << FOLD_DEBED_EARLY : 0);
+    return ((knobs & g_end_folds) >> which) & 1;
+}
 TrunkLinks& bfm::links() { return g_links.get(); }
 int bfm::flush_pending_reduce(TrunkLinks& L, hipStream_t st) {
     if (!L.reduce.on) return 0;
@@ -29,9 +35,13 @@
     TRY(launch_reduce_jobs(L.reduce.jobs, L.reduce.st));
     return L.hand_over(L.reduce.st, st);
 }
-int bfm::side_join_pending(TrunkLinks& L, hipStream_t main, int set) {
+int bfm::side_join_pending(TrunkLinks& L, hipStream_t main, int set, bool keep_prep) {
     if (set < 0) TRY(flush_pending_reduce(L, main));
     SideStream* s = L.side_stream();
+    if (set < 0 && !keep_prep && L.prep_fork.armed) {
+        L.prep_fork = TrunkLinks::PrepFork{};
+        if (s && s->prep) HIP_TRY(hipStreamWaitEvent(main, s->prep, 0));
+    }
     if (set < 0 && bf_gemm_tokred_pending()) {
         hipStream_t ws_st = s ? s->st : main;
         TRY(bf_gemm_tokred_flush(ws_st));
@@ -459,6 +469,8 @@
 
 }
 
+int bfm::run_reduce_jobs(ReduceJobs& J, hipStream_t st) { return launch_reduce_jobs(J, st); }
+
 extern "C" int64_t bf_temporal_saved_bytes(const bf_dims* s) { D d; if (get_dims(s, &d)) return -1; return (int64_t)TemporalSaved(d, nullptr).bytes; }
 extern "C" int64_t bf_spatial_saved_bytes(const bf_dims* s) { D d; if (get_dims(s, &d)) return -1; return (int64_t)SpatialSaved(d, nullptr).bytes; }
 static size_t dbr_bytes(const D& d) { return (((size_t)d.N * d.E * d.es) + 255) & ~(size_t)255; }
@@ -466,6 +478,7 @@
 
 extern "C" void bf_side_defer(int on) { g_side_defer = on != 0; }
 extern "C" int bf_side_join(bf_stream_t s) { return side_join_pending(g_links.get(), (hipStream_t)s); }
+extern "C" void bf_debug_end_folds(int mask) { g_end_folds = mask; }
 
 extern "C" void bf_stage_prepared(int on) { g_links.get().hints.prepared = on != 0; }
 extern "C" int bf_stage_chain_tail(const bf_spatial_params* prev_p, const void* prev_saved, int has_drop_mlp) {
@@ -592,6 +605,8 @@
     return temporal_bwd(L, L.take_hints(), dims, p, g, x, dout, dx, saved, scratch, drop, s);
 }
 
+static int launch_prep_batches(const D& d, int n, const int32_t* kinds, const void* const* params, void* const* saved, const float* const* drop_mlp,
+                               hipStream_t st);
 static int prep_stages(TrunkLinks& L, const bf_dims* dims, int n, const int32_t* kinds, const void* const* params, void* const* saved,
                        const float* const* drop_mlp, bf_stream_t s) {
     D d; TRY(get_dims(dims, &d));
@@ -599,6 +614,10 @@
     if (d.dtype != BF_DTYPE_BF16) return 1;
     hipStream_t st = (hipStream_t)s;
     TRY(side_join_pending(L, st));
+    return launch_prep_batches(d, n, kinds, params, saved, drop_mlp, st);
+}
+static int launch_prep_batches(const D& d, int n, const int32_t* kinds, const void* const* params, void* const* saved, const float* const* drop_mlp,
+                               hipStream_t st) {
     for (int i0 = 0; i0 < n; i0 += PREP_BATCH) {
         PrepBatch b;
         memset(&b, 0, sizeof(b));
@@ -616,6 +635,24 @@
 extern "C" int bf_prep_stages(const bf_dims* dims, int n, const int32_t* kinds, const void* const* params, void* const* saved,
                               const float* const* drop_mlp, bf_stream_t s) {
     return prep_stages(g_links.get(), dims, n, kinds, params, saved, drop_mlp, s);
+}
+extern "C" int bf_trunk_prep_fork(const bf_dims* dims, int n, const int32_t* kinds, const void* const* params, void* const* saved,
+                                  const float* const* drop_mlp, bf_stream_t s) {
+    D d; TRY(get_dims(dims, &d));
+    BF_REQUIRE(n >= 1 && kinds && params && saved, "bf_trunk_prep_fork: bad arguments");
+    if (d.dtype != BF_DTYPE_BF16 || !end_fold(FOLD_PREP_FORK)) return 1;
+    TrunkLinks& L = g_links.get();
+    SideStream* sd = L.side_stream();
+    if (!sd) return 1;
+    hipStream_t st = (hipStream_t)s;
+    TRY(side_join_pending(L, st));
+    if (!sd->prep) HIP_TRY(hipEventCreateWithFlags(&sd->prep, hipEventDisableTiming | hipEventDisableSystemFence));
+    HIP_TRY(hipEventRecord(sd->fork, st));
+    HIP_TRY(hipStreamWaitEvent(sd->st, sd->fork, 0));
+    TRY(launch_prep_batches(d, n, kinds, params, saved, drop_mlp, sd->st));
+    HIP_TRY(hipEventRecord(sd->prep, sd->st));
+    L.prep_fork = TrunkLinks::PrepFork{true, saved[0], n, st, false};
+    return 0;
 }
 
 static int spatial_fwd(TrunkLinks& L, const StageHints& H, const bf_dims* dims, const bf_spatial_params* p, const void* x, void* out, void* saved,
@@ -809,7 +846,9 @@
     TrunkLinks& L = g_links.get();
     (void)L.take_hints();
     const bool b16 = d.dtype == BF_DTYPE_BF16;
-    if (b16) {
+    const TrunkLinks::PrepFork& pf = L.prep_fork;
+    const bool forked = pf.armed && pf.saved0 == saved[0] && pf.n == n && pf.st == (hipStream_t)s;
+    if (b16 && !forked) {
         const int rc = prep_stages(L, dims, n, kinds, params, saved, drop_b, s);
         if (rc < 0) return rc;
     }
diff --git a/bubbleformer_amd/csrc/model_common.h b/bubbleformer_amd/csrc/model_common.h
--- a/bubbleformer_amd/csrc/model_common.h
+++ b/bubbleformer_amd/csrc/model_common.h
@@ -74,8 +74,10 @@
 #define ZERO_ON(stream, ptr, bytes) do { hipError_t e__ = hipMemsetAsync((ptr), 0, (bytes), (stream)); if (e__ != hipSuccess) return bf_fail(e__, __FILE__, __LINE__); } while (0)
 #define HIP_TRY(x) do { hipError_t e__ = (x); if (e__ != hipSuccess) return bf_fail(e__, __FILE__, __LINE__); } while (0)
 
-struct SideStream { hipStream_t st = nullptr; hipEvent_t fork = nullptr, join = nullptr, tail[2] = {nullptr, nullptr}; bool failed = false; bool pending[2] = {false, false}; };
+struct SideStream { hipStream_t st = nullptr; hipEvent_t fork = nullptr, join = nullptr, tail[2] = {nullptr, nullptr}, prep = nullptr; bool failed = false; bool pending[2] = {false, false}; };
 bool side_defer();
+enum EndFold { FOLD_PREP_FORK = 0, FOLD_FILM_SIDE = 1, FOLD_DEBED_EARLY = 2 };
+bool end_fold(EndFold which);
 
 struct NextHead { bool armed = false; const float *w = nullptr, *b = nullptr; float *mean = nullptr, *rstd = nullptr, *sc = nullptr, *sh = nullptr; void* xn = nullptr; const void* saved = nullptr; };
 struct NextTail { bool armed = false; const bf_spatial_params* p = nullptr; const void* saved = nullptr; bool drop = false; };
@@ -101,6 +103,7 @@
     bool take_head_done(const void* saved, hipStream_t st) { const bool hit = head_done.saved == saved && head_done.st == st; head_done = HeadDone{}; return hit; }
     struct { ReduceJobs jobs; bool on = false; hipStream_t st = nullptr; } reduce;
     hipEvent_t handoff = nullptr;
+    struct PrepFork { bool armed = false; const void* saved0 = nullptr; int n = 0; hipStream_t st = nullptr; bool seen_embed = false; } prep_fork;
     SideStream side;
     std::vector<const void*> embed_lean;
 
@@ -138,7 +141,8 @@
 };
 TrunkLinks& links();
 int flush_pending_reduce(TrunkLinks& L, hipStream_t st);
-int side_join_pending(TrunkLinks& L, hipStream_t main, int set = -1);
+int run_reduce_jobs(ReduceJobs& J, hipStream_t st);
+int side_join_pending(TrunkLinks& L, hipStream_t main, int set = -1, bool keep_prep = false);
 
 struct Fork {
     hipStream_t main; SideStream* s; bool used = false; bool deferred; int set;
diff --git a/bubbleformer_amd/csrc/patch.hip b/bubbleformer_amd/csrc/patch.hip
--- a/bubbleformer_amd/csrc/patch.hip
+++ b/bubbleformer_amd/csrc/patch.hip
@@ -629,6 +629,13 @@
                                       const void* wc, void* dpm, const void* ymap, const float* mean, const float* rstd, const float* in_w,
                                       const float* in_b, void* dx, float* d_in_w, float* d_in_b, int frames, int Ci, int Co, int h, int w, int Np,
                                       float* ws, int64_t ws_floats, bf_stream_t stream) {
+    return bf_debed_last_bwd_norm_mid(dtype, dpred, pred, y, coef, gscale, wc, dpm, ymap, mean, rstd, in_w, in_b, dx, d_in_w, d_in_b, frames, Ci, Co, h, w,
+                                      Np, ws, ws_floats, nullptr, (hipStream_t)stream);
+}
+int bf_debed_last_bwd_norm_mid(int dtype, const float* dpred, const float* pred, const float* y, const float* coef, const float* gscale,
+                               const void* wc, void* dpm, const void* ymap, const float* mean, const float* rstd, const float* in_w,
+                               const float* in_b, void* dx, float* d_in_w, float* d_in_b, int frames, int Ci, int Co, int h, int w, int Np,
+                               float* ws, int64_t ws_floats, const std::function<int()>* after_stats, hipStream_t stream) {
     if (dtype != BF_DTYPE_BF16 || Np != 16 || Co > 4 || Ci % 32 != 0 || Ci > 128 || w % 16 != 0)
         return bf_decline("bf_debed_last_bwd_norm covers bf16, Np = 16, Co <= 4, Ci a multiple of 32 up to 128, w a multiple of 16");
     static const bool off = bf_knob("BF_DEBED_LAST_NORM", 1) == 0;
@@ -652,6 +659,8 @@
 #undef DLN
         BF_CHECK_LAUNCH();
     }
+    if (after_stats)
+        if (const int rc = (*after_stats)()) return rc < 0 ? rc : bf_fail_msg("bf_debed_last_bwd_norm: the hook behind the first pass failed", __FILE__, __LINE__);
     hipLaunchKernelGGL(dl_slice_sum_kernel, dim3(bf_cdiv(Ci, 64), frames), dim3(NT), 0, st, (const float*)part, Ci, nsl, tot);
     BF_CHECK_LAUNCH();
     {
diff --git a/bubbleformer_amd/models/axial_vit.py b/bubbleformer_amd/models/axial_vit.py
--- a/bubbleformer_amd/models/axial_vit.py
+++ b/bubbleformer_amd/models/axial_vit.py
@@ -47,7 +47,48 @@
         ])
         self.debed = HMLPDebed(patch_size=patch_size, embed_dim=embed_dim, out_channels=output_fields)
 
-    def _process(self, tok):
+    def _draw(self, B, F, device):
+        rates = [float(getattr(blk.temporal.drop_path, "drop_prob", 0.0)) for blk in self.blocks]
+        table = None
+        if self.training and any(r > 0.0 for r in rates):
+            cache = self.__dict__.setdefault("_keep_cache", {})
+            key = (str(device), tuple(rates))
+            if key not in cache:
+                cache.clear()
+                cache[key] = torch.tensor([1.0 - r for r in rates], dtype=torch.float32, device=device)[:, None]
+            keep = cache[key]
+            table = torch.bernoulli(keep.expand(len(rates), B + 2 * F)).div_(keep)
+        drops = [None] * len(self.blocks)
+        if table is not None:
+            for i in range(len(self.blocks)):
+                if rates[i] > 0.0:
+                    drops[i] = (table[i, :B], table[i, B:B + F], table[i, B + F:])
+        return drops
+
+    def _stage_seq(self, drops):
+        seq = []
+        for i, blk in enumerate(self.blocks):
+            dr = drops[i]
+            seq.append(("temporal", blk.temporal.stage_params(), None if dr is None else (dr[0],)))
+            seq.append(("spatial", blk.spatial.stage_params(), None if dr is None else (dr[1], dr[2])))
+        return seq
+
+    def _plan_trunk(self, x):
+        if not x.is_cuda or x.dim() != 5 or len(self.blocks) == 0 or self.compute_dtype != torch.bfloat16:
+            return None
+        if not self.training and not torch.is_grad_enabled():
+            return None
+        B, T, _, H, W = x.shape
+        if H % self.patch_size or W % self.patch_size:
+            return None
+        drops = self._draw(B, B * T, x.device)
+        seq = self._stage_seq(drops)
+        b0 = self.blocks[0]
+        ops.trunk_prep_fork((B, T, H // self.patch_size, W // self.patch_size, self.embed.embed_dim), self.compute_dtype, x.device,
+                            b0.temporal.num_heads, b0.temporal.attn_scale, b0.spatial.feat_scale, seq)
+        return drops, seq
+
+    def _process(self, tok, plan=None):
         if not self.training and not torch.is_grad_enabled() and len(self.blocks) > 0 and ops.trunk_eval_applies(tok):
             from .. import torch_ops
             b0 = self.blocks[0]
@@ -60,29 +101,10 @@
                 owner = self.__dict__["_bf_eval_owner"] = ops.new_eval_token()
             return torch.ops.bubbleformer_amd.trunk_eval(tok.contiguous(), b0.temporal.num_heads, bool(b0.temporal.attn_scale),
                                                         bool(b0.spatial.feat_scale), kinds, params, owner)
-        rates = [float(getattr(blk.temporal.drop_path, "drop_prob", 0.0)) for blk in self.blocks]
-        table = None
-        if self.training and any(r > 0.0 for r in rates):
-            B, F = tok.shape[0], tok.shape[0] * tok.shape[1]
-            cache = self.__dict__.setdefault("_keep_cache", {})
-            key = (str(tok.device), tuple(rates))
-            if key not in cache:
-                cache.clear()
-                cache[key] = torch.tensor([1.0 - r for r in rates], dtype=torch.float32, device=tok.device)[:, None]
-            keep = cache[key]
-            table = torch.bernoulli(keep.expand(len(rates), B + 2 * F)).div_(keep)
-        drops = [None] * len(self.blocks)
-        if table is not None:
-            for i in range(len(self.blocks)):
-                if rates[i] > 0.0:
-                    drops[i] = (table[i, :B], table[i, B:B + F], table[i, B + F:])
+        drops = plan[0] if plan is not None else self._draw(tok.shape[0], tok.shape[0] * tok.shape[1], tok.device)
         if tok.is_cuda and self.blocks:
             b0 = self.blocks[0]
-            seq = []
-            for i, blk in enumerate(self.blocks):
-                dr = drops[i]
-                seq.append(("temporal", blk.temporal.stage_params(), None if dr is None else (dr[0],)))
-                seq.append(("spatial", blk.spatial.stage_params(), None if dr is None else (dr[1], dr[2])))
+            seq = plan[1] if plan is not None else self._stage_seq(drops)
             out = ops.trunk_train(tok, b0.temporal.num_heads, b0.temporal.attn_scale, b0.spatial.feat_scale, seq)
             if out is not None:
                 return out
@@ -113,7 +135,8 @@
         self._finish(output_fields, patch_size, embed_dim, num_heads, processor_blocks, attn_scale, feat_scale)
 
     def tokens(self, x):
-        return self._process(self.embed.tokens(x, compute_dtype=self.compute_dtype))
+        plan = self._plan_trunk(x)
+        return self._process(self.embed.tokens(x, compute_dtype=self.compute_dtype), plan)
 
     def forward(self, x: torch.Tensor) -> torch.Tensor:
         return self.debed.from_tokens(self.tokens(x))
@@ -134,8 +157,9 @@
         self._finish(output_fields, patch_size, embed_dim, num_heads, processor_blocks, attn_scale, feat_scale)
 
     def tokens(self, x, fluid_params):
+        plan = self._plan_trunk(x)
         tok = self.embed.tokens(x, fluid_params, self.film_embed.film_params(), compute_dtype=self.compute_dtype)
-        return self._process(tok)
+        return self._process(tok, plan)
 
     def forward(self, x: torch.Tensor, fluid_params: torch.Tensor) -> torch.Tensor:
         return self.debed.from_tokens(self.tokens(x, fluid_params))
diff --git a/bubbleformer_amd/ops.py b/bubbleformer_amd/ops.py
--- a/bubbleformer_amd/ops.py
+++ b/bubbleformer_amd/ops.py
@@ -430,6 +430,52 @@
         return (dx, None, None, None, None, None, None, *ret)
 
 
+def _trunk_arena(d, kinds, device):
+    lib = L.lib()
+    nb = {"temporal": lib.bf_temporal_saved_bytes(C.byref(d)), "spatial": lib.bf_spatial_saved_bytes(C.byref(d))}
+    if min(nb.values()) < 0:
+        L.check(-1, "bf_*_saved_bytes")
+    offs, total = [], 0
+    for k in kinds:
+        offs.append(total)
+        total += (nb[k] + 255) // 256 * 256
+    return torch.empty(total, dtype=torch.uint8, device=device), offs
+
+
+_PREFORK = {"plan": None}
+
+
+def trunk_prep_fork(shape, dtype, device, heads: int, attn_scale: bool, feat_scale: bool, stages) -> bool:
+    _PREFORK["plan"] = None
+    device = torch.device(device)
+    if device.type != "cuda" or not stages or dtype != torch.bfloat16:
+        return False
+    if os.environ.get("BF_TRUNK_NATIVE", "1") == "0" or os.environ.get("BF_STAGE_CHAIN", "1") == "0":
+        return False
+    B, T, h, w, E = shape
+    d = make_dims(dtype, B, T, h, w, E, heads, attn_scale, feat_scale)
+    lib = L.lib()
+    kinds = tuple(k for k, _, _ in stages)
+    n = len(kinds)
+    plist = [[_f32c(p) for p in ps] for _, ps, _ in stages]
+    for kind, ps in zip(kinds, plist):
+        _check_stage_params(kind, ps, E, heads, device)
+    structs = [(L.TemporalParams if kind == "temporal" else L.SpatialParams)(*[_p(p) for p in ps]) for kind, ps in zip(kinds, plist)]
+    kinds_c = (C.c_int32 * n)(*[0 if k == "temporal" else 1 for k in kinds])
+    pp = (C.c_void_p * n)(*[C.addressof(s) for s in structs])
+    arena, offs = _trunk_arena(d, kinds, device)
+    sp = (C.c_void_p * n)(*[arena.data_ptr() + o for o in offs])
+    db = [None if dr is None or len(dr) < 2 or dr[1] is None else dr[1].contiguous().float() for _, _, dr in stages]
+    dbp = (C.c_void_p * n)(*[_p(t) for t in db])
+    rc = lib.bf_trunk_prep_fork(C.byref(d), n, kinds_c, pp, sp, dbp, _stream())
+    if rc != 0:
+        L.check(min(rc, 0), "bf_trunk_prep_fork")
+        return False
+    key = (_dims_key(d), kinds, tuple(_p(p) for ps in plist for p in ps), tuple(_p(t) for t in db), _stream())
+    _PREFORK["plan"] = {"key": key, "arena": arena, "offs": offs, "keep": (plist, db)}
+    return True
+
+
 class _TrunkFn(torch.autograd.Function):
 
     @staticmethod
@@ -443,25 +489,23 @@
         n = len(kinds)
         it = iter(flat)
         plist = [[_f32c(next(it)) if m else None for m in mask] for mask in masks]
-        for kind, ps in zip(kinds, plist):
-            _check_stage_params(kind, ps, E, heads, x.device)
+        da = [None if dr is None or dr[0] is None else dr[0].contiguous().float() for dr in drops]
+        db = [None if dr is None or len(dr) < 2 or dr[1] is None else dr[1].contiguous().float() for dr in drops]
+        plan, _PREFORK["plan"] = _PREFORK["plan"], None
+        key = (_dims_key(d), tuple(kinds), tuple(_p(p) for ps in plist for p in ps), tuple(_p(t) for t in db), _stream())
+        if plan is not None and plan["key"] == key:
+            arena, offs = plan["arena"], plan["offs"]
+        else:
+            for kind, ps in zip(kinds, plist):
+                _check_stage_params(kind, ps, E, heads, x.device)
+            arena, offs = _trunk_arena(d, kinds, x.device)
         structs = [(L.TemporalParams if kind == "temporal" else L.SpatialParams)(*[_p(p) for p in ps]) for kind, ps in zip(kinds, plist)]
         kinds_c = (C.c_int32 * n)(*[0 if k == "temporal" else 1 for k in kinds])
         pp = (C.c_void_p * n)(*[C.addressof(s) for s in structs])
-        nb = {"temporal": lib.bf_temporal_saved_bytes(C.byref(d)), "spatial": lib.bf_spatial_saved_bytes(C.byref(d))}
-        if min(nb.values()) < 0:
-            L.check(-1, "bf_*_saved_bytes")
-        offs, total = [], 0
-        for k in kinds:
-            offs.append(total)
-            total += (nb[k] + 255) // 256 * 256
-        arena = torch.empty(total, dtype=torch.uint8, device=x.device)
         sp = (C.c_void_p * n)(*[arena.data_ptr() + o for o in offs])
         acts = torch.empty((max(n - 1, 1),) + tuple(x.shape), dtype=x.dtype, device=x.device)
         out = torch.empty_like(x)
         ap = (C.c_void_p * n)(*([acts[i].data_ptr() for i in range(n - 1)] + [out.data_ptr()]))
-        da = [None if dr is None or dr[0] is None else dr[0].contiguous().float() for dr in drops]
-        db = [None if dr is None or len(dr) < 2 or dr[1] is None else dr[1].contiguous().float() for dr in drops]
         dap = (C.c_void_p * n)(*[_p(t) for t in da])
         dbp = (C.c_void_p * n)(*[_p(t) for t in db])
         L.check(lib.bf_trunk_train_fwd(C.byref(d), n, kinds_c, pp, sp, dap, dbp, _p(x), ap, _p(scratch_for(d, x.device)), _stream()), "bf_trunk_train_fwd")
diff --git a/include/bubbleformer_hip.h b/include/bubbleformer_hip.h
--- a/include/bubbleformer_hip.h
+++ b/include/bubbleformer_hip.h
@@ -289,6 +289,9 @@
 int bf_prep_stages(const bf_dims* dims, int n, const int32_t* kinds, const void* const* params, void* const* saved,
                    const float* const* drop_mlp, bf_stream_t stream);
 void bf_stage_prepared(int on);
+int bf_trunk_prep_fork(const bf_dims* dims, int n, const int32_t* kinds, const void* const* params, void* const* saved,
+                       const float* const* drop_mlp, bf_stream_t stream);
+void bf_debug_end_folds(int mask);
 int64_t bf_trunk_eval_weights_bytes(const bf_dims* dims, int n, const int32_t* kinds);
 int bf_trunk_eval_prepare(const bf_dims* dims, int n, const int32_t* kinds, const void* const* params, void* weights, bf_stream_t stream);
 int bf_trunk_eval_fwd(const bf_dims* dims, int n, const int32_t* kinds, const void* const* params, const void* weights, const void* x,
```

Measured after the change: 831.1 samples/s (median of 6 runs). About the same (+0.8%).
